# adelacvg/NS2VC

Measured on NVIDIA B200. Metric: denoiser-steps/s, higher is better.
Workload: dtype f32 (3xBF16-split tensor-core contractions, fp32 accumulate)

## Files before the change

### ns2vc_b200/csrc/common.cuh

```cuda
#pragma once
#include <cuda_runtime.h>
#include <cuda_bf16.h>
#include <stdint.h>
#include <stddef.h>

namespace ns2vc {

void set_error(const char* fmt, ...);
const char* get_error();

#define NS_CHECK_CUDA(expr)                                                                    \
  do {                                                                                         \
    cudaError_t _e = (expr);                                                                   \
    if (_e != cudaSuccess) {                                                                   \
      ns2vc::set_error("%s:%d CUDA error %s: %s", __FILE__, __LINE__, cudaGetErrorName(_e),    \
                       cudaGetErrorString(_e));                                                \
      return -2;                                                                               \
    }                                                                                          \
  } while (0)

#define NS_REQUIRE(cond, ...)                                                                  \
  do {                                                                                         \
    if (!(cond)) {                                                                             \
      ns2vc::set_error(__VA_ARGS__);                                                           \
      return -1;                                                                               \
    }                                                                                          \
  } while (0)

struct SplitBuf {
  __nv_bfloat16* hi;
  __nv_bfloat16* lo;
  int T;
  int C;
  int ld;
  long long bpitch;
};

struct alignas(128) TMap { unsigned long long v[16]; };

enum PrepMode : int { PREP_RAW = 0, PREP_AFFINE = 1, PREP_AFFINE_SILU = 2 };
struct GnStats {
  const double* sum1; const double* sq1;
  const double* sum2; const double* sq2;
  const float* gamma; const float* beta;
  const float* film; int film_ld;
  int G; float eps;
  double inv_n;
};
struct alignas(16) PrepOp {
  const float* src1; int ld1; int C1;
  const float* src2; int ld2; int C2;
  int B, T_src, T_dst;
  int row_mul, row_add;
  const int* rowmap;
  int mode;
  const float* scale; const float* shift;
  GnStats gn;
  SplitBuf out;
  SplitBuf raw;
  unsigned long long* span;
};

constexpr int kMaxSrc = 4;
constexpr int kMaxSeg = 8;

struct GSeg {
  int src;
  int c0;
  int nkb;
  int tap;
};

enum EpiFlags : int {
  EPI_BIAS = 1,
  EPI_RESIDUAL = 2,
  EPI_GEGLU = 4,
  EPI_OUT_NCT = 8,
  EPI_ROWBIAS = 16,
  EPI_OUT_F32 = 32,
  EPI_OUT_SPLIT = 64,
  EPI_STATS = 128,
  EPI_LNFOLD = 256,
  EPI_ROWSTATS = 512,
  EPI_RELU = 1024,
  EPI_ROWMASK = 2048,
};

constexpr int kMaxXSeg = 4;
struct XSeg {
  int src;
  int c0;
  int ncb;
  int ntap;
  int kb_tap[3];
  int xf;
  int aff_c0;
};

struct GemmOp {
  SplitBuf src[kMaxSrc];
  int nsrc;
  GSeg seg[kMaxSeg];
  int nseg;
  int nkb_total;
  int B, T_out;
  const __nv_bfloat16* w_hi;
  const __nv_bfloat16* w_lo;
  const float* w_f32;
  int N;
  int flags;
  const float* bias;
  const float* rowbias;
  int rowbias_ld;
  const float* res;
  int res_ld;
  float* out;
  int out_ld;
  __nv_bfloat16* out_hi;
  __nv_bfloat16* out_lo;
  int out_split_ld;
  int n_valid;
  const double* ln_stats;
  const float* ln_g;
  int ln_C; float ln_eps;
  double* row_stats;
  int f16_col0;
  double* stat_sum;
  double* stat_sq;
  unsigned long long* trace;
  unsigned long long* span;
  int tma_out;
  int bn;
  int xmode;
  int ksplit;
  int nxs;
  XSeg xs[kMaxXSeg];
  const PrepOp* pre;
  const float* pre_film;
  const float* rowmask;
  TMap tmap[2 * kMaxSrc];
  TMap tmap_out[3];
};
void plan_gemm(GemmOp& op);
constexpr int kXfMaxC = 1024;
int gemm_sm_count();

int launch_gemm_tc(const GemmOp& op, cudaStream_t st);
int launch_gemm_simt(const GemmOp& op, cudaStream_t st);
int encode_tmaps(GemmOp& op);

struct PackSeg {
  const float* w;
  int n_rows;
  int cin_total;
  int ktaps;
  int tap;
  int cin0, ncin;
  int n_dst0;
  int kb0;
  int nkb;
  int geglu_half;
  const float* cscale;
};
int launch_pack_b(const PackSeg& ps, __nv_bfloat16* w_hi, __nv_bfloat16* w_lo, float* w_f32, int Npad,
                  cudaStream_t st);

int launch_prep_split(const PrepOp& op, cudaStream_t st);

int launch_ln_split(const float* x, int ld, int M, int C, float eps, const float* gamma, const float* beta,
                    SplitBuf out, cudaStream_t st, unsigned long long* span = nullptr);

struct AttnOp {
  const float* q; int q_ld;
  const float* k; int k_ld;
  const float* v; int v_ld;
  const float* bias;
  float* out; int out_ld;
  __nv_bfloat16* out_hi;
  __nv_bfloat16* out_lo;
  int out_split_ld;
  int B, H, Tq, Tk, dh;
  float scale;
  unsigned long long* span;
  unsigned long long* trace;
  SplitBuf qs, ks, vs;
  int q_c0, k_c0, v_c0;
  int v2;
  int pb;
  int p_split;
  TMap tm[6];
};
int launch_attention(const AttnOp& op, cudaStream_t st, bool simt_debug);
int launch_attention_v2(const AttnOp& op, cudaStream_t st);
bool attention_v2_supported(int dh, int Tk, bool biased);
bool attention_v2_p_fp16();
int encode_attn_tmaps(AttnOp& op);
int encode_tmap_rows(TMap* out, const __nv_bfloat16* base, int C, int T, int B, int ld, int box_c, int box_rows, int swizzle_bytes);
int encode_tmap_any(TMap* out, const void* base, int elem_bytes, int C, int T, int B, int ld, int box_c, int box_rows, int swizzle_bytes,
                    long long bpitch = 0);

int launch_ln_stats(const float* x, int ld, int M, int C, float eps, float* stats , cudaStream_t st);
int launch_ln_apply(const float* x, int ld, int M, int C, float eps, const float* gamma, const float* beta,
                    float* y, int y_ld, cudaStream_t st);

int launch_nct_to_tokens(const float* x, long long bstride, int B, int C, int T, float* out, int ldo, int Cpad,
                         cudaStream_t st);
int launch_nct_to_split(const float* x, long long bstride, int B, int C, int T, SplitBuf out, cudaStream_t st, const void* warm = nullptr,
                        long long warm_bytes = 0);
int launch_tokens_to_nct(const float* x, int ld, int B, int C, int T, float* out, cudaStream_t st);

enum LinIn : int { LIN_RAW = 0, LIN_SILU = 1, LIN_SINUSOID = 2 };
struct LinOp {
  const float* x; int x_ld; int M; int K;
  const float* W; const float* bias; int N;
  const float* add; int add_ld;
  int add_rows;
  float* out; int out_ld;
  int in_mode; int flip_sin_to_cos; float freq_shift;
  int out_silu;
};
int launch_small_linear(const LinOp& op, cudaStream_t st);

int launch_pool_class_token(const float* xn , const float* pos , int B, int S, int C,
                            float* tokens , cudaStream_t st);
int launch_pool_attend(const float* q , const float* kv , int B, int S1, int C, int heads,
                       float* out , cudaStream_t st);
int launch_mask_bias(const uint8_t* mask, int n, float* bias, cudaStream_t st);

struct DpmStepCoef {
  float alpha_s, sigma_s;
  float c_x;
  float c_m;
  float c_d;
  float inv_r0;
  int order;
};
int launch_dpm_step(const float* x, const float* unet_out, const float* m_prev, const DpmStepCoef& c,
                    float* m_cur, float* x_next, size_t n, int* nan_flag, cudaStream_t st);

struct UniPcStepCoef {
  float alpha_t, sigma_t;
  float c_x, c_m;
  float ab;
  float rk;
  float rho0, rho1;
  int corr_order;
  float n_c_x, n_c_m, nab, nrk;
  int pred_order;
};
int launch_unipc_step(const float* x_prev, const float* x_eval, const float* unet_out, const float* m0,
                      const float* m1, const UniPcStepCoef& c, float* m_t, float* x_t, float* x_pred, size_t n,
                      int* nan_flag, cudaStream_t st);

int launch_seq_mask(const long long* len, int B, int T, float* keep, float* kbias, cudaStream_t st);
int launch_enc_input(const float* x, long long bstride, const float* rowbias, const float* keep, int B, int C, int T, float* out, int ld,
                     cudaStream_t st);
int launch_ln_mask(const float* x, int ld, int M, int C, float eps, const float* gamma, const float* beta, const float* keep, float* y, int y_ld,
                   cudaStream_t st);
int launch_pool_attend_wide(const float* q, const float* kv, int B, int S1, int C, int heads, float* out, cudaStream_t st);
int launch_tbc_weight(const float* w, int k, int cin, int cout, float* o, cudaStream_t st);
int launch_ffn_taps(const float* const* w, int k, int F, int H, int centre, float scale, float* o, cudaStream_t st);
int launch_scale_vec(const float* a, float s, float* o, int n, cudaStream_t st);
int launch_ln_fold_vec(const float* W, const float* gamma, const float* beta, const float* bias, float* g, float* bf, int N, int C, cudaStream_t st);

inline int ceil_div(int a, int b) { return (a + b - 1) / b; }

}
```

### ns2vc_b200/csrc/engine.cu

```cuda
#include "common.cuh"
#include "../../include/ns2vc_b200.h"

#include <algorithm>
#include <cmath>
#include <cstdio>
#include <cstdlib>
#include <cstring>
#include <map>
#include <string>
#include <unordered_map>
#include <vector>

using namespace ns2vc;

namespace {

struct PlanOp {
  enum Kind { PUSH, POP_CAT, RESNET, XFORMER, DOWN, UP } kind;
  std::string prefix;
  int cin = 0, cout = 0, level = 0;
  int c1 = 0, c2 = 0;
};

struct WSlot {
  std::string name;
  std::vector<int64_t> shape;
  float* d = nullptr;
  bool loaded = false;
  size_t numel() const { size_t n = 1; for (auto s : shape) n *= (size_t)s; return n; }
};

struct PackedB {
  __nv_bfloat16* hi = nullptr;
  __nv_bfloat16* lo = nullptr;
  float* f32 = nullptr;
  int Npad = 0, nkb = 0, n_logical = 0;
};

inline int pad_to(int v, int m) { return (v + m - 1) / m * m; }
inline int nkb_of(int c) { return (c + 63) / 64; }

struct ResnetSite {
  std::string p;
  int c1, c2, cin, cout;
  bool shortcut;
  PackedB conv1, conv2;
  float* bias2 = nullptr;
  int film_off = 0;
};
struct XformerSite {
  std::string p;
  int c;
  PackedB proj_in, qkv, out1, q2, out2, ff1, ff2, proj_out;
  PackedB ff2p; float* bias_ff2p = nullptr;
  int kv_off = 0;
  int v_off = 0;
  float* g_qkv = nullptr; float* bf_qkv = nullptr;
  float* g_q2 = nullptr; float* bf_q2 = nullptr;
  float* g_ff1 = nullptr; float* bf_ff1 = nullptr;
};
struct ConvSite { std::string p; int c; PackedB w; };

struct Launch {
  enum Kind { GEMM, ATTN, LN_SPLIT, LN_APPLY, LINEAR, NCT2SPLIT, POOL_CLS, POOL_ATT, MASKBIAS, PREP, MEMSET, TAP } kind;
  GemmOp gemm;
  AttnOp attn;
  LinOp lin;
  PrepOp prep;
  SplitBuf split;
  const float* a = nullptr; const float* b = nullptr; const float* c = nullptr; float* o = nullptr;
  int i0 = 0, i1 = 0, i2 = 0, i3 = 0; float f0 = 0;
  void* mem = nullptr; size_t mem_bytes = 0;
  int patch = 0;
  int tap_index = -1;
  int reads_film = 0;
  int time_path = 0;
};

struct Arena {
  uint8_t* base = nullptr;
  size_t off = 0;
  template <class T> T* get(size_t n) {
    off = (off + 255) & ~(size_t)255;
    T* p = base ? reinterpret_cast<T*>(base + off) : nullptr;
    off += n * sizeof(T);
    return p;
  }
};

}

struct ns2vc_unet {
  ns2vc_unet_cfg cfg;
  int ted = 0;
  std::vector<PlanOp> plan;
  std::vector<WSlot> weights;
  std::unordered_map<std::string, int> windex;
  bool finalized = false;
  bool simt = false;
  std::string plan_str;

  std::vector<ResnetSite> resnets;
  std::vector<XformerSite> xformers;
  std::vector<ConvSite> resamplers;
  PackedB convin_lat, convin_content, conv_out, kv_all;
  int kv_total = 0, k_total = 0, film_total = 0;
  float* film_W = nullptr; float* film_b = nullptr;
  float* pool_kv_W = nullptr; float* pool_kv_b = nullptr;
  std::vector<void*> owned;

  int pB = 0, pT = 0, pS = 0; void* pws = nullptr; bool has_mask = false; bool cond_ready = false;
  float* aug = nullptr;
  std::vector<void*> static_bufs;
  std::vector<Launch> prog_cond, prog_fwd;
  std::vector<std::string> tap_names; std::vector<int> tap_level, tap_ch;
  std::vector<float*> tap_dst;
  struct Stash {
    int pB, pT, pS; void* pws; bool has_mask, cond_ready;
    std::vector<Launch> prog_cond, prog_fwd; float* film_base; float* aug;
    std::vector<std::string> tap_names; std::vector<int> tap_level, tap_ch; std::vector<float*> tap_dst;
  };
  std::vector<Stash> stash;
  int last_launches = 0;
  bool profiling = false;
  bool ksplit = true;
  bool xf = true;
  bool merge_ff = true;
  float* film_base = nullptr;
  const float* film_ext = nullptr;
  bool lnfold = true;
  unsigned long long* trace = nullptr; int trace_cap = 0;
  unsigned long long* attn_trace = nullptr; int attn_trace_cap = 0;
  unsigned long long* span = nullptr; int span_cap = 0;
  struct ProfRec { int kind; cudaEvent_t a, b; int M, N, K, nseg, ctas; };
  std::vector<ProfRec> prof;

  const float* W(const std::string& n) const {
    auto it = windex.find(n);
    return it == windex.end() ? nullptr : weights[it->second].d;
  }
};

namespace {

int level_len(int T, int level) {
  for (int i = 0; i < level; ++i) T = (T - 1) / 2 + 1;
  return T;
}

void add_w(ns2vc_unet* h, const std::string& n, std::vector<int64_t> shape) {
  h->windex[n] = (int)h->weights.size();
  WSlot s; s.name = n; s.shape = std::move(shape);
  h->weights.push_back(std::move(s));
}
void add_conv(ns2vc_unet* h, const std::string& p, int co, int ci, int k) { add_w(h, p + ".weight", {co, ci, k}); add_w(h, p + ".bias", {co}); }
void add_lin(ns2vc_unet* h, const std::string& p, int co, int ci, bool bias = true) { add_w(h, p + ".weight", {co, ci}); if (bias) add_w(h, p + ".bias", {co}); }
void add_norm(ns2vc_unet* h, const std::string& p, int c) { add_w(h, p + ".weight", {c}); add_w(h, p + ".bias", {c}); }

void build_plan(ns2vc_unet* h) {
  const ns2vc_unet_cfg& c = h->cfg;
  const int n = c.n_levels;
  std::vector<int> skip;
  auto push = [&](int ch, int level) { PlanOp o; o.kind = PlanOp::PUSH; o.cout = ch; o.level = level; h->plan.push_back(o); skip.push_back(ch); };
  int ch = c.block_out_channels[0], level = 0;
  push(ch, 0);
  for (int i = 0; i < n; ++i) {
    const int cout = c.block_out_channels[i];
    for (int j = 0; j < c.layers_per_block[i]; ++j) {
      PlanOp r; r.kind = PlanOp::RESNET; r.prefix = "down_blocks." + std::to_string(i) + ".resnets." + std::to_string(j);
      r.cin = ch; r.cout = cout; r.level = level; r.c1 = ch; r.c2 = 0; h->plan.push_back(r);
      ch = cout;
      if (c.down_has_attn[i]) {
        PlanOp x; x.kind = PlanOp::XFORMER; x.prefix = "down_blocks." + std::to_string(i) + ".attentions." + std::to_string(j);
        x.cin = x.cout = ch; x.level = level; h->plan.push_back(x);
      }
      push(ch, level);
    }
    if (i != n - 1) {
      ++level;
      PlanOp d; d.kind = PlanOp::DOWN; d.prefix = "down_blocks." + std::to_string(i) + ".downsamplers.0"; d.cin = d.cout = ch; d.level = level;
      h->plan.push_back(d);
      push(ch, level);
    }
  }
  auto res = [&](const std::string& p, int c1, int c2, int cout) {
    PlanOp r; r.kind = PlanOp::RESNET; r.prefix = p; r.cin = c1 + c2; r.cout = cout; r.level = level; r.c1 = c1; r.c2 = c2; h->plan.push_back(r);
  };
  auto xf = [&](const std::string& p, int cc) {
    PlanOp x; x.kind = PlanOp::XFORMER; x.prefix = p; x.cin = x.cout = cc; x.level = level; h->plan.push_back(x);
  };
  res("mid_block.resnets.0", ch, 0, ch);
  xf("mid_block.attentions.0", ch);
  res("mid_block.resnets.1", ch, 0, ch);
  for (int i = 0; i < n; ++i) {
    const int cout = c.block_out_channels[n - 1 - i];
    const int layers = c.layers_per_block[n - 1 - i] + 1;
    for (int j = 0; j < layers; ++j) {
      const int sk = skip.back(); skip.pop_back();
      PlanOp pc; pc.kind = PlanOp::POP_CAT; pc.cin = ch; pc.cout = ch + sk; pc.level = level; h->plan.push_back(pc);
      res("up_blocks." + std::to_string(i) + ".resnets." + std::to_string(j), ch, sk, cout);
      ch = cout;
      if (c.up_has_attn[i]) xf("up_blocks." + std::to_string(i) + ".attentions." + std::to_string(j), ch);
    }
    if (i != n - 1) {
      --level;
      PlanOp u; u.kind = PlanOp::UP; u.prefix = "up_blocks." + std::to_string(i) + ".upsamplers.0"; u.cin = u.cout = ch; u.level = level;
      h->plan.push_back(u);
    }
  }
  static const char* kn[] = {"push", "pop_cat", "resnet", "xformer", "down", "up"};
  for (auto& o : h->plan) {
    char buf[256];
    snprintf(buf, sizeof(buf), "%s|%s|%d|%d|%d\n", kn[o.kind], o.prefix.c_str(), o.cin, o.cout, o.level);
    h->plan_str += buf;
  }
}

void register_weights(ns2vc_unet* h) {
  const ns2vc_unet_cfg& c = h->cfg;
  const int c0 = c.block_out_channels[0], ted = h->ted, xd = c.cross_attention_dim;
  add_conv(h, "conv_in", c0, c.in_channels, 3);
  add_lin(h, "time_embedding.linear_1", ted, c0);
  add_lin(h, "time_embedding.linear_2", ted, ted);
  if (c.add_embed_text) {
    add_norm(h, "add_embedding.norm1", xd);
    add_w(h, "add_embedding.pool.positional_embedding", {1, xd});
    add_lin(h, "add_embedding.pool.k_proj", xd, xd);
    add_lin(h, "add_embedding.pool.q_proj", xd, xd);
    add_lin(h, "add_embedding.pool.v_proj", xd, xd);
    add_lin(h, "add_embedding.proj", ted, xd);
    add_norm(h, "add_embedding.norm2", ted);
  }
  for (auto& o : h->plan) {
    if (o.kind == PlanOp::RESNET) {
      const std::string& p = o.prefix;
      add_norm(h, p + ".norm1", o.cin);
      add_conv(h, p + ".conv1", o.cout, o.cin, 3);
      add_lin(h, p + ".time_emb_proj", c.time_scale_shift ? 2 * o.cout : o.cout, ted);
      add_norm(h, p + ".norm2", o.cout);
      add_conv(h, p + ".conv2", o.cout, o.cout, 3);
      if (o.cin != o.cout) add_conv(h, p + ".conv_shortcut", o.cout, o.cin, 1);
    } else if (o.kind == PlanOp::XFORMER) {
      const std::string& p = o.prefix; const int cc = o.cout;
      add_norm(h, p + ".norm", cc);
      add_conv(h, p + ".proj_in", cc, cc, 1);
      const std::string b = p + ".transformer_blocks.0";
      add_norm(h, b + ".norm1", cc);
      add_lin(h, b + ".attn1.to_q", cc, cc, false); add_lin(h, b + ".attn1.to_k", cc, cc, false); add_lin(h, b + ".attn1.to_v", cc, cc, false);
      add_lin(h, b + ".attn1.to_out.0", cc, cc);
      add_norm(h, b + ".norm2", cc);
      add_lin(h, b + ".attn2.to_q", cc, cc, false); add_lin(h, b + ".attn2.to_k", cc, xd, false); add_lin(h, b + ".attn2.to_v", cc, xd, false);
      add_lin(h, b + ".attn2.to_out.0", cc, cc);
      add_norm(h, b + ".norm3", cc);
      add_lin(h, b + ".ff.net.0.proj", 8 * cc, cc);
      add_lin(h, b + ".ff.net.2", cc, 4 * cc);
      add_conv(h, p + ".proj_out", cc, cc, 1);
    } else if (o.kind == PlanOp::DOWN || o.kind == PlanOp::UP) {
      add_conv(h, o.prefix + ".conv", o.cout, o.cin, 3);
    }
  }
  add_norm(h, "conv_norm_out", c0);
  add_conv(h, "conv_out", c.out_channels, c0, 3);
}

template <class T>
int dev_alloc(ns2vc_unet* h, T** p, size_t n, bool zero) {
  void* q = nullptr;
  NS_CHECK_CUDA(cudaMalloc(&q, std::max<size_t>(n, 1) * sizeof(T)));
  if (zero) NS_CHECK_CUDA(cudaMemset(q, 0, std::max<size_t>(n, 1) * sizeof(T)));
  h->owned.push_back(q);
  *p = reinterpret_cast<T*>(q);
  return 0;
}

int alloc_packed(ns2vc_unet* h, PackedB& pb, int n_logical, int n_packed, int nkb) {
  pb.n_logical = n_logical;
  pb.Npad = pad_to(n_packed, 128);
  pb.nkb = nkb;
  const size_t elems = (size_t)nkb * pb.Npad * 64;
  if (dev_alloc(h, &pb.hi, elems, true)) return -2;
  if (dev_alloc(h, &pb.lo, elems, true)) return -2;
  if (h->simt) { if (dev_alloc(h, &pb.f32, elems, true)) return -2; }
  return 0;
}

__global__ void ln_fold_vec_kernel(const float* __restrict__ W, const float* __restrict__ gamma, const float* __restrict__ beta,
                                   const float* __restrict__ bias, float* __restrict__ g, float* __restrict__ bf, int N, int C) {
  const int n = blockIdx.x * (blockDim.x >> 5) + (threadIdx.x >> 5), lane = threadIdx.x & 31;
  if (n >= N) return;
  double sg = 0, sb = 0;
  for (int c = lane; c < C; c += 32) { const double w = W[(long long)n * C + c]; sg += w * gamma[c]; sb += w * beta[c]; }
  for (int o = 16; o > 0; o >>= 1) { sg += __shfl_xor_sync(0xffffffffu, sg, o); sb += __shfl_xor_sync(0xffffffffu, sb, o); }
  if (lane == 0) { g[n] = (float)sg; bf[n] = (float)(sb + (bias ? (double)bias[n] : 0.0)); }
}
int ln_fold_vectors(ns2vc_unet* h, const std::string& wname, const std::string& bname, const std::string& norm, int N, int C,
                    float* g, float* bf, int n_dst0, cudaStream_t st) {
  const float* W = h->W(wname); const float* ga = h->W(norm + ".weight"); const float* be = h->W(norm + ".bias");
  NS_REQUIRE(W && ga && be, "ln fold: %s / %s missing", wname.c_str(), norm.c_str());
  const float* bias = bname.empty() ? nullptr : h->W(bname);
  ln_fold_vec_kernel<<<ceil_div(N, 8), 256, 0, st>>>(W, ga, be, bias, g + n_dst0, bf + n_dst0, N, C);
  NS_CHECK_CUDA(cudaGetLastError());
  return 0;
}

int pack_seg_ptr(ns2vc_unet* h, PackedB& pb, const float* w, int n_rows, int cin_total, int ktaps, int tap, int cin0,
                 int ncin, int n_dst0, int kb0, int geglu_half, cudaStream_t st, const float* cscale = nullptr);
int pack_seg(ns2vc_unet* h, PackedB& pb, const std::string& wname, int n_rows, int cin_total, int ktaps, int tap, int cin0,
             int ncin, int n_dst0, int kb0, int geglu_half, cudaStream_t st, const float* cscale = nullptr) {
  const float* w = h->W(wname);
  NS_REQUIRE(w != nullptr, "pack: weight %s missing", wname.c_str());
  return pack_seg_ptr(h, pb, w, n_rows, cin_total, ktaps, tap, cin0, ncin, n_dst0, kb0, geglu_half, st, cscale);
}
int pack_seg_ptr(ns2vc_unet* h, PackedB& pb, const float* w, int n_rows, int cin_total, int ktaps, int tap, int cin0,
                 int ncin, int n_dst0, int kb0, int geglu_half, cudaStream_t st, const float* cscale) {
  (void)h;
  PackSeg ps;
  ps.cscale = cscale;
  ps.w = w; ps.n_rows = n_rows; ps.cin_total = cin_total; ps.ktaps = ktaps; ps.tap = tap; ps.cin0 = cin0; ps.ncin = ncin;
  ps.n_dst0 = n_dst0; ps.kb0 = kb0; ps.nkb = nkb_of(ncin); ps.geglu_half = geglu_half;
  return launch_pack_b(ps, pb.hi, pb.lo, pb.f32, pb.Npad, st);
}

__global__ void matmul_nn_kernel(const float* __restrict__ Wp, const float* __restrict__ W2, float* __restrict__ Wm, int N, int Cmid, int K) {
  const int k = blockIdx.x * blockDim.x + threadIdx.x, n = blockIdx.y;
  if (k >= K || n >= N) return;
  double acc = 0;
  for (int c = 0; c < Cmid; ++c) acc += (double)Wp[(long long)n * Cmid + c] * (double)W2[(long long)c * K + k];
  Wm[(long long)n * K + k] = (float)acc;
}
__global__ void matvec_bias_kernel(const float* __restrict__ Wp, const float* __restrict__ b2, const float* __restrict__ bp, float* __restrict__ bm, int N, int Cmid) {
  const int n = blockIdx.x * blockDim.x + threadIdx.x;
  if (n >= N) return;
  double acc = bp[n];
  for (int c = 0; c < Cmid; ++c) acc += (double)Wp[(long long)n * Cmid + c] * (double)b2[c];
  bm[n] = (float)acc;
}

__global__ void add_vec_kernel(const float* a, const float* b, float* o, int n) {
  int i = blockIdx.x * blockDim.x + threadIdx.x;
  if (i < n) o[i] = a[i] + (b ? b[i] : 0.f);
}

int pack_all(ns2vc_unet* h, cudaStream_t st) {
  const ns2vc_unet_cfg& c = h->cfg;
  const int c0 = c.block_out_channels[0];
  const int Cl = c.latent_channels, Cc = c.in_channels - c.latent_channels;
  int rc;
  {
    const int nl = nkb_of(Cl);
    if ((rc = alloc_packed(h, h->convin_lat, c0, c0, 3 * nl))) return rc;
    for (int j = 0; j < 3; ++j)
      if ((rc = pack_seg(h, h->convin_lat, "conv_in.weight", c0, c.in_channels, 3, j, 0, Cl, 0, j * nl, 0, st))) return rc;
    if (Cc > 0) {
      const int nc = nkb_of(Cc);
      if ((rc = alloc_packed(h, h->convin_content, c0, c0, 3 * nc))) return rc;
      for (int j = 0; j < 3; ++j)
        if ((rc = pack_seg(h, h->convin_content, "conv_in.weight", c0, c.in_channels, 3, j, Cl, Cc, 0, j * nc, 0, st))) return rc;
    }
  }
  int film_off = 0, kv_off = 0;
  for (auto& o : h->plan) {
    if (o.kind == PlanOp::RESNET) {
      ResnetSite s; s.p = o.prefix; s.c1 = o.c1; s.c2 = o.c2; s.cin = o.cin; s.cout = o.cout; s.shortcut = o.cin != o.cout;
      const int ni = nkb_of(s.cin), no = nkb_of(s.cout);
      if ((rc = alloc_packed(h, s.conv1, s.cout, s.cout, 3 * ni))) return rc;
      for (int j = 0; j < 3; ++j)
        if ((rc = pack_seg(h, s.conv1, s.p + ".conv1.weight", s.cout, s.cin, 3, j, 0, s.cin, 0, j * ni, 0, st))) return rc;
      const int nsc = s.shortcut ? ni : 0;
      if ((rc = alloc_packed(h, s.conv2, s.cout, s.cout, 3 * no + nsc))) return rc;
      for (int j = 0; j < 3; ++j)
        if ((rc = pack_seg(h, s.conv2, s.p + ".conv2.weight", s.cout, s.cout, 3, j, 0, s.cout, 0, j * no, 0, st))) return rc;
      if (s.shortcut)
        if ((rc = pack_seg(h, s.conv2, s.p + ".conv_shortcut.weight", s.cout, s.cin, 1, 0, 0, s.cin, 0, 3 * no, 0, st))) return rc;
      if (dev_alloc(h, &s.bias2, s.cout, false)) return -2;
      add_vec_kernel<<<ceil_div(s.cout, 256), 256, 0, st>>>(h->W(s.p + ".conv2.bias"), s.shortcut ? h->W(s.p + ".conv_shortcut.bias") : nullptr, s.bias2, s.cout);
      s.film_off = film_off;
      film_off += c.time_scale_shift ? 2 * s.cout : s.cout;
      h->resnets.push_back(s);
    } else if (o.kind == PlanOp::XFORMER) {
      XformerSite x; x.p = o.prefix; x.c = o.cout;
      const int C = x.c, nk = nkb_of(C);
      const std::string b = x.p + ".transformer_blocks.0";
      if ((rc = alloc_packed(h, x.proj_in, C, C, nk))) return rc;
      if ((rc = pack_seg(h, x.proj_in, x.p + ".proj_in.weight", C, C, 1, 0, 0, C, 0, 0, 0, st))) return rc;
      if ((rc = alloc_packed(h, x.qkv, 3 * C, 3 * C, nk))) return rc;
      const char* qkvn[3] = {".attn1.to_q.weight", ".attn1.to_k.weight", ".attn1.to_v.weight"};
      const bool fold = h->lnfold;
      for (int i = 0; i < 3; ++i)
        if ((rc = pack_seg(h, x.qkv, b + qkvn[i], C, C, 1, 0, 0, C, i * C, 0, 0, st, fold ? h->W(b + ".norm1.weight") : nullptr))) return rc;
      if (fold) {
        if (dev_alloc(h, &x.g_qkv, (size_t)3 * C, false) || dev_alloc(h, &x.bf_qkv, (size_t)3 * C, false)) return -2;
        if (dev_alloc(h, &x.g_q2, (size_t)C, false) || dev_alloc(h, &x.bf_q2, (size_t)C, false)) return -2;
        if (dev_alloc(h, &x.g_ff1, (size_t)8 * C, false) || dev_alloc(h, &x.bf_ff1, (size_t)8 * C, false)) return -2;
        for (int i = 0; i < 3; ++i)
          if ((rc = ln_fold_vectors(h, b + qkvn[i], "", b + ".norm1", C, C, x.g_qkv, x.bf_qkv, i * C, st))) return rc;
        if ((rc = ln_fold_vectors(h, b + ".attn2.to_q.weight", "", b + ".norm2", C, C, x.g_q2, x.bf_q2, 0, st))) return rc;
        if ((rc = ln_fold_vectors(h, b + ".ff.net.0.proj.weight", b + ".ff.net.0.proj.bias", b + ".norm3", 8 * C, C, x.g_ff1, x.bf_ff1, 0, st))) return rc;
      }
      if ((rc = alloc_packed(h, x.out1, C, C, nk))) return rc;
      if ((rc = pack_seg(h, x.out1, b + ".attn1.to_out.0.weight", C, C, 1, 0, 0, C, 0, 0, 0, st))) return rc;
      if ((rc = alloc_packed(h, x.q2, C, C, nk))) return rc;
      if ((rc = pack_seg(h, x.q2, b + ".attn2.to_q.weight", C, C, 1, 0, 0, C, 0, 0, 0, st, fold ? h->W(b + ".norm2.weight") : nullptr))) return rc;
      if ((rc = alloc_packed(h, x.out2, C, C, nk))) return rc;
      if ((rc = pack_seg(h, x.out2, b + ".attn2.to_out.0.weight", C, C, 1, 0, 0, C, 0, 0, 0, st))) return rc;
      NS_REQUIRE((4 * C) % 64 == 0, "transformer width %d: 4C must be a multiple of 64", C);
      if ((rc = alloc_packed(h, x.ff1, 4 * C, 8 * C, nk))) return rc;
      if ((rc = pack_seg(h, x.ff1, b + ".ff.net.0.proj.weight", 8 * C, C, 1, 0, 0, C, 0, 0, 4 * C, st, fold ? h->W(b + ".norm3.weight") : nullptr))) return rc;
      if ((rc = alloc_packed(h, x.ff2, C, C, nkb_of(4 * C)))) return rc;
      if ((rc = pack_seg(h, x.ff2, b + ".ff.net.2.weight", C, 4 * C, 1, 0, 0, 4 * C, 0, 0, 0, st))) return rc;
      if ((rc = alloc_packed(h, x.proj_out, C, C, nk))) return rc;
      if ((rc = pack_seg(h, x.proj_out, x.p + ".proj_out.weight", C, C, 1, 0, 0, C, 0, 0, 0, st))) return rc;
      if (h->merge_ff && fold) {
        const float* Wp = h->W(x.p + ".proj_out.weight"); const float* W2 = h->W(b + ".ff.net.2.weight");
        NS_REQUIRE(Wp && W2, "pack: %s feed-forward / proj_out weights missing", x.p.c_str());
        float* Wm = nullptr;
        if (dev_alloc(h, &Wm, (size_t)C * 4 * C, false) || dev_alloc(h, &x.bias_ff2p, (size_t)C, false)) return -2;
        matmul_nn_kernel<<<dim3(ceil_div(4 * C, 128), C), 128, 0, st>>>(Wp, W2, Wm, C, C, 4 * C);
        matvec_bias_kernel<<<ceil_div(C, 128), 128, 0, st>>>(Wp, h->W(b + ".ff.net.2.bias"), h->W(x.p + ".proj_out.bias"), x.bias_ff2p, C, C);
        if ((rc = alloc_packed(h, x.ff2p, C, C, nkb_of(4 * C) + nk))) return rc;
        if ((rc = pack_seg_ptr(h, x.ff2p, Wm, C, 4 * C, 1, 0, 0, 4 * C, 0, 0, 0, st))) return rc;
        if ((rc = pack_seg(h, x.ff2p, x.p + ".proj_out.weight", C, C, 1, 0, 0, C, 0, nkb_of(4 * C), 0, st))) return rc;
      }
      x.kv_off = kv_off;
      kv_off += C;
      h->xformers.push_back(x);
    } else if (o.kind == PlanOp::DOWN || o.kind == PlanOp::UP) {
      ConvSite s; s.p = o.prefix; s.c = o.cout;
      const int nk = nkb_of(s.c);
      if ((rc = alloc_packed(h, s.w, s.c, s.c, 3 * nk))) return rc;
      for (int j = 0; j < 3; ++j)
        if ((rc = pack_seg(h, s.w, s.p + ".conv.weight", s.c, s.c, 3, j, 0, s.c, 0, j * nk, 0, st))) return rc;
      h->resamplers.push_back(s);
    }
  }
  h->film_total = film_off;
  h->k_total = kv_off;
  for (auto& x : h->xformers) x.v_off = h->k_total + x.kv_off;
  h->kv_total = 2 * kv_off;
  {
    const int nk = nkb_of(c0);
    if ((rc = alloc_packed(h, h->conv_out, c.out_channels, c.out_channels, 3 * nk))) return rc;
    for (int j = 0; j < 3; ++j)
      if ((rc = pack_seg(h, h->conv_out, "conv_out.weight", c.out_channels, c0, 3, j, 0, c0, 0, j * nk, 0, st))) return rc;
  }
  if (h->kv_total > 0) {
    const int xd = c.cross_attention_dim;
    if ((rc = alloc_packed(h, h->kv_all, h->kv_total, h->kv_total, nkb_of(xd)))) return rc;
    for (auto& x : h->xformers) {
      const std::string b = x.p + ".transformer_blocks.0";
      if ((rc = pack_seg(h, h->kv_all, b + ".attn2.to_k.weight", x.c, xd, 1, 0, 0, xd, x.kv_off, 0, 0, st))) return rc;
      if ((rc = pack_seg(h, h->kv_all, b + ".attn2.to_v.weight", x.c, xd, 1, 0, 0, xd, x.v_off, 0, 0, st))) return rc;
    }
  }
  if (dev_alloc(h, &h->film_W, (size_t)h->film_total * h->ted, false)) return -2;
  if (dev_alloc(h, &h->film_b, (size_t)h->film_total, false)) return -2;
  for (auto& s : h->resnets) {
    const int rows = c.time_scale_shift ? 2 * s.cout : s.cout;
    NS_CHECK_CUDA(cudaMemcpyAsync(h->film_W + (size_t)s.film_off * h->ted, h->W(s.p + ".time_emb_proj.weight"), (size_t)rows * h->ted * 4, cudaMemcpyDeviceToDevice, st));
    NS_CHECK_CUDA(cudaMemcpyAsync(h->film_b + s.film_off, h->W(s.p + ".time_emb_proj.bias"), (size_t)rows * 4, cudaMemcpyDeviceToDevice, st));
  }
  if (c.add_embed_text) {
    const int xd = c.cross_attention_dim;
    if (dev_alloc(h, &h->pool_kv_W, (size_t)2 * xd * xd, false)) return -2;
    if (dev_alloc(h, &h->pool_kv_b, (size_t)2 * xd, false)) return -2;
    NS_CHECK_CUDA(cudaMemcpyAsync(h->pool_kv_W, h->W("add_embedding.pool.k_proj.weight"), (size_t)xd * xd * 4, cudaMemcpyDeviceToDevice, st));
    NS_CHECK_CUDA(cudaMemcpyAsync(h->pool_kv_W + (size_t)xd * xd, h->W("add_embedding.pool.v_proj.weight"), (size_t)xd * xd * 4, cudaMemcpyDeviceToDevice, st));
    NS_CHECK_CUDA(cudaMemcpyAsync(h->pool_kv_b, h->W("add_embedding.pool.k_proj.bias"), (size_t)xd * 4, cudaMemcpyDeviceToDevice, st));
    NS_CHECK_CUDA(cudaMemcpyAsync(h->pool_kv_b + xd, h->W("add_embedding.pool.v_proj.bias"), (size_t)xd * 4, cudaMemcpyDeviceToDevice, st));
  }
  NS_CHECK_CUDA(cudaGetLastError());
  return 0;
}

__global__ void nearest_index_kernel(int t_in, int t_out, int* idx) {
  const int i = blockIdx.x * blockDim.x + threadIdx.x;
  if (i >= t_out) return;
  int s;
  if (t_out == t_in) s = i;
  else if (t_out == 2 * t_in) s = i >> 1;
  else { const float scale = __fdiv_rn((float)t_in, (float)t_out); s = min((int)floorf(__fmul_rn((float)i, scale)), t_in - 1); }
  idx[i] = s;
}

struct Builder {
  ns2vc_unet* h;
  Arena ar;
  int B, T, S;
  std::vector<Launch>* out;
  bool dry;
  bool taps = false;
  int err = 0;

  SplitBuf split(int Tn, int C) {
    SplitBuf s{}; s.T = Tn; s.C = C; s.ld = pad_to(C, 8);
    s.hi = ar.get<__nv_bfloat16>((size_t)B * Tn * s.ld);
    s.lo = ar.get<__nv_bfloat16>((size_t)B * Tn * s.ld);
    return s;
  }
  static SplitBuf view(const SplitBuf& base, int Tn, int C) {
    SplitBuf s = base; s.T = Tn; s.C = C; s.ld = pad_to(C, 8); return s;
  }
  GemmOp gemm_base(const PackedB& w, int T_out) {
    GemmOp g; memset(&g, 0, sizeof(g));
    g.B = B; g.T_out = T_out;
    g.w_hi = w.hi; g.w_lo = w.lo; g.w_f32 = w.f32; g.N = w.Npad; g.n_valid = w.n_logical;
    g.f16_col0 = 0x7fffffff;
    g.ksplit = 1;
    return g;
  }
  int add_src(GemmOp& g, const SplitBuf& s) { g.src[g.nsrc] = s; return g.nsrc++; }
  void seg(GemmOp& g, int src, int c0, int nch, int tap) {
    GSeg& s = g.seg[g.nseg++];
    s.src = src; s.c0 = c0; s.nkb = nkb_of(nch); s.tap = tap;
    g.nkb_total += s.nkb;
  }
  void conv3(GemmOp& g, const SplitBuf& s) {
    const int i = add_src(g, s);
    for (int j = 0; j < 3; ++j) seg(g, i, 0, s.C, j - 1);
  }
  void emit_gemm(GemmOp& g, const PackedB& w, int patch = 0) {
    Launch l; l.kind = Launch::GEMM; l.patch = patch;
    if (g.xmode && h->ksplit) {
      const int tiles = B * ceil_div(g.T_out, 128) * (w.Npad / 64);
      int panels = 0;
      for (int i = 0; i < g.nxs; ++i) panels += g.xs[i].ncb;
      if (2 * tiles <= gemm_sm_count() && panels >= 8) g.ksplit = 2;
    }
    if (!dry) {
      if (g.nkb_total != w.nkb) { fprintf(stderr, "ns2vc: internal K mismatch %d vs %d\n", g.nkb_total, w.nkb); abort(); }
      plan_gemm(g);
      if (!h->simt) { int rc = encode_tmaps(g); if (rc) err = rc; }
    }
    l.gemm = g;
    if (g.pre_film || (g.flags & EPI_ROWBIAS)) l.reads_film = 1;
    out->push_back(l);
  }
  void xseg(GemmOp& g, int src, int c0, int nch, int ntap, int kb0, int kb_stride, int xf, int aff_c0) {
    XSeg& x = g.xs[g.nxs++];
    x.src = src; x.c0 = c0; x.ncb = nkb_of(nch); x.ntap = ntap; x.xf = xf; x.aff_c0 = aff_c0;
    for (int j = 0; j < 3; ++j) x.kb_tap[j] = kb0 + j * kb_stride;
    g.nkb_total += x.ncb * ntap;
    g.xmode = 1;
  }
  const PrepOp* affine_desc(const double* st1, int C1, const double* st2, int C2, int Tn, int mode, float eps, const float* gamma,
                            const float* beta, int film_ld) {
    PrepOp p; memset(&p, 0, sizeof(p));
    p.C1 = C1; p.C2 = C2; p.B = B; p.T_src = Tn; p.T_dst = Tn; p.mode = mode;
    p.gn.sum1 = st1; p.gn.sq1 = st1 ? st1 + (size_t)B * C1 : nullptr;
    p.gn.sum2 = st2; p.gn.sq2 = st2 ? st2 + (size_t)B * C2 : nullptr;
    p.gn.gamma = gamma; p.gn.beta = beta; p.gn.film_ld = film_ld; p.gn.G = h->cfg.norm_num_groups; p.gn.eps = eps;
    p.gn.inv_n = 1.0 / ((double)Tn * ((C1 + C2) / p.gn.G));
    if ((int)aff_host.size() >= aff_cap) { err = -1; set_error("internal: affine descriptor table full"); return nullptr; }
    aff_host.push_back(p);
    return aff_dev ? aff_dev + (aff_host.size() - 1) : reinterpret_cast<const PrepOp*>(uintptr_t(16));
  }
  std::vector<PrepOp> aff_host; PrepOp* aff_dev = nullptr; int aff_cap = 0;
  Arena sar;
  void reserve_affine(int n) { aff_cap = n; aff_dev = sar.get<PrepOp>((size_t)n); aff_host.reserve(n); }
  int upload_affine(cudaStream_t st) {
    if (dry || aff_host.empty()) return 0;
    return cudaMemcpyAsync(aff_dev, aff_host.data(), aff_host.size() * sizeof(PrepOp), cudaMemcpyHostToDevice, st) == cudaSuccess ? 0 : -2;
  }
  void push(const Launch& l) { out->push_back(l); }
  void emit_prep(const float* s1, int C1, const float* s2, int C2, int T_src, int T_dst, int mode, const float* scale,
                 const float* shift, const SplitBuf& o, const SplitBuf* raw = nullptr, int row_mul = 1, int row_add = 0,
                 const int* rowmap = nullptr, int patch = 0) {
    Launch l; l.kind = Launch::PREP; l.patch = patch;
    PrepOp& p = l.prep; memset(&p, 0, sizeof(p));
    p.src1 = s1; p.ld1 = C1; p.C1 = C1; p.src2 = s2; p.ld2 = C2; p.C2 = C2; p.B = B; p.T_src = T_src; p.T_dst = T_dst;
    p.row_mul = row_mul; p.row_add = row_add; p.rowmap = rowmap; p.mode = mode; p.scale = scale; p.shift = shift; p.out = o;
    if (raw) p.raw = *raw;
    out->push_back(l);
  }
  void emit_prep_gn(const float* s1, int C1, const double* st1, const float* s2, int C2, const double* st2, int Tn, int mode,
                    float eps, const float* gamma, const float* beta, const float* film, int film_ld, const SplitBuf& o,
                    const SplitBuf* raw = nullptr) {
    emit_prep(s1, C1, s2, C2, Tn, Tn, mode, nullptr, nullptr, o, raw);
    PrepOp& p = out->back().prep;
    if (film) out->back().reads_film = 1;
    p.gn.sum1 = st1; p.gn.sq1 = st1 ? st1 + (size_t)B * C1 : nullptr;
    p.gn.sum2 = st2; p.gn.sq2 = st2 ? st2 + (size_t)B * C2 : nullptr;
    p.gn.gamma = gamma; p.gn.beta = beta; p.gn.film = film; p.gn.film_ld = film_ld; p.gn.G = h->cfg.norm_num_groups; p.gn.eps = eps;
    p.gn.inv_n = 1.0 / ((double)Tn * ((C1 + C2) / p.gn.G));
  }
  void emit_ln_split(const float* x, int ld, int M, int C, const float* gamma, const float* beta, const SplitBuf& o) {
    Launch l; l.kind = Launch::LN_SPLIT; l.a = x; l.i0 = ld; l.i1 = M; l.i2 = C; l.f0 = 1e-5f; l.b = gamma; l.c = beta; l.split = o;
    push(l);
  }
  void emit_tap(const std::string& name, const float* src, int level, int C, int Tl) {
    if (!dry && taps) {
      Launch l; l.kind = Launch::TAP; l.a = src; l.i0 = B * Tl * C; l.tap_index = (int)h->tap_names.size(); push(l);
      h->tap_names.push_back(name); h->tap_level.push_back(level); h->tap_ch.push_back(C);
    }
  }
};

int build_programs(ns2vc_unet* h, int B, int T, int S, void* ws, size_t* bytes_out, cudaStream_t st = nullptr) {
  const ns2vc_unet_cfg& c = h->cfg;
  const bool dry = (ws == nullptr);
  const int nlev = c.n_levels;
  const int c0 = c.block_out_channels[0];
  const int Cl = c.latent_channels, Cc = c.in_channels - Cl;
  const int xd = c.cross_attention_dim, ted = h->ted;
  std::vector<int> Tl(nlev);
  for (int l = 0; l < nlev; ++l) Tl[l] = level_len(T, l);
  NS_REQUIRE(Tl[nlev - 1] >= 1 && T >= 1 && B >= 1 && S >= 1, "bad shape B=%d T=%d S=%d", B, T, S);

  std::vector<Launch> cond, fwd;
  if (!dry) {
    cudaStreamCaptureStatus cs = cudaStreamCaptureStatusNone;
    if (cudaStreamIsCapturing(st, &cs) == cudaSuccess && cs != cudaStreamCaptureStatusNone) {
      set_error("the first call for a new (B=%d, T=%d, S=%d, workspace) builds its launch program and must not run under stream capture", B, T, S);
      return -1;
    }
    h->tap_names.clear(); h->tap_level.clear(); h->tap_ch.clear();
  }
  Builder bld{h, Arena{(uint8_t*)ws, 0}, B, T, S, &cond, dry};
  Arena& ar = bld.ar;
  {
    const int n_aff = 2 * (int)h->resnets.size() + (int)h->xformers.size() + 2;
    size_t sbytes = 1024 + (size_t)n_aff * sizeof(PrepOp);
    for (auto& o : h->plan) if (o.kind == PlanOp::UP) sbytes += 256 + (size_t)Tl[o.level] * sizeof(int);
    if (!dry) {
      void* sb = nullptr;
      NS_CHECK_CUDA(cudaMalloc(&sb, sbytes));
      h->static_bufs.push_back(sb);
      bld.sar = Arena{(uint8_t*)sb, 0};
    }
    bld.reserve_affine(n_aff);
  }

  float* P = (Cc > 0) ? ar.get<float>((size_t)B * T * c0) : nullptr;
  float* kvc = ar.get<float>((size_t)B * S * std::max(h->kv_total, 1));
  SplitBuf kvs{};
  kvs.T = S; kvs.C = std::max(h->kv_total, 8); kvs.ld = pad_to(kvs.C, 8);
  kvs.hi = ar.get<__nv_bfloat16>((size_t)B * S * kvs.ld);
  kvs.lo = ar.get<__nv_bfloat16>((size_t)B * S * kvs.ld);
  float* maskbias = ar.get<float>((size_t)B * S);
  float* aug = ar.get<float>((size_t)B * ted);
  SplitBuf s_content = (Cc > 0) ? bld.split(T, Cc) : SplitBuf{};
  SplitBuf s_prompt = bld.split(S, xd);
  float* pn = ar.get<float>((size_t)B * S * xd);
  float* ptok = ar.get<float>((size_t)B * (S + 1) * xd);
  float* pq = ar.get<float>((size_t)B * xd);
  float* pkv = ar.get<float>((size_t)B * (S + 1) * 2 * xd);
  float* ppool = ar.get<float>((size_t)B * xd);
  float* pproj = ar.get<float>((size_t)B * ted);

  constexpr int kFp16MinKeys = 256;
  auto p16 = [&](int keys) { return attention_v2_p_fp16() && keys >= kFp16MinKeys; };

  if (Cc > 0) {
    { Launch l; l.kind = Launch::NCT2SPLIT; l.patch = 4; l.i0 = Cc; l.i1 = T; l.split = s_content; cond.push_back(l); }
    GemmOp g = bld.gemm_base(h->convin_content, T);
    bld.conv3(g, s_content);
    g.flags = EPI_BIAS | EPI_OUT_F32; g.bias = h->W("conv_in.bias"); g.out = P; g.out_ld = c0;
    bld.emit_gemm(g, h->convin_content);
  }
  { Launch l; l.kind = Launch::MASKBIAS; l.patch = 6; l.i0 = B * S; l.o = maskbias; cond.push_back(l); }
  if (h->kv_total > 0) {
    bld.emit_prep(nullptr, xd, nullptr, 0, S, S, PREP_RAW, nullptr, nullptr, s_prompt, nullptr, 1, 0, nullptr, 5);
    GemmOp g = bld.gemm_base(h->kv_all, S);
    const int i = bld.add_src(g, s_prompt);
    bld.seg(g, i, 0, xd, 0);
    g.flags = EPI_OUT_F32 | EPI_OUT_SPLIT; g.out = kvc; g.out_ld = h->kv_total;
    g.out_hi = kvs.hi; g.out_lo = kvs.lo; g.out_split_ld = kvs.ld;
    if (p16(S)) g.f16_col0 = h->k_total;
    bld.emit_gemm(g, h->kv_all);
  }
  if (c.add_embed_text) {
    { Launch l; l.kind = Launch::LN_APPLY; l.patch = 5; l.i0 = xd; l.i1 = B * S; l.i2 = xd; l.f0 = 1e-5f;
      l.b = h->W("add_embedding.norm1.weight"); l.c = h->W("add_embedding.norm1.bias"); l.o = pn; l.i3 = xd; cond.push_back(l); }
    { Launch l; l.kind = Launch::POOL_CLS; l.a = pn; l.b = h->W("add_embedding.pool.positional_embedding"); l.i0 = S; l.i1 = xd; l.o = ptok; cond.push_back(l); }
    { Launch l; l.kind = Launch::LINEAR; LinOp& o = l.lin; memset(&o, 0, sizeof(o));
      o.x = ptok; o.x_ld = (S + 1) * xd; o.M = B; o.K = xd; o.W = h->W("add_embedding.pool.q_proj.weight"); o.bias = h->W("add_embedding.pool.q_proj.bias");
      o.N = xd; o.out = pq; o.out_ld = xd; cond.push_back(l); }
    { Launch l; l.kind = Launch::LINEAR; LinOp& o = l.lin; memset(&o, 0, sizeof(o));
      o.x = ptok; o.x_ld = xd; o.M = B * (S + 1); o.K = xd; o.W = h->pool_kv_W; o.bias = h->pool_kv_b; o.N = 2 * xd; o.out = pkv; o.out_ld = 2 * xd; cond.push_back(l); }
    { Launch l; l.kind = Launch::POOL_ATT; l.a = pq; l.b = pkv; l.i0 = S + 1; l.i1 = xd; l.i2 = c.add_embed_heads; l.o = ppool; cond.push_back(l); }
    { Launch l; l.kind = Launch::LINEAR; LinOp& o = l.lin; memset(&o, 0, sizeof(o));
      o.x = ppool; o.x_ld = xd; o.M = B; o.K = xd; o.W = h->W("add_embedding.proj.weight"); o.bias = h->W("add_embedding.proj.bias"); o.N = ted; o.out = pproj; o.out_ld = ted; cond.push_back(l); }
    { Launch l; l.kind = Launch::LN_APPLY; l.a = pproj; l.i0 = ted; l.i1 = B; l.i2 = ted; l.f0 = 1e-5f;
      l.b = h->W("add_embedding.norm2.weight"); l.c = h->W("add_embedding.norm2.bias"); l.o = aug; l.i3 = ted; cond.push_back(l); }
  }

  bld.out = &fwd;
  bld.taps = true;
  SplitBuf s_xin = bld.split(T, Cl);
  float* temb1 = ar.get<float>((size_t)B * ted);
  float* emb = ar.get<float>((size_t)B * ted);
  float* film = ar.get<float>((size_t)B * std::max(h->film_total, 1));
  size_t stat_doubles = (size_t)2 * B * c0;
  for (auto& o : h->plan) {
    if (o.kind == PlanOp::RESNET) stat_doubles += (size_t)4 * B * o.cout;
    else if (o.kind == PlanOp::XFORMER || o.kind == PlanOp::DOWN || o.kind == PlanOp::UP) stat_doubles += (size_t)2 * B * o.cout;
    if (o.kind == PlanOp::XFORMER && h->lnfold) stat_doubles += (size_t)3 * 2 * B * Tl[o.level];
  }
  double* stat_arena = ar.get<double>(stat_doubles);
  size_t stat_used = 0;
  auto new_stats = [&](int C) { double* p = stat_arena ? stat_arena + stat_used : nullptr; stat_used += (size_t)2 * B * C; return p; };
  auto new_rowstats = [&](size_t nrows) { double* p = stat_arena ? stat_arena + stat_used : nullptr; stat_used += 2 * nrows; return p; };
  auto with_stats = [&](GemmOp& g, double* st_, int C) { g.flags |= EPI_STATS; g.stat_sum = st_; g.stat_sq = st_ ? st_ + (size_t)B * C : nullptr; };
  { Launch l; l.kind = Launch::MEMSET; l.mem = stat_arena; l.mem_bytes = stat_doubles * sizeof(double); fwd.push_back(l); }
  size_t max_act = (size_t)B * T * c0, max_cat = 0, max_ff = 1, max_qkv = 1;
  for (auto& o : h->plan) {
    const size_t rows = (size_t)B * Tl[o.level];
    if (o.kind == PlanOp::RESNET) { max_act = std::max(max_act, rows * o.cout); max_cat = std::max(max_cat, rows * o.cin); }
    if (o.kind == PlanOp::DOWN || o.kind == PlanOp::UP) { max_act = std::max(max_act, rows * o.cout); max_cat = std::max(max_cat, rows * o.cout); }
    if (o.kind == PlanOp::XFORMER) { max_act = std::max(max_act, rows * o.cout); max_ff = std::max(max_ff, rows * 4 * o.cout); max_qkv = std::max(max_qkv, rows * 3 * o.cout); }
  }
  max_cat = std::max(max_cat, max_act);
  float* rot[3]; for (int i = 0; i < 3; ++i) rot[i] = ar.get<float>(max_act);
  float* H1 = ar.get<float>(max_act);
  float* T0 = ar.get<float>(max_act);
  float* T1 = ar.get<float>(max_act);
  float* QKV = ar.get<float>(max_qkv);
  auto scratch_split = [&](size_t elems) { SplitBuf s{}; s.hi = ar.get<__nv_bfloat16>(elems); s.lo = ar.get<__nv_bfloat16>(elems); return s; };
  const SplitBuf SP_A = scratch_split(max_cat);
  const SplitBuf SP_R = scratch_split(max_cat);
  const SplitBuf SP_H = scratch_split(max_act);
  const SplitBuf SP_X = scratch_split(max_act);
  const SplitBuf SP_ATT = scratch_split(max_act);
  const SplitBuf SP_FF = scratch_split(max_ff);
  const SplitBuf SP_QKV = scratch_split(max_qkv);
  const SplitBuf SP_LN = scratch_split(max_act);

  { Launch l; l.kind = Launch::NCT2SPLIT; l.patch = 1; l.i0 = Cl; l.i1 = T; l.split = s_xin; fwd.push_back(l); }
  { Launch l; l.kind = Launch::LINEAR; l.patch = 2; LinOp& o = l.lin; memset(&o, 0, sizeof(o));
    o.x = nullptr; o.x_ld = 1; o.M = B; o.K = c0; o.W = h->W("time_embedding.linear_1.weight"); o.bias = h->W("time_embedding.linear_1.bias");
    o.N = ted; o.out = temb1; o.out_ld = ted; o.in_mode = LIN_SINUSOID; o.flip_sin_to_cos = c.flip_sin_to_cos; o.freq_shift = c.freq_shift; o.out_silu = 1; l.time_path = 1; fwd.push_back(l); }
  { Launch l; l.kind = Launch::LINEAR; LinOp& o = l.lin; memset(&o, 0, sizeof(o));
    o.x = temb1; o.x_ld = ted; o.M = B; o.K = ted; o.W = h->W("time_embedding.linear_2.weight"); o.bias = h->W("time_embedding.linear_2.bias");
    o.N = ted; o.out = emb; o.out_ld = ted; if (c.add_embed_text) { o.add = aug; o.add_ld = ted; } l.time_path = 1; fwd.push_back(l); }
  if (h->film_total > 0) {
    Launch l; l.kind = Launch::LINEAR; LinOp& o = l.lin; memset(&o, 0, sizeof(o));
    o.x = emb; o.x_ld = ted; o.M = B; o.K = ted; o.W = h->film_W; o.bias = h->film_b; o.N = h->film_total; o.out = film; o.out_ld = h->film_total; o.in_mode = LIN_SILU; l.time_path = 1; fwd.push_back(l);
  }

  struct Act { float* p = nullptr; SplitBuf sp{}; int c = 0; double* st = nullptr; };
  const bool xf_on = h->xf && !h->simt;
  SplitBuf rot_sp[3];
  for (int i = 0; i < 3; ++i) rot_sp[i] = xf_on ? scratch_split(max_act) : SplitBuf{};
  std::vector<Act> skips;
  int rot_i = 0;
  auto next_out = [&](bool is_skip, int TLn, int C) -> Act {
    Act a; a.c = C;
    const size_t elems = (size_t)B * TLn * C;
    if (is_skip) { a.p = ar.get<float>(elems); if (xf_on) a.sp = Builder::view(scratch_split((size_t)B * TLn * pad_to(C, 8)), TLn, C); }
    else { a.p = rot[rot_i]; if (xf_on) a.sp = Builder::view(rot_sp[rot_i], TLn, C); rot_i = (rot_i + 1) % 3; }
    return a;
  };
  auto emits_block_out = [&](GemmOp& g, const Act& a) {
    g.flags |= EPI_OUT_F32; g.out = a.p; g.out_ld = a.c;
    if (xf_on) { g.flags |= EPI_OUT_SPLIT; g.out_hi = a.sp.hi; g.out_lo = a.sp.lo; g.out_split_ld = a.sp.ld; }
  };
  auto xf_ok = [&](int c1, int c2) { return xf_on && (c2 == 0 || c1 % 64 == 0) && c1 + c2 <= kXfMaxC && c.norm_num_groups <= 64; };
  auto followed_by_push = [&](size_t i) { return i + 1 < h->plan.size() && h->plan[i + 1].kind == PlanOp::PUSH; };

  Act cur;
  {
    Act o = next_out(true, T, c0);
    GemmOp g = bld.gemm_base(h->convin_lat, T);
    bld.conv3(g, s_xin);
    if (Cc > 0) { g.flags |= EPI_RESIDUAL; g.res = P; g.res_ld = c0; }
    else { g.flags |= EPI_BIAS; g.bias = h->W("conv_in.bias"); }
    emits_block_out(g, o);
    o.st = new_stats(c0);
    with_stats(g, o.st, c0);
    bld.emit_gemm(g, h->convin_lat);
    cur = o;
    bld.emit_tap("conv_in", cur.p, 0, c0, T);
  }
  Act cat2;
  size_t ri = 0, xi = 0, si = 0;
  for (size_t pi = 0; pi < h->plan.size(); ++pi) {
    const PlanOp& o = h->plan[pi];
    const int TL = Tl[o.level];
    const size_t rows = (size_t)B * TL;
    switch (o.kind) {
      case PlanOp::PUSH: skips.push_back(cur); break;
      case PlanOp::POP_CAT: cat2 = skips.back(); skips.pop_back(); break;
      case PlanOp::RESNET: {
        const ResnetSite& s = h->resnets[ri++];
        const float* s1 = cur.p; const float* s2 = s.c2 ? cat2.p : nullptr;
        const SplitBuf a_h = Builder::view(SP_H, TL, s.cout);
        double* h1_st = new_stats(s.cout);
        Act outp = next_out(followed_by_push(pi), TL, s.cout);
        outp.st = new_stats(s.cout);
        if (xf_ok(s.c1, s.c2) && s.cout <= kXfMaxC) {
          const int ni = nkb_of(s.cin), n1 = nkb_of(s.c1), no = nkb_of(s.cout);
          {
            GemmOp g = bld.gemm_base(s.conv1, TL);
            const int i0 = bld.add_src(g, cur.sp);
            bld.xseg(g, i0, 0, s.c1, 3, 0, ni, 1, 0);
            if (s.c2) { const int i1 = bld.add_src(g, cat2.sp); bld.xseg(g, i1, 0, s.c2, 3, n1, ni, 1, s.c1); }
            g.pre = bld.affine_desc(cur.st, s.c1, s.c2 ? cat2.st : nullptr, s.c2, TL, PREP_AFFINE_SILU, c.norm_eps,
                                    h->W(s.p + ".norm1.weight"), h->W(s.p + ".norm1.bias"), 0);
            g.flags = EPI_BIAS | EPI_OUT_SPLIT; g.bias = h->W(s.p + ".conv1.bias");
            if (!c.time_scale_shift) { g.flags |= EPI_ROWBIAS; g.rowbias = film + s.film_off; g.rowbias_ld = h->film_total; }
            g.out_hi = a_h.hi; g.out_lo = a_h.lo; g.out_split_ld = a_h.ld;
            with_stats(g, h1_st, s.cout);
            bld.emit_gemm(g, s.conv1);
          }
          {
            GemmOp g = bld.gemm_base(s.conv2, TL);
            g.flags = EPI_BIAS; g.bias = s.bias2;
            if (s.shortcut) {
              const int a0 = bld.add_src(g, cur.sp);
              bld.xseg(g, a0, 0, s.c1, 1, 3 * no, 0, 0, 0);
              if (s.c2) { const int a1 = bld.add_src(g, cat2.sp); bld.xseg(g, a1, 0, s.c2, 1, 3 * no + n1, 0, 0, 0); }
            } else { g.flags |= EPI_RESIDUAL; g.res = s1; g.res_ld = s.c1; }
            const int j0 = bld.add_src(g, a_h);
            bld.xseg(g, j0, 0, s.cout, 3, 0, no, 1, 0);
            g.pre = bld.affine_desc(h1_st, s.cout, nullptr, 0, TL, PREP_AFFINE_SILU, c.norm_eps, h->W(s.p + ".norm2.weight"),
                                    h->W(s.p + ".norm2.bias"), h->film_total);
            g.pre_film = c.time_scale_shift ? film + s.film_off : nullptr;
            emits_block_out(g, outp);
            with_stats(g, outp.st, s.cout);
            bld.emit_gemm(g, s.conv2);
          }
        } else {
          const SplitBuf a_in = Builder::view(SP_A, TL, s.cin), a_raw = Builder::view(SP_R, TL, s.cin);
          bld.emit_prep_gn(s1, s.c1, cur.st, s2, s.c2, s.c2 ? cat2.st : nullptr, TL, PREP_AFFINE_SILU, c.norm_eps,
                           h->W(s.p + ".norm1.weight"), h->W(s.p + ".norm1.bias"), nullptr, 0, a_in, s.shortcut ? &a_raw : nullptr);
          {
            GemmOp g = bld.gemm_base(s.conv1, TL);
            bld.conv3(g, a_in);
            g.flags = EPI_BIAS | EPI_OUT_F32; g.bias = h->W(s.p + ".conv1.bias");
            if (!c.time_scale_shift) { g.flags |= EPI_ROWBIAS; g.rowbias = film + s.film_off; g.rowbias_ld = h->film_total; }
            g.out = H1; g.out_ld = s.cout;
            with_stats(g, h1_st, s.cout);
            bld.emit_gemm(g, s.conv1);
          }
          bld.emit_prep_gn(H1, s.cout, h1_st, nullptr, 0, nullptr, TL, PREP_AFFINE_SILU, c.norm_eps, h->W(s.p + ".norm2.weight"),
                           h->W(s.p + ".norm2.bias"), c.time_scale_shift ? film + s.film_off : nullptr, h->film_total, a_h);
          {
            GemmOp g = bld.gemm_base(s.conv2, TL);
            bld.conv3(g, a_h);
            g.flags = EPI_BIAS; g.bias = s.bias2;
            if (s.shortcut) { const int i = bld.add_src(g, a_raw); bld.seg(g, i, 0, s.cin, 0); }
            else { g.flags |= EPI_RESIDUAL; g.res = s1; g.res_ld = s.c1; }
            emits_block_out(g, outp);
            with_stats(g, outp.st, s.cout);
            bld.emit_gemm(g, s.conv2);
          }
        }
        cur = outp; cat2 = Act{};
        bld.emit_tap(s.p, cur.p, o.level, cur.c, TL);
        break;
      }
      case PlanOp::XFORMER: {
        const XformerSite& x = h->xformers[xi++];
        const int C = x.c, H = c.num_heads, dh = C / H;
        const std::string b = x.p + ".transformer_blocks.0";
        const SplitBuf sx = Builder::view(SP_X, TL, C), satt = Builder::view(SP_ATT, TL, C), sff = Builder::view(SP_FF, TL, 4 * C),
                       sh2 = Builder::view(SP_H, TL, C);
        auto lin = [&](const PackedB& w, const SplitBuf& in, int nch) { GemmOp g = bld.gemm_base(w, TL); const int i = bld.add_src(g, in); bld.seg(g, i, 0, nch, 0); return g; };
        const bool xin = xf_ok(C, 0);
        if (!xin) bld.emit_prep_gn(cur.p, C, cur.st, nullptr, 0, nullptr, TL, PREP_AFFINE, 1e-6f, h->W(x.p + ".norm.weight"), h->W(x.p + ".norm.bias"), nullptr, 0, sx);
        const bool fold = h->lnfold;
        const SplitBuf sln = Builder::view(SP_LN, TL, C);
        double* rs1 = fold ? new_rowstats(rows) : nullptr; double* rs2 = fold ? new_rowstats(rows) : nullptr; double* rs3 = fold ? new_rowstats(rows) : nullptr;
        auto emits_ln_input = [&](GemmOp& g, double* rs) { g.flags |= EPI_OUT_SPLIT | EPI_ROWSTATS; g.out_hi = sln.hi; g.out_lo = sln.lo; g.out_split_ld = sln.ld; g.row_stats = rs; };
        auto consumes_ln = [&](GemmOp& g, const double* rs, const float* gv, const float* bf) {
          g.flags |= EPI_LNFOLD | EPI_BIAS; g.ln_stats = rs; g.ln_g = gv; g.bias = bf; g.ln_C = C; g.ln_eps = 1e-5f; };
        { GemmOp g = xin ? bld.gemm_base(x.proj_in, TL) : lin(x.proj_in, sx, C);
          if (xin) {
            const int i0 = bld.add_src(g, cur.sp);
            bld.xseg(g, i0, 0, C, 1, 0, 0, 1, 0);
            g.pre = bld.affine_desc(cur.st, C, nullptr, 0, TL, PREP_AFFINE, 1e-6f, h->W(x.p + ".norm.weight"), h->W(x.p + ".norm.bias"), 0);
          }
          g.flags = EPI_BIAS | EPI_OUT_F32; g.bias = h->W(x.p + ".proj_in.bias"); g.out = T0; g.out_ld = C;
          if (fold) emits_ln_input(g, rs1);
          bld.emit_gemm(g, x.proj_in); }
        if (!fold) bld.emit_ln_split(T0, C, (int)rows, C, h->W(b + ".norm1.weight"), h->W(b + ".norm1.bias"), sx);
        const SplitBuf& sn = fold ? sln : sx;
        const bool av2 = !h->simt && attention_v2_supported(dh, TL, false) && attention_v2_supported(dh, S, true);
        const SplitBuf sqkv = Builder::view(SP_QKV, TL, 3 * C), sq2 = Builder::view(SP_QKV, TL, C);
        { GemmOp g = lin(x.qkv, sn, C);
          if (av2) { g.flags = EPI_OUT_SPLIT; g.out_hi = sqkv.hi; g.out_lo = sqkv.lo; g.out_split_ld = sqkv.ld;
                     if (p16(TL)) g.f16_col0 = 2 * C; }
          else { g.flags = EPI_OUT_F32; g.out = QKV; g.out_ld = 3 * C; }
          if (fold) consumes_ln(g, rs1, x.g_qkv, x.bf_qkv);
          bld.emit_gemm(g, x.qkv); }
        { Launch l; l.kind = Launch::ATTN; AttnOp& a = l.attn; memset(&a, 0, sizeof(a));
          a.q = QKV; a.q_ld = 3 * C; a.k = QKV + C; a.k_ld = 3 * C; a.v = QKV + 2 * C; a.v_ld = 3 * C;
          a.out_hi = satt.hi; a.out_lo = satt.lo; a.out_split_ld = satt.ld;
          a.B = B; a.H = H; a.Tq = TL; a.Tk = TL; a.dh = dh; a.scale = 1.0f / sqrtf((float)dh);
          if (av2) { a.v2 = 1; a.p_split = p16(TL) ? 0 : 1; a.qs = sqkv; a.ks = sqkv; a.vs = sqkv; a.q_c0 = 0; a.k_c0 = C; a.v_c0 = 2 * C;
                     if (!dry) { int rc = encode_attn_tmaps(a); if (rc) bld.err = rc; } }
          bld.push(l); }
        { GemmOp g = lin(x.out1, satt, C); g.flags = EPI_BIAS | EPI_RESIDUAL | EPI_OUT_F32; g.bias = h->W(b + ".attn1.to_out.0.bias"); g.res = T0; g.res_ld = C; g.out = T1; g.out_ld = C;
          if (fold) emits_ln_input(g, rs2);
          bld.emit_gemm(g, x.out1); }
        if (!fold) bld.emit_ln_split(T1, C, (int)rows, C, h->W(b + ".norm2.weight"), h->W(b + ".norm2.bias"), sx);
        { GemmOp g = lin(x.q2, sn, C);
          if (av2) { g.flags = EPI_OUT_SPLIT; g.out_hi = sq2.hi; g.out_lo = sq2.lo; g.out_split_ld = sq2.ld; }
          else { g.flags = EPI_OUT_F32; g.out = QKV; g.out_ld = C; }
          if (fold) consumes_ln(g, rs2, x.g_q2, x.bf_q2);
          bld.emit_gemm(g, x.q2); }
        { Launch l; l.kind = Launch::ATTN; AttnOp& a = l.attn; memset(&a, 0, sizeof(a));
          a.q = QKV; a.q_ld = C; a.k = kvc + x.kv_off; a.k_ld = h->kv_total; a.v = kvc + x.v_off; a.v_ld = h->kv_total; a.bias = maskbias;
          a.out_hi = satt.hi; a.out_lo = satt.lo; a.out_split_ld = satt.ld;
          a.B = B; a.H = H; a.Tq = TL; a.Tk = S; a.dh = dh; a.scale = 1.0f / sqrtf((float)dh); l.i0 = 1 ;
          if (av2) { a.v2 = 1; a.p_split = p16(S) ? 0 : 1; a.qs = sq2; a.ks = kvs; a.vs = kvs; a.q_c0 = 0; a.k_c0 = x.kv_off; a.v_c0 = x.v_off;
                     if (!dry) { int rc = encode_attn_tmaps(a); if (rc) bld.err = rc; } }
          bld.push(l); }
        { GemmOp g = lin(x.out2, satt, C); g.flags = EPI_BIAS | EPI_RESIDUAL | EPI_OUT_F32; g.bias = h->W(b + ".attn2.to_out.0.bias"); g.res = T1; g.res_ld = C; g.out = T0; g.out_ld = C;
          if (fold) emits_ln_input(g, rs3);
          bld.emit_gemm(g, x.out2); }
        if (!fold) bld.emit_ln_split(T0, C, (int)rows, C, h->W(b + ".norm3.weight"), h->W(b + ".norm3.bias"), sx);
        { GemmOp g = lin(x.ff1, sn, C); g.flags = EPI_GEGLU | EPI_OUT_SPLIT; g.bias = h->W(b + ".ff.net.0.proj.bias");
          g.out_hi = sff.hi; g.out_lo = sff.lo; g.out_split_ld = sff.ld;
          if (fold) { consumes_ln(g, rs3, x.g_ff1, x.bf_ff1); g.flags &= ~EPI_BIAS; }
          bld.emit_gemm(g, x.ff1); }
        Act outp = next_out(followed_by_push(pi), TL, C);
        outp.st = new_stats(C);
        if (h->merge_ff && fold) {
          GemmOp g = bld.gemm_base(x.ff2p, TL);
          const int i0 = bld.add_src(g, sff); bld.seg(g, i0, 0, 4 * C, 0);
          const int i1 = bld.add_src(g, sln); bld.seg(g, i1, 0, C, 0);
          g.flags = EPI_BIAS | EPI_RESIDUAL; g.bias = x.bias_ff2p; g.res = cur.p; g.res_ld = C;
          emits_block_out(g, outp); with_stats(g, outp.st, C); bld.emit_gemm(g, x.ff2p);
        } else {
          { GemmOp g = lin(x.ff2, sff, 4 * C); g.flags = EPI_BIAS | EPI_RESIDUAL | EPI_OUT_SPLIT; g.bias = h->W(b + ".ff.net.2.bias"); g.res = T0; g.res_ld = C;
            g.out_hi = sh2.hi; g.out_lo = sh2.lo; g.out_split_ld = sh2.ld; bld.emit_gemm(g, x.ff2); }
          { GemmOp g = lin(x.proj_out, sh2, C); g.flags = EPI_BIAS | EPI_RESIDUAL; g.bias = h->W(x.p + ".proj_out.bias"); g.res = cur.p; g.res_ld = C;
            emits_block_out(g, outp); with_stats(g, outp.st, C); bld.emit_gemm(g, x.proj_out); }
        }
        cur = outp;
        bld.emit_tap(x.p, cur.p, o.level, C, TL);
        break;
      }
      case PlanOp::DOWN: {
        const ConvSite& s = h->resamplers[si++];
        const int Tin = Tl[o.level - 1];
        const int To = Tin / 2;
        SplitBuf ev = Builder::view(SP_A, TL, s.c), od = Builder::view(SP_R, std::max(To, 1), s.c);
        if (xf_on && To >= 1) {
          ev = cur.sp; ev.T = TL; ev.ld = 2 * cur.sp.ld; ev.bpitch = (long long)Tin * cur.sp.ld;
          od = ev; od.hi += cur.sp.ld; od.lo += cur.sp.ld; od.T = To;
        } else {
          bld.emit_prep(cur.p, s.c, nullptr, 0, Tin, TL, PREP_RAW, nullptr, nullptr, ev, nullptr, 2, 0);
          bld.emit_prep(cur.p, s.c, nullptr, 0, Tin, std::max(To, 1), PREP_RAW, nullptr, nullptr, od, nullptr, 2, 1);
        }
        Act outp = next_out(followed_by_push(pi), TL, s.c);
        outp.st = new_stats(s.c);
        GemmOp g = bld.gemm_base(s.w, TL);
        const int ie = bld.add_src(g, ev), io = bld.add_src(g, od);
        bld.seg(g, io, 0, s.c, -1); bld.seg(g, ie, 0, s.c, 0); bld.seg(g, io, 0, s.c, 0);
        g.flags = EPI_BIAS; g.bias = h->W(s.p + ".conv.bias");
        emits_block_out(g, outp); with_stats(g, outp.st, s.c);
        bld.emit_gemm(g, s.w);
        cur = outp;
        bld.emit_tap(s.p, cur.p, o.level, s.c, TL);
        break;
      }
      case PlanOp::UP: {
        const ConvSite& s = h->resamplers[si++];
        const int Tin = Tl[o.level + 1];
        int* map_d = bld.sar.get<int>((size_t)TL);
        if (!dry) {
          nearest_index_kernel<<<ceil_div(TL, 256), 256, 0, st>>>(Tin, TL, map_d);
          NS_CHECK_CUDA(cudaGetLastError());
        }
        const SplitBuf up = Builder::view(SP_A, TL, s.c);
        bld.emit_prep(cur.p, s.c, nullptr, 0, Tin, TL, PREP_RAW, nullptr, nullptr, up, nullptr, 1, 0, map_d);
        Act outp = next_out(followed_by_push(pi), TL, s.c);
        outp.st = new_stats(s.c);
        GemmOp g = bld.gemm_base(s.w, TL);
        bld.conv3(g, up);
        g.flags = EPI_BIAS; g.bias = h->W(s.p + ".conv.bias");
        emits_block_out(g, outp); with_stats(g, outp.st, s.c);
        bld.emit_gemm(g, s.w);
        cur = outp;
        bld.emit_tap(s.p, cur.p, o.level, s.c, TL);
        break;
      }
    }
  }
  {
    const SplitBuf a_h = Builder::view(SP_H, T, c0);
    GemmOp g = bld.gemm_base(h->conv_out, T);
    if (xf_ok(c0, 0)) {
      const int i0 = bld.add_src(g, cur.sp);
      bld.xseg(g, i0, 0, c0, 3, 0, nkb_of(c0), 1, 0);
      g.pre = bld.affine_desc(cur.st, c0, nullptr, 0, T, PREP_AFFINE_SILU, c.norm_eps, h->W("conv_norm_out.weight"), h->W("conv_norm_out.bias"), 0);
    } else {
      bld.emit_prep_gn(cur.p, c0, cur.st, nullptr, 0, nullptr, T, PREP_AFFINE_SILU, c.norm_eps, h->W("conv_norm_out.weight"), h->W("conv_norm_out.bias"), nullptr, 0, a_h);
      bld.conv3(g, a_h);
    }
    g.flags = EPI_BIAS | EPI_OUT_NCT; g.bias = h->W("conv_out.bias"); g.out = nullptr;
    bld.emit_gemm(g, h->conv_out, 3);
  }
  if (!bld.err && bld.upload_affine(st)) { set_error("affine descriptor upload failed"); return -2; }
  if (bld.err) return bld.err;
  if (bytes_out) *bytes_out = ar.off + 256;
  if (!dry) {
    h->prog_cond = std::move(cond);
    h->prog_fwd = std::move(fwd);
    h->tap_dst.assign(h->tap_names.size(), nullptr);
    h->pB = B; h->pT = T; h->pS = S; h->pws = ws; h->cond_ready = false;
    h->film_base = film; h->aug = aug;
  }
  return 0;
}

int run_program(ns2vc_unet* h, std::vector<Launch>& prog, const float* x, long long x_bstride, const float* t, float* out,
                const float* content, long long content_bstride, const float* prompt, const uint8_t* mask, cudaStream_t st) {
  int rc = 0, count = 0, gemm_idx = 0, attn_idx = 0;
  const float* film_ext = h->film_ext;
  auto rebase = [&](const float* p) { return (film_ext && p) ? film_ext + (p - h->film_base) : p; };
  for (size_t li = 0; li < prog.size(); ++li) {
    Launch& l = prog[li];
    if (film_ext && l.time_path) continue;
    cudaEvent_t ev_a = nullptr, ev_b = nullptr;
    const bool prof = h->profiling && l.kind != Launch::TAP;
    if (prof) {
      cudaEventCreate(&ev_a); cudaEventCreate(&ev_b);
      cudaEventRecord(ev_a, st);
    }
    switch (l.kind) {
      case Launch::GEMM: {
        if (l.patch == 3 || h->trace || h->span || (film_ext && l.reads_film)) {
          GemmOp g = l.gemm;
          if (l.patch == 3) g.out = out;
          if (film_ext && l.reads_film) {
            g.rowbias = rebase(g.rowbias);
            g.pre_film = rebase(g.pre_film);
          }
          if (h->span && count < h->span_cap) g.span = h->span + 2 * count;
          if (h->trace && gemm_idx < h->trace_cap) g.trace = h->trace + 32 * gemm_idx;
          ++gemm_idx;
          rc = h->simt ? launch_gemm_simt(g, st) : launch_gemm_tc(g, st);
        } else {
          rc = h->simt ? launch_gemm_simt(l.gemm, st) : launch_gemm_tc(l.gemm, st);
        }
        break;
      }
      case Launch::ATTN: {
        AttnOp a = l.attn;
        if (l.i0 == 1 && !h->has_mask) a.bias = nullptr;
        if (h->span && count < h->span_cap) a.span = h->span + 2 * count;
        if (h->attn_trace && attn_idx < h->attn_trace_cap) a.trace = h->attn_trace + 2048 * attn_idx;
        ++attn_idx;
        rc = (a.v2 && !h->simt) ? launch_attention_v2(a, st) : launch_attention(a, st, h->simt);
        break;
      }
      case Launch::LN_SPLIT: rc = launch_ln_split(l.a, l.i0, l.i1, l.i2, l.f0, l.b, l.c, l.split, st, (h->span && count < h->span_cap) ? h->span + 2 * count : nullptr); break;
      case Launch::LN_APPLY: {
        const float* src = (l.patch == 5) ? prompt : l.a;
        rc = launch_ln_apply(src, l.i0, l.i1, l.i2, l.f0, l.b, l.c, l.o, l.i3, st);
        break;
      }
      case Launch::LINEAR: {
        LinOp o = l.lin;
        if (l.patch == 2) o.x = t;
        rc = launch_small_linear(o, st);
        break;
      }
      case Launch::NCT2SPLIT: {
        const float* src = (l.patch == 1) ? x : content;
        const long long bs = (l.patch == 1) ? x_bstride : content_bstride;
        const bool warm = l.patch == 1 && film_ext != nullptr;
        rc = launch_nct_to_split(src, bs, h->pB, l.i0, l.i1, l.split, st, warm ? film_ext : nullptr, warm ? (long long)h->pB * h->film_total * 4 : 0);
        break;
      }
      case Launch::PREP: {
        PrepOp p = l.prep;
        if (l.patch == 5) p.src1 = prompt;
        if (film_ext && l.reads_film) p.gn.film = rebase(p.gn.film);
        if (h->span && count < h->span_cap) p.span = h->span + 2 * count;
        rc = launch_prep_split(p, st);
        break;
      }
      case Launch::MEMSET: {
        cudaError_t e = cudaMemsetAsync(l.mem, 0, l.mem_bytes, st);
        if (e != cudaSuccess) { set_error("memset failed: %s", cudaGetErrorString(e)); rc = -2; }
        break;
      }
      case Launch::POOL_CLS: rc = launch_pool_class_token(l.a, l.b, h->pB, l.i0, l.i1, l.o, st); break;
      case Launch::POOL_ATT: rc = launch_pool_attend(l.a, l.b, h->pB, l.i0, l.i1, l.i2, l.o, st); break;
      case Launch::MASKBIAS:
        if (mask) rc = launch_mask_bias(mask, l.i0, l.o, st); else --count;
        break;
      case Launch::TAP:
        --count;
        if (l.tap_index >= 0 && l.tap_index < (int)h->tap_dst.size() && h->tap_dst[l.tap_index]) {
          cudaError_t e = cudaMemcpyAsync(h->tap_dst[l.tap_index], l.a, (size_t)l.i0 * sizeof(float), cudaMemcpyDeviceToDevice, st);
          if (e != cudaSuccess) { set_error("tap copy failed: %s", cudaGetErrorString(e)); rc = -2; }
        }
        break;
    }
    if (prof) {
      cudaEventRecord(ev_b, st);
      ns2vc_unet::ProfRec pr{(int)l.kind, ev_a, ev_b, 0, 0, 0, 0, 0};
      if (l.kind == Launch::GEMM) { pr.M = l.gemm.B * l.gemm.T_out; pr.N = l.gemm.n_valid; pr.K = l.gemm.nkb_total * 64; pr.nseg = l.gemm.nseg; }
      if (l.kind == Launch::PREP) { pr.M = l.prep.B * l.prep.T_dst; pr.N = l.prep.C1 + l.prep.C2; }
      if (l.kind == Launch::ATTN) { pr.M = l.attn.Tq; pr.N = l.attn.Tk; pr.K = l.attn.dh; }
      h->prof.push_back(pr);
    }
    if (rc) return rc;
    ++count;
  }
  h->last_launches = count;
  return 0;
}

void stash_active(ns2vc_unet* h) {
  if (!h->pws) return;
  ns2vc_unet::Stash s;
  s.pB = h->pB; s.pT = h->pT; s.pS = h->pS; s.pws = h->pws; s.has_mask = h->has_mask; s.cond_ready = false;
  s.prog_cond = std::move(h->prog_cond); s.prog_fwd = std::move(h->prog_fwd); s.film_base = h->film_base; s.aug = h->aug;
  s.tap_names = std::move(h->tap_names); s.tap_level = std::move(h->tap_level); s.tap_ch = std::move(h->tap_ch); s.tap_dst = std::move(h->tap_dst);
  h->prog_cond.clear(); h->prog_fwd.clear(); h->tap_names.clear(); h->tap_level.clear(); h->tap_ch.clear(); h->tap_dst.clear();
  h->pB = h->pT = h->pS = 0; h->pws = nullptr; h->cond_ready = false;
  if (h->stash.size() >= 16) h->stash.erase(h->stash.begin());
  h->stash.push_back(std::move(s));
}

void drop_all_programs(ns2vc_unet* h) {
  h->stash.clear();
  for (void* p : h->static_bufs) cudaFree(p);
  h->static_bufs.clear();
  h->prog_cond.clear(); h->prog_fwd.clear();
  h->pB = h->pT = h->pS = 0; h->pws = nullptr; h->cond_ready = false;
}

int ensure_program(ns2vc_unet* h, int B, int T, int S, void* ws, cudaStream_t st) {
  NS_REQUIRE(h->finalized, "ns2vc_unet_finalize() has not been called");
  NS_REQUIRE(ws != nullptr, "workspace is NULL");
  if (h->pB == B && h->pT == T && h->pS == S && h->pws == ws) return 0;
  stash_active(h);
  for (size_t i = 0; i < h->stash.size(); ++i) {
    ns2vc_unet::Stash& s = h->stash[i];
    if (s.pB == B && s.pT == T && s.pS == S && s.pws == ws) {
      h->pB = s.pB; h->pT = s.pT; h->pS = s.pS; h->pws = s.pws; h->has_mask = s.has_mask; h->cond_ready = s.cond_ready;
      h->prog_cond = std::move(s.prog_cond); h->prog_fwd = std::move(s.prog_fwd); h->film_base = s.film_base; h->aug = s.aug;
      h->tap_names = std::move(s.tap_names); h->tap_level = std::move(s.tap_level); h->tap_ch = std::move(s.tap_ch); h->tap_dst = std::move(s.tap_dst);
      h->stash.erase(h->stash.begin() + i);
      return 0;
    }
  }
  return build_programs(h, B, T, S, ws, nullptr, st);
}

}

extern "C" {

const char* ns2vc_last_error(void) { return ns2vc::get_error(); }

const char* ns2vc_build_info(void) { return "ns2vc_b200 sm_100a tcgen05/3xBF16 engine, built " __DATE__ " " __TIME__; }

int ns2vc_down_length(int t) { return (t - 1) / 2 + 1; }

int ns2vc_nearest_index(int t_in, int t_out, int* idx) {
  if (t_in <= 0 || t_out <= 0 || !idx) { ns2vc::set_error("nearest_index: bad sizes %d -> %d", t_in, t_out); return -1; }
  const float scale = (float)t_in / (float)t_out;
  for (int i = 0; i < t_out; ++i) {
    int s;
    if (t_out == t_in) s = i;
    else if (t_out == 2 * t_in) s = i >> 1;
    else s = std::min((int)floorf((float)i * scale), t_in - 1);
    idx[i] = s;
  }
  return 0;
}

int ns2vc_unet_create(const ns2vc_unet_cfg* cfg, ns2vc_unet** out) {
  NS_REQUIRE(cfg && out, "null argument");
  NS_REQUIRE(cfg->n_levels >= 1 && cfg->n_levels <= NS2VC_MAX_LEVELS, "n_levels %d out of range", cfg->n_levels);
  NS_REQUIRE(cfg->latent_channels >= 1 && cfg->latent_channels <= cfg->in_channels, "latent_channels %d invalid", cfg->latent_channels);
  for (int i = 0; i < cfg->n_levels; ++i) {
    const int c = cfg->block_out_channels[i];
    NS_REQUIRE(c % cfg->norm_num_groups == 0 && c % cfg->num_heads == 0 && c % 16 == 0,
               "block width %d must be divisible by groups %d, heads %d and 16", c, cfg->norm_num_groups, cfg->num_heads);
    NS_REQUIRE(cfg->layers_per_block[i] >= 1, "layers_per_block must be >= 1");
  }
  NS_REQUIRE(cfg->cross_attention_dim % 8 == 0, "cross_attention_dim must be a multiple of 8");
  if (cfg->add_embed_text)
    NS_REQUIRE(cfg->cross_attention_dim % cfg->add_embed_heads == 0 && cfg->cross_attention_dim / cfg->add_embed_heads <= 16,
               "addition_embed heads %d unsupported for dim %d", cfg->add_embed_heads, cfg->cross_attention_dim);
  ns2vc_unet* h = new ns2vc_unet();
  h->cfg = *cfg;
  h->ted = 4 * cfg->block_out_channels[0];
  const char* be = getenv("NS2VC_GEMM_BACKEND");
  h->simt = be && strcmp(be, "simt") == 0;
  { const char* e = getenv("NS2VC_LNFOLD"); h->lnfold = !(e && e[0] == '0'); }
  { const char* e = getenv("NS2VC_XF"); h->xf = !(e && e[0] == '0'); }
  { const char* e = getenv("NS2VC_KSPLIT"); h->ksplit = !(e && e[0] == '0'); }
  { const char* e = getenv("NS2VC_MERGE_FF"); h->merge_ff = !(e && e[0] == '0'); }
  build_plan(h);
  register_weights(h);
  *out = h;
  return 0;
}

void ns2vc_unet_destroy(ns2vc_unet* h) {
  if (!h) return;
  for (auto& w : h->weights) if (w.d) cudaFree(w.d);
  for (void* p : h->owned) cudaFree(p);
  drop_all_programs(h);
  delete h;
}

int ns2vc_unet_num_weights(const ns2vc_unet* h) { return h ? (int)h->weights.size() : -1; }

int ns2vc_unet_weight_info(const ns2vc_unet* h, int i, const char** name, int64_t shape[4], int* ndim) {
  NS_REQUIRE(h && i >= 0 && i < (int)h->weights.size(), "weight index %d out of range", i);
  const WSlot& w = h->weights[i];
  if (name) *name = w.name.c_str();
  if (ndim) *ndim = (int)w.shape.size();
  if (shape) for (size_t k = 0; k < w.shape.size() && k < 4; ++k) shape[k] = w.shape[k];
  return 0;
}

int ns2vc_unet_load_weight(ns2vc_unet* h, const char* key, const float* dptr, const int64_t* shape, int ndim, ns2vc_stream stream) {
  NS_REQUIRE(h && key && dptr, "null argument");
  auto it = h->windex.find(key);
  NS_REQUIRE(it != h->windex.end(), "Unexpected key in state_dict: %s", key);
  WSlot& w = h->weights[it->second];
  NS_REQUIRE(ndim == (int)w.shape.size(), "size mismatch for %s: expected %d dims, got %d", key, (int)w.shape.size(), ndim);
  for (int k = 0; k < ndim; ++k) NS_REQUIRE(shape[k] == w.shape[k], "size mismatch for %s at dim %d: expected %lld, got %lld", key, k, (long long)w.shape[k], (long long)shape[k]);
  if (!w.d) NS_CHECK_CUDA(cudaMalloc(&w.d, w.numel() * sizeof(float)));
  NS_CHECK_CUDA(cudaMemcpyAsync(w.d, dptr, w.numel() * sizeof(float), cudaMemcpyDeviceToDevice, (cudaStream_t)stream));
  w.loaded = true;
  h->finalized = false;
  return 0;
}

int ns2vc_unet_finalize(ns2vc_unet* h, ns2vc_stream stream) {
  NS_REQUIRE(h, "null handle");
  for (auto& w : h->weights) NS_REQUIRE(w.loaded, "Missing key in state_dict: %s", w.name.c_str());
  for (void* p : h->owned) cudaFree(p);
  h->owned.clear(); h->resnets.clear(); h->xformers.clear(); h->resamplers.clear();
  drop_all_programs(h);
  int rc = pack_all(h, (cudaStream_t)stream);
  if (rc) return rc;
  h->finalized = true;
  return 0;
}

int ns2vc_unet_workspace_bytes(const ns2vc_unet* h, int B, int T, int S, size_t* bytes) {
  NS_REQUIRE(h && bytes, "null argument");
  NS_REQUIRE(h->finalized, "ns2vc_unet_finalize() has not been called");
  return build_programs(const_cast<ns2vc_unet*>(h), B, T, S, nullptr, bytes);
}

int ns2vc_unet_prepare_cond(ns2vc_unet* h, const float* content, long long content_bstride, const float* prompt, const uint8_t* mask,
                            int B, int T, int S, void* ws, ns2vc_stream stream) {
  NS_REQUIRE(h && prompt, "null argument");
  int rc = ensure_program(h, B, T, S, ws, (cudaStream_t)stream);
  if (rc) return rc;
  const int Cc = h->cfg.in_channels - h->cfg.latent_channels;
  NS_REQUIRE(Cc == 0 || content != nullptr, "content is NULL but the model has %d content channels", Cc);
  h->has_mask = mask != nullptr;
  rc = run_program(h, h->prog_cond, nullptr, 0, nullptr, nullptr, content, content_bstride, prompt, mask, (cudaStream_t)stream);
  if (rc) return rc;
  h->cond_ready = true;
  return 0;
}

int ns2vc_unet_forward(ns2vc_unet* h, const float* x, long long x_bstride, const float* t, float* out, int B, int T, int S, void* ws,
                       ns2vc_stream stream) {
  NS_REQUIRE(h && x && t && out, "null argument");
  int rc0 = ensure_program(h, B, T, S, ws, (cudaStream_t)stream);
  if (rc0) return rc0;
  NS_REQUIRE(h->cond_ready, "ns2vc_unet_prepare_cond() must be called with the same (B,T,S,workspace) before forward");
  return run_program(h, h->prog_fwd, x, x_bstride, t, out, nullptr, 0, nullptr, nullptr, (cudaStream_t)stream);
}

int ns2vc_unet_film_width(const ns2vc_unet* h) { return h ? h->film_total : -1; }

size_t ns2vc_unet_time_table_floats(const ns2vc_unet* h, int n_rows) {
  if (!h || n_rows <= 0) return 0;
  return (size_t)n_rows * ((size_t)std::max(h->film_total, 1) + 2 * (size_t)h->ted);
}

int ns2vc_unet_time_table(ns2vc_unet* h, const float* t_rows, int n_rows, float* table, int B, int T, int S, void* ws, ns2vc_stream stream) {
  NS_REQUIRE(h && t_rows && table, "null argument");
  NS_REQUIRE(n_rows > 0 && n_rows % B == 0, "time table: %d rows is not a multiple of the batch %d", n_rows, B);
  int rc = ensure_program(h, B, T, S, ws, (cudaStream_t)stream);
  if (rc) return rc;
  NS_REQUIRE(h->cond_ready || !h->cfg.add_embed_text, "ns2vc_unet_prepare_cond() must precede ns2vc_unet_time_table() (the pooled prompt embedding is added to every row)");
  const ns2vc_unet_cfg& c = h->cfg;
  const int ted = h->ted, c0 = c.block_out_channels[0];
  float* film = table;
  float* temb1 = table + (size_t)n_rows * std::max(h->film_total, 1);
  float* emb = temb1 + (size_t)n_rows * ted;
  cudaStream_t st = (cudaStream_t)stream;
  { LinOp o; memset(&o, 0, sizeof(o));
    o.x = t_rows; o.x_ld = 1; o.M = n_rows; o.K = c0; o.W = h->W("time_embedding.linear_1.weight"); o.bias = h->W("time_embedding.linear_1.bias");
    o.N = ted; o.out = temb1; o.out_ld = ted; o.in_mode = LIN_SINUSOID; o.flip_sin_to_cos = c.flip_sin_to_cos; o.freq_shift = c.freq_shift; o.out_silu = 1;
    if ((rc = launch_small_linear(o, st))) return rc; }
  { LinOp o; memset(&o, 0, sizeof(o));
    o.x = temb1; o.x_ld = ted; o.M = n_rows; o.K = ted; o.W = h->W("time_embedding.linear_2.weight"); o.bias = h->W("time_embedding.linear_2.bias");
    o.N = ted; o.out = emb; o.out_ld = ted; if (c.add_embed_text) { o.add = h->aug; o.add_ld = ted; o.add_rows = B; }
    if ((rc = launch_small_linear(o, st))) return rc; }
  if (h->film_total > 0) {
    LinOp o; memset(&o, 0, sizeof(o));
    o.x = emb; o.x_ld = ted; o.M = n_rows; o.K = ted; o.W = h->film_W; o.bias = h->film_b; o.N = h->film_total; o.out = film; o.out_ld = h->film_total; o.in_mode = LIN_SILU;
    if ((rc = launch_small_linear(o, st))) return rc;
  }
  return 0;
}

int ns2vc_unet_forward_film(ns2vc_unet* h, const float* x, long long x_bstride, const float* film_rows, float* out, int B, int T, int S,
                            void* ws, ns2vc_stream stream) {
  NS_REQUIRE(h && x && film_rows && out, "null argument");
  int rc0 = ensure_program(h, B, T, S, ws, (cudaStream_t)stream);
  if (rc0) return rc0;
  NS_REQUIRE(h->cond_ready, "ns2vc_unet_prepare_cond() must be called with the same (B,T,S,workspace) before forward");
  NS_REQUIRE(h->film_total > 0, "the model has no FiLM rows");
  h->film_ext = film_rows;
  const int rc = run_program(h, h->prog_fwd, x, x_bstride, nullptr, out, nullptr, 0, nullptr, nullptr, (cudaStream_t)stream);
  h->film_ext = nullptr;
  return rc;
}

int ns2vc_dpm_step(const float* x, const float* unet_out, const float* m_prev, const ns2vc_dpm_coef* c, float* m_cur, float* x_next,
                   size_t n, int* nan_flag, ns2vc_stream stream) {
  NS_REQUIRE(x && unet_out && c && m_cur, "null argument");
  NS_REQUIRE(c->order == 0 || x_next, "x_next is NULL");
  NS_REQUIRE(c->order < 2 || m_prev, "m_prev is NULL for a second-order step");
  DpmStepCoef k; k.alpha_s = c->alpha_s; k.sigma_s = c->sigma_s; k.c_x = c->c_x; k.c_m = c->c_m; k.c_d = c->c_d; k.inv_r0 = c->inv_r0; k.order = c->order;
  return launch_dpm_step(x, unet_out, m_prev, k, m_cur, x_next, n, nan_flag, (cudaStream_t)stream);
}

int ns2vc_unipc_step(const float* x_prev, const float* x_eval, const float* unet_out, const float* m0, const float* m1,
                     const ns2vc_unipc_coef* c, float* m_t, float* x_t, float* x_pred, size_t n, int* nan_flag, ns2vc_stream stream) {
  NS_REQUIRE(x_eval && unet_out && c && m_t, "null argument");
  NS_REQUIRE(c->corr_order == 0 || (x_prev && m0 && x_t), "corrector inputs missing");
  NS_REQUIRE(c->corr_order < 2 || m1, "m1 is NULL for an order-2 corrector");
  NS_REQUIRE(c->pred_order == 0 || x_pred, "x_pred is NULL");
  NS_REQUIRE(c->pred_order < 2 || c->corr_order > 0, "order-2 predictor needs the previous model output");
  UniPcStepCoef k;
  k.alpha_t = c->alpha_t; k.sigma_t = c->sigma_t; k.c_x = c->c_x; k.c_m = c->c_m; k.ab = c->ab; k.rk = c->rk; k.rho0 = c->rho0; k.rho1 = c->rho1;
  k.corr_order = c->corr_order; k.n_c_x = c->n_c_x; k.n_c_m = c->n_c_m; k.nab = c->nab; k.nrk = c->nrk; k.pred_order = c->pred_order;
  return launch_unipc_step(x_prev, x_eval, unet_out, m0, m1, k, m_t, x_t, x_pred, n, nan_flag, (cudaStream_t)stream);
}

int ns2vc_mask_bias(const uint8_t* mask, int n, float* bias, ns2vc_stream stream) {
  NS_REQUIRE(mask && bias && n >= 0, "bad argument");
  return launch_mask_bias(mask, n, bias, (cudaStream_t)stream);
}

int ns2vc_unet_num_taps(const ns2vc_unet* h) { return h ? (int)h->tap_names.size() : -1; }
int ns2vc_unet_tap_info(const ns2vc_unet* h, int i, const char** name, int* level, int* channels) {
  NS_REQUIRE(h && i >= 0 && i < (int)h->tap_names.size(), "tap index %d out of range", i);
  if (name) *name = h->tap_names[i].c_str();
  if (level) *level = h->tap_level[i];
  if (channels) *channels = h->tap_ch[i];
  return 0;
}
int ns2vc_unet_set_tap(ns2vc_unet* h, int i, float* dst) {
  NS_REQUIRE(h && i >= 0 && i < (int)h->tap_dst.size(), "tap index %d out of range", i);
  h->tap_dst[i] = dst;
  return 0;
}
int ns2vc_unet_set_attn_trace(ns2vc_unet* h, unsigned long long* dbuf, int n_launches) {
  if (!h) return -1;
  h->attn_trace = dbuf; h->attn_trace_cap = n_launches;
  return 0;
}
int ns2vc_unet_set_trace(ns2vc_unet* h, unsigned long long* dbuf, int n_gemms) {
  NS_REQUIRE(h, "null handle");
  h->trace = dbuf; h->trace_cap = n_gemms;
  return 0;
}
int ns2vc_unet_set_span_trace(ns2vc_unet* h, unsigned long long* dbuf, int n_launches) {
  NS_REQUIRE(h, "null handle");
  h->span = dbuf; h->span_cap = n_launches;
  return 0;
}
int ns2vc_unet_launch_kind(const ns2vc_unet* h, int i) {
  if (!h || i < 0) return -1;
  int c = 0;
  for (auto& l : h->prog_fwd) {
    if (l.kind == Launch::TAP) continue;
    if (c == i) return (int)l.kind;
    ++c;
  }
  return -1;
}
int ns2vc_unet_set_profiling(ns2vc_unet* h, int on) {
  NS_REQUIRE(h, "null handle");
  h->profiling = on != 0;
  return 0;
}
int ns2vc_profile_num_kinds(void) { return 11; }
const char* ns2vc_profile_kind_name(int k) {
  static const char* names[] = {"gemm_tc", "attention", "ln_split", "ln_apply", "small_linear", "nct_to_split",
                               "pool_class_token", "pool_attend", "mask_bias", "prep_split", "memset"};
  return (k >= 0 && k < 11) ? names[k] : "";
}
int ns2vc_unet_profile_read(ns2vc_unet* h, int kind, double* ms_total, long long* launches) {
  NS_REQUIRE(h && ms_total && launches, "null argument");
  double ms = 0; long long n = 0;
  for (auto& r : h->prof) {
    if (r.kind != kind) continue;
    NS_CHECK_CUDA(cudaEventSynchronize(r.b));
    float e = 0;
    NS_CHECK_CUDA(cudaEventElapsedTime(&e, r.a, r.b));
    ms += e; ++n;
  }
  *ms_total = ms; *launches = n;
  return 0;
}
int ns2vc_unet_profile_dump(ns2vc_unet* h, const char* path) {
  NS_REQUIRE(h && path, "null argument");
  FILE* f = fopen(path, "w");
  NS_REQUIRE(f, "cannot open %s", path);
  fprintf(f, "idx,kind,us,M,N,K,nseg\n");
  int i = 0;
  for (auto& r : h->prof) {
    cudaEventSynchronize(r.b);
    float e = 0; cudaEventElapsedTime(&e, r.a, r.b);
    fprintf(f, "%d,%s,%.2f,%d,%d,%d,%d\n", i++, ns2vc_profile_kind_name(r.kind), e * 1e3f, r.M, r.N, r.K, r.nseg);
  }
  fclose(f);
  return 0;
}
int ns2vc_unet_profile_reset(ns2vc_unet* h) {
  NS_REQUIRE(h, "null handle");
  for (auto& r : h->prof) { cudaEventDestroy(r.a); cudaEventDestroy(r.b); }
  h->prof.clear();
  return 0;
}
const char* ns2vc_unet_plan_string(const ns2vc_unet* h) { return h ? h->plan_str.c_str() : ""; }
int ns2vc_unet_launch_count(const ns2vc_unet* h) { return h ? h->last_launches : -1; }

}
```

### ns2vc_b200/csrc/gemm_common.cuh

```cuda
#pragma once
#include "common.cuh"

namespace ns2vc {

__device__ __forceinline__ float silu_f(float v) {
  float e, r;
  asm("ex2.approx.ftz.f32 %0, %1;" : "=f"(e) : "f"(v * -1.4426950408889634f));
  asm("rcp.approx.ftz.f32 %0, %1;" : "=f"(r) : "f"(1.0f + e));
  return v * r;
}

__device__ __forceinline__ float gelu_erf_f(float v) {
  const float x = fabsf(v) * 0.70710678118654752440f;
  const float t = __fdividef(1.0f, fmaf(0.3275911f, x, 1.0f));
  float p = fmaf(t, 1.061405429f, -1.453152027f);
  p = fmaf(t, p, 1.421413741f);
  p = fmaf(t, p, -0.284496736f);
  p = fmaf(t, p, 0.254829592f);
  const float erf_abs = 1.0f - p * t * __expf(-x * x);
  return 0.5f * v * (1.0f + copysignf(erf_abs, v));
}

__device__ __forceinline__ uint32_t pack_bf16x2(float a, float b) {
  __nv_bfloat162 t = __floats2bfloat162_rn(a, b);
  return *reinterpret_cast<uint32_t*>(&t);
}

__device__ __forceinline__ unsigned long long pk2(float a, float b) { unsigned long long r; asm("mov.b64 %0, {%1, %2};" : "=l"(r) : "f"(a), "f"(b)); return r; }
__device__ __forceinline__ void upk2(unsigned long long v, float& a, float& b) { asm("mov.b64 {%0, %1}, %2;" : "=f"(a), "=f"(b) : "l"(v)); }
__device__ __forceinline__ unsigned long long ffma2(unsigned long long a, unsigned long long b, unsigned long long c) {
  unsigned long long d; asm("fma.rn.f32x2 %0, %1, %2, %3;" : "=l"(d) : "l"(a), "l"(b), "l"(c)); return d; }
__device__ __forceinline__ unsigned long long fadd2(unsigned long long a, unsigned long long b) {
  unsigned long long d; asm("add.rn.f32x2 %0, %1, %2;" : "=l"(d) : "l"(a), "l"(b)); return d; }
__device__ __forceinline__ unsigned long long fsub2(unsigned long long a, unsigned long long b) {
  unsigned long long d; asm("sub.rn.f32x2 %0, %1, %2;" : "=l"(d) : "l"(a), "l"(b)); return d; }
__device__ __forceinline__ unsigned long long fmul2(unsigned long long a, unsigned long long b) {
  unsigned long long d; asm("mul.rn.f32x2 %0, %1, %2;" : "=l"(d) : "l"(a), "l"(b)); return d; }

__device__ __forceinline__ void split2(float a, float b, uint32_t& hi, uint32_t& lo) {
  hi = pack_bf16x2(a, b);
  const float ha = __uint_as_float(hi << 16), hb = __uint_as_float(hi & 0xffff0000u);
  float la, lb;
  upk2(fsub2(pk2(a, b), pk2(ha, hb)), la, lb);
  lo = pack_bf16x2(la, lb);
}

__device__ __forceinline__ unsigned long long gelu_erf2(unsigned long long v2) {
  float a, b;
  upk2(v2, a, b);
  const unsigned long long x2 = pk2(fabsf(a) * 0.70710678118654752440f, fabsf(b) * 0.70710678118654752440f);
  float da, db;
  upk2(ffma2(pk2(0.3275911f, 0.3275911f), x2, pk2(1.0f, 1.0f)), da, db);
  float ta, tb;
  asm("rcp.approx.ftz.f32 %0, %1;" : "=f"(ta) : "f"(da));
  asm("rcp.approx.ftz.f32 %0, %1;" : "=f"(tb) : "f"(db));
  const unsigned long long t2 = pk2(ta, tb);
  unsigned long long p2 = ffma2(t2, pk2(1.061405429f, 1.061405429f), pk2(-1.453152027f, -1.453152027f));
  p2 = ffma2(t2, p2, pk2(1.421413741f, 1.421413741f));
  p2 = ffma2(t2, p2, pk2(-0.284496736f, -0.284496736f));
  p2 = ffma2(t2, p2, pk2(0.254829592f, 0.254829592f));
  float ea, eb;
  upk2(fmul2(fmul2(x2, x2), pk2(-1.4426950408889634f, -1.4426950408889634f)), ea, eb);
  asm("ex2.approx.ftz.f32 %0, %1;" : "=f"(ea) : "f"(ea));
  asm("ex2.approx.ftz.f32 %0, %1;" : "=f"(eb) : "f"(eb));
  float ra, rb;
  upk2(fsub2(pk2(1.0f, 1.0f), fmul2(fmul2(p2, t2), pk2(ea, eb))), ra, rb);
  const unsigned long long one_plus = fadd2(pk2(1.0f, 1.0f), pk2(copysignf(ra, a), copysignf(rb, b)));
  return fmul2(fmul2(v2, pk2(0.5f, 0.5f)), one_plus);
}

__device__ __forceinline__ unsigned long long silu2(unsigned long long y2) {
  float z0, z1, e0, e1, r0, r1, d0, d1;
  upk2(fmul2(y2, pk2(-1.4426950408889634f, -1.4426950408889634f)), z0, z1);
  asm("ex2.approx.ftz.f32 %0, %1;" : "=f"(e0) : "f"(z0));
  asm("ex2.approx.ftz.f32 %0, %1;" : "=f"(e1) : "f"(z1));
  upk2(fadd2(pk2(e0, e1), pk2(1.0f, 1.0f)), d0, d1);
  asm("rcp.approx.ftz.f32 %0, %1;" : "=f"(r0) : "f"(d0));
  asm("rcp.approx.ftz.f32 %0, %1;" : "=f"(r1) : "f"(d1));
  return fmul2(y2, pk2(r0, r1));
}

__device__ __forceinline__ uint32_t pack_f16x2(float lo, float hi) { uint32_t r; asm("cvt.rn.f16x2.f32 %0, %1, %2;" : "=r"(r) : "f"(hi), "f"(lo)); return r; }
__device__ __forceinline__ float f16lo_to_f32(uint32_t h2) { float f; asm("{.reg .f16 l, h; mov.b32 {l, h}, %1; cvt.f32.f16 %0, l;}" : "=f"(f) : "r"(h2)); return f; }
__device__ __forceinline__ float f16hi_to_f32(uint32_t h2) { float f; asm("{.reg .f16 l, h; mov.b32 {l, h}, %1; cvt.f32.f16 %0, h;}" : "=f"(f) : "r"(h2)); return f; }
__device__ __forceinline__ void split2_f16(float a, float b, uint32_t& hi, uint32_t& lo) {
  hi = pack_f16x2(a, b);
  float la, lb;
  upk2(fsub2(pk2(a, b), pk2(f16lo_to_f32(hi), f16hi_to_f32(hi))), la, lb);
  lo = pack_f16x2(la, lb);
}
__device__ __forceinline__ void split8_f16(const float* v, uint4& hi, uint4& lo) {
  split2_f16(v[0], v[1], hi.x, lo.x); split2_f16(v[2], v[3], hi.y, lo.y);
  split2_f16(v[4], v[5], hi.z, lo.z); split2_f16(v[6], v[7], hi.w, lo.w);
}

__device__ __forceinline__ void split8(const float* v, uint4& hi, uint4& lo) {
  split2(v[0], v[1], hi.x, lo.x); split2(v[2], v[3], hi.y, lo.y);
  split2(v[4], v[5], hi.z, lo.z); split2(v[6], v[7], hi.w, lo.w);
}

__device__ __forceinline__ float a_fetch_split(const GemmOp& op, const GSeg& s, int b, int t, int c) {
  const SplitBuf& src = op.src[s.src];
  const int r = t + s.tap, ch = s.c0 + c;
  if (r < 0 || r >= src.T || ch >= src.C) return 0.f;
  const long long off = (src.bpitch ? (long long)b * src.bpitch + (long long)r * src.ld : ((long long)b * src.T + r) * src.ld) + ch;
  return __bfloat162float(src.hi[off]) + __bfloat162float(src.lo[off]);
}

__device__ __forceinline__ void ln_row_stats(const GemmOp& op, long long m, float& mu, float& rstd) {
  const double s = op.ln_stats[m * 2], q = op.ln_stats[m * 2 + 1];
  const double mean = s / (double)op.ln_C;
  double var = q / (double)op.ln_C - mean * mean;
  if (var < 0) var = 0;
  mu = (float)mean;
  rstd = rsqrtf((float)var + op.ln_eps);
}

template <bool LNF = true>
__device__ __forceinline__ float epi_value(const GemmOp& op, int b, long long m, int n, float acc, float acc_gate) {
  if (LNF && (op.flags & EPI_LNFOLD)) {
    float mu, rstd;
    ln_row_stats(op, m, mu, rstd);
    acc = rstd * (acc - mu * __ldg(op.ln_g + n));
    if (op.flags & EPI_GEGLU) acc_gate = rstd * (acc_gate - mu * __ldg(op.ln_g + op.n_valid + n));
  }
  float v = acc;
  if (op.flags & EPI_GEGLU) {
    const int half = op.n_valid;
    v = (acc + __ldg(op.bias + n)) * gelu_erf_f(acc_gate + __ldg(op.bias + half + n));
  } else if (op.flags & EPI_BIAS) {
    v += __ldg(op.bias + n);
  }
  if (op.flags & EPI_ROWBIAS) v += __ldg(op.rowbias + (long long)b * op.rowbias_ld + n);
  if (op.flags & EPI_RESIDUAL) v += __ldg(op.res + m * op.res_ld + n);
  if (op.flags & EPI_RELU) v = fmaxf(v, 0.f);
  if (op.flags & EPI_ROWMASK) v *= __ldg(op.rowmask + m);
  return v;
}

}
```

### ns2vc_b200/csrc/gemm_tc.cu

```cuda
#include "gemm_common.cuh"
#include "prep_common.cuh"
#include "tc_common.cuh"
#include "launch.cuh"
#include <cuda.h>
#include <cuda_fp16.h>
#include <cstdlib>

namespace ns2vc {

constexpr int BM = 128;
constexpr int BK = 64;
constexpr int kEpiWarps = 8;
constexpr int kThreads = (2 + kEpiWarps) * 32;
constexpr int kATileBytes = BM * BK * 2;

constexpr int kMaxStages = 4;
constexpr int kStagePerWarp = 8192;
constexpr int kStageOff = 8192;
constexpr int kStagingBytes = kStageOff + kEpiWarps * kStagePerWarp;

constexpr int kPanelRows = BM + 2;
constexpr int kPanelBytes = 136 * 128;
constexpr int kXAStageBytes = 2 * kPanelBytes;
constexpr int kXBStageBytes = 3 * 2 * (64 * BK * 2);
constexpr int kXAStages = 3;
constexpr int kXBStages = 2;
constexpr int kXOffB = kXAStages * kXAStageBytes;
constexpr int kXOffAff = kXOffB + kXBStages * kXBStageBytes;
constexpr int kXAffBytes = (2 * kXfMaxC + 2 * 64) * 4;

template <int BN_> struct TileCfg {
  static constexpr int BN = BN_;
  static constexpr int kBTileBytes = BN_ * BK * 2;
  static constexpr int kStageBytes = 2 * kATileBytes + 2 * kBTileBytes;
  static constexpr int kStagesSingle = (BN_ == 128) ? 3 : 4;
  static constexpr int kStagesMulti = (BN_ == 128) ? 2 : 3;
  static constexpr int kOffStagingMulti = kStagesMulti * kStageBytes;
  static constexpr int kPipeBytes = (kStagesSingle * kStageBytes > kOffStagingMulti + kStagingBytes) ? kStagesSingle * kStageBytes : kOffStagingMulti + kStagingBytes;
  static constexpr int kOffBar = kPipeBytes;
  static constexpr int kOffDesc = kOffBar + 1024;
  static constexpr int kOffLnG = kOffDesc + 3072;
  static constexpr int kSmemBytes = kOffLnG + 4096 + 1024 ;
  static constexpr uint32_t kIdesc = umma_idesc_bf16(BM, BN_);
  static constexpr uint32_t kIdesc2 = umma_idesc_bf16(BM, 2 * BN_);
};
static_assert(TileCfg<64>::kSmemBytes <= 227 * 1024 && TileCfg<128>::kSmemBytes <= 227 * 1024, "shared memory budget");
static_assert(kXOffAff + kXAffBytes <= TileCfg<64>::kPipeBytes && kPrepSlots * kEpiWarps * 32 >= kXfMaxC, "panel mode: stages + affine table inside the pipeline area");


__device__ __forceinline__ float* stage_f32_ptr(uint8_t* st, int row, int c4) {
  return reinterpret_cast<float*>(st + row * 128 + ((c4 ^ (row & 7)) << 4));
}


template <bool LNF>
__device__ __noinline__ void epi_cold(const GemmOp& op, int b, long long m, int nbase, uint8_t* st, int lane, bool with_gate) {
#pragma unroll 1
  for (int j = 0; j < 32; ++j) {
    float* pv = stage_f32_ptr(st, lane, j >> 2) + (j & 3);
    const float g = with_gate ? reinterpret_cast<const float*>(st + 4096)[lane * 32 + j] : 0.f;
    *pv = (nbase + j < op.n_valid) ? epi_value<LNF>(op, b, m, nbase + j, *pv, g) : 0.f;
  }
}
__device__ __noinline__ void store_cold(const GemmOp& op, int flags, int b, int t, long long m, int nbase, uint8_t* st, int lane) {
  const bool f16 = nbase >= op.f16_col0;
#pragma unroll 1
  for (int j = 0; j < 32; ++j) {
    const int n = nbase + j;
    if (n >= op.n_valid) break;
    const float v = stage_f32_ptr(st, lane, j >> 2)[j & 3];
    if (flags & EPI_OUT_NCT) { op.out[((long long)b * op.n_valid + n) * op.T_out + t] = v; continue; }
    if (flags & EPI_OUT_F32) op.out[m * op.out_ld + n] = v;
    if (flags & EPI_OUT_SPLIT) {
      const long long o = m * op.out_split_ld + n;
      if (f16) {
        const __half h = __float2half_rn(v);
        reinterpret_cast<__half*>(op.out_hi)[o] = h;
        reinterpret_cast<__half*>(op.out_lo)[o] = __float2half_rn(v - __half2float(h));
      } else {
        const __nv_bfloat16 h = __float2bfloat16_rn(v);
        op.out_hi[o] = h;
        op.out_lo[o] = __float2bfloat16_rn(v - __bfloat162float(h));
      }
    }
  }
}
__device__ __forceinline__ void park_row(uint8_t* st, int lane, const float* val) {
#pragma unroll
  for (int j = 0; j < 8; ++j) *reinterpret_cast<float4*>(stage_f32_ptr(st, lane, j)) = make_float4(val[4 * j], val[4 * j + 1], val[4 * j + 2], val[4 * j + 3]);
}
__device__ __forceinline__ void fetch_row(uint8_t* st, int lane, float* val) {
#pragma unroll
  for (int j = 0; j < 8; ++j) { const float4 v = *reinterpret_cast<const float4*>(stage_f32_ptr(st, lane, j)); val[4 * j] = v.x; val[4 * j + 1] = v.y; val[4 * j + 2] = v.z; val[4 * j + 3] = v.w; }
}

__device__ __forceinline__ void emit_chunk(const GemmOp& op, const TMap* tmo, uint8_t* st, int lane, bool leader, bool stage_f32, int b, int t,
                                           int t_warp0, long long m, bool mv, int nbase, const float* val, bool with_split = true,
                                           unsigned long long* stamp = nullptr) {
  if (stage_f32) {
#pragma unroll
    for (int j = 0; j < 8; ++j) *reinterpret_cast<float4*>(stage_f32_ptr(st, lane, j)) = make_float4(val[4 * j], val[4 * j + 1], val[4 * j + 2], val[4 * j + 3]);
  }
  const int tma = with_split ? op.tma_out : (op.tma_out & ~2);
  if (tma & 2) {
    const bool f16 = nbase >= op.f16_col0;
#pragma unroll
    for (int j = 0; j < 4; ++j) {
      uint4 hi, lo;
      if (f16) split8_f16(val + 8 * j, hi, lo); else split8(val + 8 * j, hi, lo);
      const int off = lane * 64 + ((j ^ ((lane >> 1) & 3)) << 4);
      *reinterpret_cast<uint4*>(st + 4096 + off) = hi;
      *reinterpret_cast<uint4*>(st + 6144 + off) = lo;
    }
  }
  if (stamp) { long long t; asm volatile("mov.u64 %0, %%clock64;" : "=l"(t)); stamp[12] = t; }
  if (tma & 3) {
    fence_proxy_async();
    __syncwarp();
    if (stamp) { long long t; asm volatile("mov.u64 %0, %%clock64;" : "=l"(t)); stamp[13] = t; }
    if (leader) {
      const uint32_t sa = smem_u32(st);
      if (tma & 1) tma_store_3d(&tmo[0], sa, nbase, t_warp0, b);
      if (tma & 2) { tma_store_3d(&tmo[1], sa + 4096u, nbase, t_warp0, b); tma_store_3d(&tmo[2], sa + 6144u, nbase, t_warp0, b); }
      bulk_commit();
    }
  }
  const int direct = ((op.flags & EPI_OUT_NCT) ? EPI_OUT_NCT : 0) | (((op.flags & EPI_OUT_F32) && !(op.tma_out & 1)) ? EPI_OUT_F32 : 0) |
                     (((op.flags & EPI_OUT_SPLIT) && with_split && !(op.tma_out & 2)) ? EPI_OUT_SPLIT : 0);
  if (direct) {
    if (!stage_f32) park_row(st, lane, val);
    if (mv) store_cold(op, direct, b, t, m, nbase, st, lane);
  }
}

__device__ __forceinline__ unsigned long long gtime() { unsigned long long t; asm volatile("mov.u64 %0, %%globaltimer;" : "=l"(t)); return t; }
#define XTRACE(i) do { if (op_param.trace && blockIdx.x == 0 && tid == 64) op_param.trace[16 + (i)] = gtime(); } while (0)
#define TRACE(i) do { if (op.trace && blockIdx.x == 0 && blockIdx.y == 0) op.trace[i] = gtime(); } while (0)
__device__ __forceinline__ long long gclk() { long long t; asm volatile("mov.u64 %0, %%clock64;" : "=l"(t)); return t; }
#define ETRACE(i) do { if (op.trace && blockIdx.x == 0 && blockIdx.y == 0 && warp == 2 && lane == 0) op.trace[8 + (i)] = gclk(); } while (0)

constexpr int kGemmOpHotBytes = (int)offsetof(GemmOp, tmap);
static_assert(kGemmOpHotBytes % 16 == 0 && kGemmOpHotBytes <= 2688 && sizeof(PrepOp) <= 320, "GemmOp's hot part must fit the shared-memory descriptor copy");

template <int BN_, bool LNF, bool XF, bool ENC = false>
__global__ void __launch_bounds__(kThreads, 1) gemm_tc_kernel(const __grid_constant__ GemmOp op_param) {
  using Cfg = TileCfg<BN_>;
  constexpr int BN = Cfg::BN;
  constexpr int kStageBytes = Cfg::kStageBytes;
  constexpr int kAccCols = 2 * BN;
  extern __shared__ uint8_t smem_raw[];
  const uint32_t raw = smem_u32(smem_raw);
  const uint32_t base = (raw + 1023u) & ~1023u;
  uint8_t* smem = smem_raw + (base - raw);
  const uint32_t bar_base = base + Cfg::kOffBar;
  auto full_bar = [&](int s) { return bar_base + 8u * s; };
  auto empty_bar = [&](int s) { return bar_base + 8u * (kMaxStages + s); };
  auto acc_full = [&](int a) { return bar_base + 8u * (2 * kMaxStages + a); };
  auto acc_empty = [&](int a) { return bar_base + 8u * (2 * kMaxStages + 2 + a); };
  volatile uint32_t* tmem_slot = reinterpret_cast<volatile uint32_t*>(smem + Cfg::kOffBar + 8 * (2 * kMaxStages + 4));
  auto a_ready = [&](int s) { return bar_base + 8u * (16 + s); };
  auto b_full = [&](int s) { return bar_base + 8u * (19 + s); };
  auto b_empty = [&](int s) { return bar_base + 8u * (21 + s); };

  const int tid = threadIdx.x, warp = tid >> 5, lane = tid & 31;
  {
    const uint4* src = reinterpret_cast<const uint4*>(&op_param);
    uint4* dst = reinterpret_cast<uint4*>(smem + Cfg::kOffDesc);
    for (int i = tid; i < kGemmOpHotBytes / 16; i += kThreads) dst[i] = src[i];
    if (XF && op_param.xmode && op_param.pre) {
      const uint4* ps = reinterpret_cast<const uint4*>(op_param.pre);
      uint4* pd = reinterpret_cast<uint4*>(smem + Cfg::kOffDesc + 2688);
      for (int i = tid; i < (int)(sizeof(PrepOp) / 16); i += kThreads) pd[i] = __ldg(ps + i);
    }
  }
  const GemmOp& op = *reinterpret_cast<const GemmOp*>(smem + Cfg::kOffDesc);
  const TMap* tmaps = op_param.tmap;
  const int tiles_per_batch = (op_param.T_out + BM - 1) / BM;
  const int n_tiles = op_param.N / BN;
  const int total_tiles = op_param.B * tiles_per_batch * n_tiles;
  const int ks = (XF && op_param.xmode && op_param.ksplit > 1) ? op_param.ksplit : 1;
  const int kr = (int)blockIdx.x % ks, bid = (int)blockIdx.x / ks, nblk = (int)gridDim.x / ks;
  const int my_tiles = (total_tiles - bid + nblk - 1) / nblk;
  const bool multi = my_tiles > 1;
  const int nst = multi ? Cfg::kStagesMulti : Cfg::kStagesSingle;
  uint8_t* stage_area = smem + (multi ? Cfg::kOffStagingMulti : 0);
  const int nkb = op_param.nkb_total;
  const bool tr0 = blockIdx.x == 0;
  auto xr_ready = [&]() { return bar_base + 8u * 23; };
  auto xr_full = [&]() { return bar_base + 8u * 24; };
  if (tid == 0 && op_param.trace && tr0) op_param.trace[0] = gtime();
  span_begin(op_param.span);

  if (warp == 1 && lane == 0) {
    for (int s = 0; s < kMaxStages; ++s) { mbar_init(full_bar(s), 1); mbar_init(empty_bar(s), 1); }
    for (int a = 0; a < 2; ++a) { mbar_init(acc_full(a), 1); mbar_init(acc_empty(a), kEpiWarps); }
    if (XF) { mbar_init(xr_ready(), 1); mbar_init(xr_full(), kEpiWarps); for (int a = 0; a < kXAStages; ++a) mbar_init(a_ready(a), kEpiWarps); for (int a = 0; a < kXBStages; ++a) { mbar_init(b_full(a), 1); mbar_init(b_empty(a), 1); } }
    mbar_fence_init();
  }
  if (warp == 0 && lane == 0) {
    for (int i = 0; i < 2 * op_param.nsrc; ++i) prefetch_tmap(&tmaps[i]);
    const TMap* pm = op_param.tmap_out;
    if (op_param.tma_out & 1) prefetch_tmap(&pm[0]);
    if (op_param.tma_out & 2) { prefetch_tmap(&pm[1]); prefetch_tmap(&pm[2]); }
  }
  pdl_trigger();
#ifdef NS2VC_TMEM_LATE
  __syncthreads();
  uint32_t tmem_base = 0;
  if (warp >= 1) {
    if (warp == 2) tmem_alloc(smem_u32((const void*)tmem_slot), 2 * kAccCols);
    tc_fence_before();
    asm volatile("bar.sync 2, 288;" ::: "memory");
    tc_fence_after();
    tmem_base = *tmem_slot;
  }
#else
  if (warp == 2) tmem_alloc(smem_u32((const void*)tmem_slot), 2 * kAccCols);
  tc_fence_before();
  __syncthreads();
  tc_fence_after();
  const uint32_t tmem_base = *tmem_slot;
#endif
  if (tid == 0 && tr0) TRACE(1);
  if constexpr (XF) if (ks > 1) cluster_sync_all();

  constexpr bool xpanel = XF;
  if constexpr (XF) {
    const int tile = bid, mtile = tile / n_tiles;
    const int xb = mtile / tiles_per_batch, xt0 = (mtile % tiles_per_batch) * BM, xn0 = (tile % n_tiles) * BN;
    int ncblk = 0;
    for (int si = 0; si < op.nxs; ++si) ncblk += op.xs[si].ncb;
    const int p_lo = ncblk * kr / ks, p_hi = ncblk * (kr + 1) / ks;
    if (warp == 0) {
      if (elect_one()) {
        auto issue_w = [&](const XSeg& xs, int cb, int sb) {
          const uint32_t b0 = base + kXOffB + sb * kXBStageBytes;
          mbar_arrive_expect_tx(b_full(sb), (uint32_t)xs.ntap * 2u * Cfg::kBTileBytes);
          for (int j = 0; j < xs.ntap; ++j) {
            const size_t eoff = ((size_t)(xs.kb_tap[j] + cb) * op.N + xn0) * 64;
            bulk_g2s(b0 + j * 2 * Cfg::kBTileBytes, op.w_hi + eoff, Cfg::kBTileBytes, b_full(sb));
            bulk_g2s(b0 + j * 2 * Cfg::kBTileBytes + Cfg::kBTileBytes, op.w_lo + eoff, Cfg::kBTileBytes, b_full(sb));
          }
        };
        { int it = 0, gp = 0;
          for (int si = 0; si < op.nxs && it < kXBStages; ++si)
            for (int cb = 0; cb < op.xs[si].ncb && it < kXBStages; ++cb, ++gp) {
              if (gp < p_lo || gp >= p_hi) continue;
              issue_w(op.xs[si], cb, it); ++it;
            } }
        pdl_wait();
        if (tr0) TRACE(2);
        int it = 0, gp = 0;
        for (int si = 0; si < op.nxs; ++si) {
          const XSeg& xs = op.xs[si];
          for (int cb = 0; cb < xs.ncb; ++cb, ++gp) {
            if (gp < p_lo || gp >= p_hi) continue;
            const int sa = it % kXAStages, sb = it % kXBStages;
            if (it >= kXAStages) mbar_wait(empty_bar(sa), (uint32_t)(((it / kXAStages) & 1) ^ 1));
            const uint32_t a_hi = base + sa * kXAStageBytes;
            const uint32_t rows = xs.ntap == 3 ? (uint32_t)kPanelRows : (uint32_t)BM;
            const int c = xs.c0 + cb * 64, trow = xt0 + (xs.ntap == 3 ? -1 : 0);
            mbar_arrive_expect_tx(full_bar(sa), 2u * rows * 128u);
            tma_load_3d(a_hi, &tmaps[2 * xs.src], c, trow, xb, full_bar(sa));
            tma_load_3d(a_hi + kPanelBytes, &tmaps[2 * xs.src + 1], c, trow, xb, full_bar(sa));
            if (it >= kXBStages) { mbar_wait(b_empty(sb), (uint32_t)(((it / kXBStages) & 1) ^ 1)); issue_w(xs, cb, sb); }
            ++it;
          }
        }
      }
    } else if (warp == 1) {
      if (elect_one()) {
        int it = 0, gp = 0;
        for (int si = 0; si < op.nxs; ++si) {
          const XSeg& xs = op.xs[si];
          for (int cb = 0; cb < xs.ncb; ++cb, ++gp) {
            if (gp < p_lo || gp >= p_hi) continue;
            const int sa = it % kXAStages, sb = it % kXBStages;
            mbar_wait(b_full(sb), (uint32_t)((it / kXBStages) & 1));
            mbar_wait(a_ready(sa), (uint32_t)((it / kXAStages) & 1));
            if (it == 0 && tr0) TRACE(3);
            tc_fence_after();
            const uint32_t a_hi = base + sa * kXAStageBytes, a_lo = a_hi + kPanelBytes, b0 = base + kXOffB + sb * kXBStageBytes;
            for (int j = 0; j < xs.ntap; ++j) {
#pragma unroll
              for (int k = 0; k < BK / 16; ++k) {
                const uint64_t dah = umma_desc(a_hi + j * 128 + k * 32), dal = umma_desc(a_lo + j * 128 + k * 32);
                const uint64_t dbh = umma_desc(b0 + j * 2 * Cfg::kBTileBytes + k * 32);
                umma_bf16(tmem_base, dah, dbh, Cfg::kIdesc2, (it | j | k) != 0 ? 1u : 0u);
                umma_bf16(tmem_base, dal, dbh, Cfg::kIdesc, 1u);
              }
            }
            umma_commit(empty_bar(sa));
            umma_commit(b_empty(sb));
            ++it;
          }
        }
        umma_commit(acc_full(0));
        if (tr0) TRACE(4);
      }
    } else {
      const int xt = tid - 64;
      float* aff = reinterpret_cast<float*>(smem + kXOffAff);
      const PrepOp& pr = *reinterpret_cast<const PrepOp*>(smem + Cfg::kOffDesc + 2688);
      const bool have_aff = op.pre != nullptr;
      const int C = have_aff ? pr.C1 + pr.C2 : 0;
      auto sync256 = [] { asm volatile("bar.sync 1, 256;" ::: "memory"); };
      float pg[kPrepSlots], pbv[kPrepSlots], fs[kPrepSlots], fbv[kPrepSlots];
      if (have_aff) prep_fetch_norm_weights(pr, C, pg, pbv, xt, 256);
      pdl_wait();
      XTRACE(0);
      if (have_aff) prep_fetch_film(pr, op.pre_film, xb, C, fs, fbv, xt, 256);
      bool aff_done = !have_aff;
      const bool silu = have_aff && pr.mode == PREP_AFFINE_SILU;
      int it = 0, gp = 0;
      for (int si = 0; si < op.nxs; ++si) {
        const XSeg& xs = op.xs[si];
        const int rows = xs.ntap == 3 ? kPanelRows : BM, tfirst = xt0 + (xs.ntap == 3 ? -1 : 0);
        const int Tsrc = op.src[xs.src].T;
        if (xs.xf && !aff_done && gp < p_hi && gp + xs.ncb > p_lo) {
          for (int c = C + xt; c < ((C + 63) & ~63); c += 256) { aff[c] = 0.f; aff[kXfMaxC + c] = 0.f; }
          prep_affine(pr, xb, C, kXfMaxC, aff, pg, pbv, fs, fbv, xt, 256, sync256);
          aff_done = true;
          XTRACE(1);
        }
        for (int cb = 0; cb < xs.ncb; ++cb, ++gp) {
          if (gp < p_lo || gp >= p_hi) continue;
          const int sa = it % kXAStages;
          const int q = xt & 7;
          float scv[8], shv[8];
          if (xs.xf) {
            const float* sc = aff + xs.aff_c0 + cb * 64 + q * 8;
            const float4 s0 = *reinterpret_cast<const float4*>(sc), s1 = *reinterpret_cast<const float4*>(sc + 4);
            const float4 b0 = *reinterpret_cast<const float4*>(sc + kXfMaxC), b1 = *reinterpret_cast<const float4*>(sc + kXfMaxC + 4);
            scv[0] = s0.x; scv[1] = s0.y; scv[2] = s0.z; scv[3] = s0.w; scv[4] = s1.x; scv[5] = s1.y; scv[6] = s1.z; scv[7] = s1.w;
            shv[0] = b0.x; shv[1] = b0.y; shv[2] = b0.z; shv[3] = b0.w; shv[4] = b1.x; shv[5] = b1.y; shv[6] = b1.z; shv[7] = b1.w;
          }
          mbar_wait(full_bar(sa), (uint32_t)((it / kXAStages) & 1));
          if (it == 0) XTRACE(2);
          if (xs.xf) {
            uint8_t* p_hi = smem + sa * kXAStageBytes;
            uint8_t* p_lo = p_hi + kPanelBytes;
            auto xform = [&](int r, uint4& h4, uint4& l4) {
              const int t = tfirst + r;
              const float keep = (t >= 0 && t < Tsrc) ? 1.f : 0.f;
              const uint32_t hw[4] = {h4.x, h4.y, h4.z, h4.w}, lw[4] = {l4.x, l4.y, l4.z, l4.w};
              float v[8];
#pragma unroll
              for (int j = 0; j < 4; ++j) {
                float x0, x1;
                upk2(fadd2(pk2(__uint_as_float(hw[j] << 16), __uint_as_float(hw[j] & 0xffff0000u)),
                           pk2(__uint_as_float(lw[j] << 16), __uint_as_float(lw[j] & 0xffff0000u))), x0, x1);
                unsigned long long y2 = ffma2(pk2(x0, x1), pk2(scv[2 * j], scv[2 * j + 1]), pk2(shv[2 * j], shv[2 * j + 1]));
                if (silu) y2 = silu2(y2);
                upk2(fmul2(y2, pk2(keep, keep)), v[2 * j], v[2 * j + 1]);
              }
              split8(v, h4, l4);
            };
            const int rb = xt >> 3;
            uint4 h4[4], l4[4];
            int off[4];
#pragma unroll
            for (int u = 0; u < 4; ++u) {
              const int r = rb + 32 * u;
              off[u] = r * 128 + ((q ^ (r & 7)) << 4);
              h4[u] = *reinterpret_cast<const uint4*>(p_hi + off[u]);
              l4[u] = *reinterpret_cast<const uint4*>(p_lo + off[u]);
            }
#pragma unroll
            for (int u = 0; u < 4; ++u) xform(rb + 32 * u, h4[u], l4[u]);
#pragma unroll
            for (int u = 0; u < 4; ++u) {
              *reinterpret_cast<uint4*>(p_hi + off[u]) = h4[u];
              *reinterpret_cast<uint4*>(p_lo + off[u]) = l4[u];
            }
            if (rb + 128 < rows) {
              const int r = rb + 128, o = r * 128 + ((q ^ (r & 7)) << 4);
              uint4 hh = *reinterpret_cast<const uint4*>(p_hi + o), ll = *reinterpret_cast<const uint4*>(p_lo + o);
              xform(r, hh, ll);
              *reinterpret_cast<uint4*>(p_hi + o) = hh; *reinterpret_cast<uint4*>(p_lo + o) = ll;
            }
            fence_proxy_async();
          }
          __syncwarp();
          if (lane == 0) mbar_arrive(a_ready(sa));
          if (it == 0) XTRACE(3);
          ++it;
        }
      }
      XTRACE(4);
    }
  }

  const int npf = nkb < nst ? nkb : nst;
  if constexpr (!xpanel) if (warp == 0 && elect_one()) {
    const int n0 = (bid % n_tiles) * BN;
    for (int kb = 0; kb < npf; ++kb) {
      const uint32_t b_hi = base + kb * kStageBytes + 2 * kATileBytes;
      mbar_arrive_expect_tx(full_bar(kb), 2u * kATileBytes + 2u * Cfg::kBTileBytes);
      const size_t eoff = ((size_t)kb * op.N + n0) * 64;
      bulk_g2s(b_hi, op.w_hi + eoff, Cfg::kBTileBytes, full_bar(kb));
      bulk_g2s(b_hi + Cfg::kBTileBytes, op.w_lo + eoff, Cfg::kBTileBytes, full_bar(kb));
    }
  }
  __syncwarp();

  if (warp == 0) {
    if constexpr (!xpanel) if (elect_one()) {
      const int npre = npf;
      pdl_wait();
      if (tr0) TRACE(2);
      int g = 0;
      for (int it = 0; it < my_tiles; ++it) {
        const int tile = bid + it * nblk;
        const int mt = tile / n_tiles, n0 = (tile % n_tiles) * BN;
        const int b = mt / tiles_per_batch, t0 = (mt % tiles_per_batch) * BM;
        int si = 0, kbl = 0;
        for (int kb = 0; kb < nkb; ++kb, ++g) {
          const int stage = g % nst;
          const GSeg& s = op.seg[si];
          const uint32_t a_hi = base + stage * kStageBytes;
          const uint32_t a_lo = a_hi + kATileBytes;
          const uint32_t b_hi = a_lo + kATileBytes;
          if (g >= npre) {
            if (g >= nst) mbar_wait(empty_bar(stage), (uint32_t)(((g / nst) & 1) ^ 1));
            mbar_arrive_expect_tx(full_bar(stage), 2u * kATileBytes + 2u * Cfg::kBTileBytes);
            const size_t eoff = ((size_t)kb * op.N + n0) * 64;
            bulk_g2s(b_hi, op.w_hi + eoff, Cfg::kBTileBytes, full_bar(stage));
            bulk_g2s(b_hi + Cfg::kBTileBytes, op.w_lo + eoff, Cfg::kBTileBytes, full_bar(stage));
          }
          const int c = s.c0 + kbl * 64;
          tma_load_3d(a_hi, &tmaps[2 * s.src], c, t0 + s.tap, b, full_bar(stage));
          tma_load_3d(a_lo, &tmaps[2 * s.src + 1], c, t0 + s.tap, b, full_bar(stage));
          if (++kbl == s.nkb) { kbl = 0; ++si; }
        }
      }
    }
  } else if (warp == 1) {
    if constexpr (!xpanel) if (elect_one()) {
      int g = 0;
      for (int it = 0; it < my_tiles; ++it) {
        const uint32_t acc = tmem_base + (uint32_t)((it & 1) * kAccCols);
        if (it >= 2) { mbar_wait(acc_empty(it & 1), (uint32_t)(((it >> 1) & 1) ^ 1)); tc_fence_after(); }
        for (int kb = 0; kb < nkb; ++kb, ++g) {
          const int stage = g % nst;
          mbar_wait(full_bar(stage), (uint32_t)((g / nst) & 1));
          if (g == 0 && tr0) TRACE(3);
          tc_fence_after();
          const uint32_t a_hi = base + stage * kStageBytes;
          const uint32_t a_lo = a_hi + kATileBytes;
          const uint32_t b_hi = a_lo + kATileBytes;
#pragma unroll
          for (int k = 0; k < BK / 16; ++k) {
            const uint64_t dah = umma_desc(a_hi + k * 32), dal = umma_desc(a_lo + k * 32);
            const uint64_t dbh = umma_desc(b_hi + k * 32);
            umma_bf16(acc, dah, dbh, Cfg::kIdesc2, (kb | k) != 0 ? 1u : 0u);
            umma_bf16(acc, dal, dbh, Cfg::kIdesc, 1u);
          }
          umma_commit(empty_bar(stage));
        }
        umma_commit(acc_full(it & 1));
        if (it == 0 && tr0) TRACE(4);
      }
    }
  } else {
    pdl_wait();
    __syncwarp();
    const bool leader = elect_one();
    const int q = warp & 3;
    const int r = q * 32 + lane;
    const int cc0 = (warp - 2) >> 2;
    uint8_t* st = stage_area + kStageOff + (warp - 2) * kStagePerWarp;
    const TMap* tmo = op_param.tmap_out;
    bool staged_once = false;
    for (int it = 0; it < my_tiles; ++it) {
      const int tile = bid + it * nblk;
      const int mt = tile / n_tiles, nt = tile % n_tiles, n0 = nt * BN;
      const int b = mt / tiles_per_batch, t0 = (mt % tiles_per_batch) * BM;
      const int t = t0 + r;
      const bool mv = t < op.T_out;
      const long long m = (long long)b * op.T_out + t;
      const uint32_t trow = tmem_base + (uint32_t)((it & 1) * kAccCols) + ((uint32_t)(q * 32) << 16);
      const int t_warp0 = t0 + q * 32;
      float pre[32];
      float preg[32];
      bool pre_ok = false;
      float ln_mu = 0.f, ln_rstd = 1.f;
      float* sg = reinterpret_cast<float*>(smem + Cfg::kOffLnG) + (warp - 2) * 128;
      if constexpr (LNF) {
        if (mv) ln_row_stats(op, m, ln_mu, ln_rstd);
        __syncwarp();
        if constexpr (BN == 128) {
          const int nb = nt * 64 + cc0 * 32 + lane;
          const bool ok = nb < op.n_valid;
          sg[lane] = ok ? __ldg(op.ln_g + nb) : 0.f;
          sg[32 + lane] = ok ? __ldg(op.ln_g + op.n_valid + nb) : 0.f;
          sg[64 + lane] = ok ? __ldg(op.bias + nb) : 0.f;
          sg[96 + lane] = ok ? __ldg(op.bias + op.n_valid + nb) : 0.f;
          pre_ok = BN == 128 && nt * 64 + cc0 * 32 + 32 <= op.n_valid;
        } else {
          const int nb = n0 + cc0 * 32 + lane;
          const bool ok = nb < op.n_valid;
          sg[lane] = ok ? __ldg(op.ln_g + nb) : 0.f;
          sg[64 + lane] = (ok && (op.flags & EPI_BIAS)) ? __ldg(op.bias + nb) : 0.f;
          pre_ok = mv && n0 + cc0 * 32 + 32 <= op.n_valid && !(op.flags & (EPI_ROWBIAS | EPI_RESIDUAL));
        }
        __syncwarp();
      }
      if constexpr (!LNF) {
      if constexpr (BN == 128) {
        const int nb = nt * 64 + cc0 * 32;
        if (BN == 128 && nb + 32 <= op.n_valid) {
          pre_ok = true;
          const float4* bv = reinterpret_cast<const float4*>(op.bias + nb);
          const float4* bg = reinterpret_cast<const float4*>(op.bias + op.n_valid + nb);
#pragma unroll
          for (int j = 0; j < 8; ++j) {
            const float4 x = __ldg(bv + j), y = __ldg(bg + j);
            pre[4 * j] = x.x; pre[4 * j + 1] = x.y; pre[4 * j + 2] = x.z; pre[4 * j + 3] = x.w;
            preg[4 * j] = y.x; preg[4 * j + 1] = y.y; preg[4 * j + 2] = y.z; preg[4 * j + 3] = y.w;
          }
        }
      } else {
        const int nb = n0 + cc0 * 32;
        if (mv && nb + 32 <= op.n_valid && !(op.flags & EPI_ROWBIAS) && (!(op.flags & EPI_RESIDUAL) || (op.res_ld & 3) == 0)) {
          pre_ok = true;
#pragma unroll
          for (int j = 0; j < 32; ++j) pre[j] = 0.f;
          if (op.flags & EPI_BIAS) {
            const float4* pb = reinterpret_cast<const float4*>(op.bias + nb);
#pragma unroll
            for (int j = 0; j < 8; ++j) { const float4 v = __ldg(pb + j); pre[4 * j] = v.x; pre[4 * j + 1] = v.y; pre[4 * j + 2] = v.z; pre[4 * j + 3] = v.w; }
          }
          if (op.flags & EPI_RESIDUAL) {
            const float4* pr = reinterpret_cast<const float4*>(op.res + m * op.res_ld + nb);
#pragma unroll
            for (int j = 0; j < 8; ++j) { const float4 v = __ldg(pr + j); pre[4 * j] += v.x; pre[4 * j + 1] += v.y; pre[4 * j + 2] += v.z; pre[4 * j + 3] += v.w; }
          }
        }
      }
      }
      float enc_keep = 1.f;
      if constexpr (ENC) if ((op.flags & EPI_ROWMASK) && mv) enc_keep = __ldg(op.rowmask + m);
      mbar_wait(acc_full(it & 1), (uint32_t)((it >> 1) & 1));
      if (it == 0 && tr0 && warp == 2 && lane == 0) TRACE(5);
      if (it == 0 && tr0) ETRACE(0);
      tc_fence_after();
      auto release_acc = [&]() {
        tc_fence_before();
        __syncwarp();
        if (lane == 0) mbar_arrive(acc_empty(it & 1));
      };
      auto wait_staging = [&]() {
        if (staged_once && op.tma_out) {
          if (leader) asm volatile("cp.async.bulk.wait_group.read 0;" ::: "memory");
          __syncwarp();
        }
      };
      if constexpr (BN == 128) {
        {
          const int hh = cc0;
          float val[32], gate[32];
          tmem_ld32_sum(trow + (uint32_t)(hh * 32), trow + (uint32_t)(BN + hh * 32), val);
          tmem_ld32_sum(trow + (uint32_t)(64 + hh * 32), trow + (uint32_t)(BN + 64 + hh * 32), gate);
          release_acc();
          const int nbase = nt * 64 + hh * 32;
          if (nbase < op.n_valid) {
            if (!mv) {
#pragma unroll
              for (int j = 0; j < 32; ++j) val[j] = 0.f;
            } else if (pre_ok) {
              if constexpr (LNF) {
#pragma unroll
                for (int j = 0; j < 32; j += 2) {
                  const float v0 = fmaf(ln_rstd, val[j] - ln_mu * sg[j], sg[64 + j]), v1 = fmaf(ln_rstd, val[j + 1] - ln_mu * sg[j + 1], sg[65 + j]);
                  const float g0 = fmaf(ln_rstd, gate[j] - ln_mu * sg[32 + j], sg[96 + j]), g1 = fmaf(ln_rstd, gate[j + 1] - ln_mu * sg[33 + j], sg[97 + j]);
                  upk2(fmul2(pk2(v0, v1), gelu_erf2(pk2(g0, g1))), val[j], val[j + 1]);
                }
              } else {
#pragma unroll
                for (int j = 0; j < 32; j += 2)
                  upk2(fmul2(fadd2(pk2(val[j], val[j + 1]), pk2(pre[j], pre[j + 1])), gelu_erf2(fadd2(pk2(gate[j], gate[j + 1]), pk2(preg[j], preg[j + 1])))),
                       val[j], val[j + 1]);
              }
            } else {
              wait_staging();
              park_row(st, lane, val);
#pragma unroll
              for (int j = 0; j < 8; ++j) reinterpret_cast<float4*>(st + 4096)[lane * 8 + j] = make_float4(gate[4 * j], gate[4 * j + 1], gate[4 * j + 2], gate[4 * j + 3]);
              epi_cold<LNF>(op, b, m, nbase, st, lane, true);
              fetch_row(st, lane, val);
            }
            wait_staging();
            emit_chunk(op, tmo, st, lane, leader, false, b, t, t_warp0, m, mv, nbase, val);
            staged_once = true;
          }
        }
      } else {
        float* sm_part = reinterpret_cast<float*>(stage_area) + (it & 1) * (4 * BN * 2);
        const bool stage_f32 = (op.tma_out & 1) || (op.flags & EPI_STATS);
#pragma unroll 1
        for (int cc = cc0; cc < BN / 32; cc += 2) {
          float acc[32];
          tmem_ld32_sum(trow + (uint32_t)(cc * 32), trow + (uint32_t)(BN + cc * 32), acc);
          if (cc + 2 >= BN / 32) release_acc();
          if (it == 0 && tr0) ETRACE(1);
          if constexpr (XF) if (ks > 1) {
            const int te = tid - 64;
            if (kr != 0) {
              mbar_wait_cluster(xr_ready(), 0);
              const uint32_t rbase = mapa_u32(base + kXOffB, 0);
#pragma unroll
              for (int j = 0; j < 8; ++j) st_remote_f32x4(rbase + (uint32_t)((j * 256 + te) * 16), acc[4 * j], acc[4 * j + 1], acc[4 * j + 2], acc[4 * j + 3]);
              asm volatile("fence.acq_rel.cluster;" ::: "memory");
              __syncwarp();
              if (lane == 0) mbar_arrive_remote(mapa_u32(xr_full(), 0));
              continue;
            }
            if (warp == 2 && lane == 0) mbar_arrive_remote(mapa_u32(xr_ready(), 1));
            mbar_wait_cluster(xr_full(), 0);
            const float4* xr = reinterpret_cast<const float4*>(smem + kXOffB);
#pragma unroll
            for (int j = 0; j < 8; ++j) {
              const float4 v = xr[j * 256 + te];
              acc[4 * j] += v.x; acc[4 * j + 1] += v.y; acc[4 * j + 2] += v.z; acc[4 * j + 3] += v.w;
            }
          }
          const int nbase = n0 + cc * 32;
          const bool cvalid = nbase < op.n_valid;
          if (cvalid) {
            const bool fullc = nbase + 32 <= op.n_valid;
            bool enc_hot = ENC && mv;
            if (!mv) {
#pragma unroll
              for (int j = 0; j < 32; ++j) acc[j] = 0.f;
            } else if (cc == cc0 && pre_ok) {
              if constexpr (LNF) {
#pragma unroll
                for (int j = 0; j < 32; ++j) acc[j] = fmaf(ln_rstd, acc[j] - ln_mu * sg[j], sg[64 + j]);
              } else {
#pragma unroll
                for (int j = 0; j < 32; ++j) acc[j] += pre[j];
              }
            } else if (!LNF && fullc && !(op.flags & EPI_ROWBIAS) && (!(op.flags & EPI_RESIDUAL) || (op.res_ld & 3) == 0)) {
              if (op.flags & EPI_BIAS) {
                const float4* pb = reinterpret_cast<const float4*>(op.bias + nbase);
#pragma unroll
                for (int j = 0; j < 8; ++j) { const float4 v = __ldg(pb + j); acc[4 * j] += v.x; acc[4 * j + 1] += v.y; acc[4 * j + 2] += v.z; acc[4 * j + 3] += v.w; }
              }
              if (op.flags & EPI_RESIDUAL) {
                const float4* pr = reinterpret_cast<const float4*>(op.res + m * op.res_ld + nbase);
#pragma unroll
                for (int j = 0; j < 8; ++j) { const float4 v = __ldg(pr + j); acc[4 * j] += v.x; acc[4 * j + 1] += v.y; acc[4 * j + 2] += v.z; acc[4 * j + 3] += v.w; }
              }
            } else {
              wait_staging();
              park_row(st, lane, acc);
              epi_cold<LNF>(op, b, m, nbase, st, lane, false);
              fetch_row(st, lane, acc);
              enc_hot = false;
            }
            if constexpr (ENC) if (enc_hot) {
              if (op.flags & EPI_RELU) {
#pragma unroll
                for (int j = 0; j < 32; ++j) acc[j] = fmaxf(acc[j], 0.f);
              }
              if (op.flags & EPI_ROWMASK) {
#pragma unroll
                for (int j = 0; j < 32; ++j) acc[j] *= enc_keep;
              }
            }
            if (it == 0 && tr0) ETRACE(2);
            if ((op.flags & EPI_ROWSTATS) && mv) {
              float rs = 0.f, rq = 0.f;
#pragma unroll
              for (int j = 0; j < 32; ++j) { rs += acc[j]; rq = fmaf(acc[j], acc[j], rq); }
              atomicAdd(op.row_stats + m * 2, (double)rs);
              atomicAdd(op.row_stats + m * 2 + 1, (double)rq);
            }
            wait_staging();
            emit_chunk(op, tmo, st, lane, leader, stage_f32, b, t, t_warp0, m, mv, nbase, acc, true,
                       (it == 0 && tr0 && warp == 2 && lane == 0) ? op.trace : nullptr);
            staged_once = true;
            if (it == 0 && tr0) ETRACE(3);
            if (op.flags & EPI_STATS) {
              __syncwarp();
              float cs = 0.f, cq = 0.f;
#pragma unroll
              for (int rr = 0; rr < 32; ++rr) { const float v = stage_f32_ptr(st, rr, lane >> 2)[lane & 3]; cs += v; cq += v * v; }
              sm_part[(q * BN + cc * 32 + lane) * 2] = cs;
              sm_part[(q * BN + cc * 32 + lane) * 2 + 1] = cq;
              if (it == 0 && tr0) ETRACE(4);
            }
          } else if (op.flags & EPI_STATS) {
            sm_part[(q * BN + cc * 32 + lane) * 2] = 0.f;
            sm_part[(q * BN + cc * 32 + lane) * 2 + 1] = 0.f;
          }
        }
        if ((op.flags & EPI_STATS) && kr == 0) {
          asm volatile("bar.sync 1, 256;" ::: "memory");
          if (it == 0 && tr0) ETRACE(5);
          const int col = tid - 64;
          if (col < BN && n0 + col < op.n_valid) {
            double cs = 0, cq = 0;
#pragma unroll
            for (int w = 0; w < 4; ++w) { cs += (double)sm_part[(w * BN + col) * 2]; cq += (double)sm_part[(w * BN + col) * 2 + 1]; }
            atomicAdd(op.stat_sum + (long long)b * op.n_valid + n0 + col, cs);
            atomicAdd(op.stat_sq + (long long)b * op.n_valid + n0 + col, cq);
          }
        }
      }
    }
    if (op.tma_out && leader) asm volatile("cp.async.bulk.wait_group.read 0;" ::: "memory");
  }

  if (warp == 2 && lane == 0 && tr0) TRACE(6);
  if (tr0) ETRACE(6);
  tc_fence_before();
  __syncthreads();
  if (tr0) ETRACE(7);
  if (tid == 0 && tr0) TRACE(7);
  span_end(op.span);
  if (warp == 2) tmem_dealloc(tmem_base, 2 * kAccCols);
}

typedef CUresult (*EncodeTiledFn)(CUtensorMap*, CUtensorMapDataType, cuuint32_t, void*, const cuuint64_t*, const cuuint64_t*,
                                  const cuuint32_t*, const cuuint32_t*, CUtensorMapInterleave, CUtensorMapSwizzle,
                                  CUtensorMapL2promotion, CUtensorMapFloatOOBfill);
static EncodeTiledFn get_encode_fn() {
  static EncodeTiledFn fn = nullptr;
  if (!fn) {
    void* p = nullptr;
    cudaDriverEntryPointQueryResult q;
    if (cudaGetDriverEntryPoint("cuTensorMapEncodeTiled", &p, cudaEnableDefault, &q) == cudaSuccess && q == cudaDriverEntryPointSuccess)
      fn = reinterpret_cast<EncodeTiledFn>(p);
  }
  return fn;
}

int encode_tmap_any(TMap* out, const void* base, int elem_bytes, int C, int T, int B, int ld, int box_c, int box_rows, int swizzle_bytes,
                    long long bpitch) {
  static_assert(sizeof(CUtensorMap) == sizeof(TMap), "CUtensorMap size");
  EncodeTiledFn fn = get_encode_fn();
  if (!fn) { set_error("cuTensorMapEncodeTiled entry point not available"); return -2; }
  if (((long long)ld * elem_bytes) % 16 || (reinterpret_cast<uintptr_t>(base) & 15)) { set_error("buffer not TMA-aligned (ld=%d)", ld); return -1; }
  const CUtensorMapSwizzle sw = swizzle_bytes == 128 ? CU_TENSOR_MAP_SWIZZLE_128B : swizzle_bytes == 64 ? CU_TENSOR_MAP_SWIZZLE_64B
                               : swizzle_bytes == 32 ? CU_TENSOR_MAP_SWIZZLE_32B : CU_TENSOR_MAP_SWIZZLE_NONE;
  const cuuint64_t gdim[3] = {(cuuint64_t)C, (cuuint64_t)T, (cuuint64_t)B};
  const cuuint64_t gstr[2] = {(cuuint64_t)ld * elem_bytes, (cuuint64_t)(bpitch ? bpitch : (long long)T * ld) * elem_bytes};
  const cuuint32_t box[3] = {(cuuint32_t)box_c, (cuuint32_t)box_rows, 1};
  const cuuint32_t estr[3] = {1, 1, 1};
  CUresult r = fn(reinterpret_cast<CUtensorMap*>(out), elem_bytes == 4 ? CU_TENSOR_MAP_DATA_TYPE_FLOAT32 : CU_TENSOR_MAP_DATA_TYPE_BFLOAT16, 3,
                  const_cast<void*>(base), gdim, gstr, box, estr, CU_TENSOR_MAP_INTERLEAVE_NONE, sw, CU_TENSOR_MAP_L2_PROMOTION_L2_256B,
                  CU_TENSOR_MAP_FLOAT_OOB_FILL_NONE);
  if (r != CUDA_SUCCESS) { set_error("cuTensorMapEncodeTiled failed (%d) C=%d T=%d B=%d ld=%d box=%dx%d sw=%d", (int)r, C, T, B, ld, box_c, box_rows, swizzle_bytes); return -2; }
  return 0;
}
int encode_tmap_rows(TMap* out, const __nv_bfloat16* base, int C, int T, int B, int ld, int box_c, int box_rows, int swizzle_bytes) {
  return encode_tmap_any(out, base, 2, C, T, B, ld, box_c, box_rows, swizzle_bytes);
}

static int encode_one(TMap* out, const __nv_bfloat16* base, const SplitBuf& s, int B, int box_rows) {
  return encode_tmap_any(out, base, 2, s.C, s.T, B, s.ld, 64, box_rows, 128, s.bpitch);
}

int encode_tmaps(GemmOp& op) {
  op.tma_out = 0;
  if (!(op.flags & EPI_OUT_NCT)) {
    if ((op.flags & EPI_OUT_F32) && op.out && (op.out_ld & 3) == 0 && (reinterpret_cast<uintptr_t>(op.out) & 15) == 0) {
      int rc = encode_tmap_any(&op.tmap_out[0], op.out, 4, op.n_valid, op.T_out, op.B, op.out_ld, 32, 32, 128);
      if (rc) return rc;
      op.tma_out |= 1;
    }
    if ((op.flags & EPI_OUT_SPLIT) && (op.out_split_ld & 7) == 0 && (reinterpret_cast<uintptr_t>(op.out_hi) & 15) == 0 &&
        (reinterpret_cast<uintptr_t>(op.out_lo) & 15) == 0) {
      int rc = encode_tmap_any(&op.tmap_out[1], op.out_hi, 2, op.n_valid, op.T_out, op.B, op.out_split_ld, 32, 32, 64);
      if (rc) return rc;
      rc = encode_tmap_any(&op.tmap_out[2], op.out_lo, 2, op.n_valid, op.T_out, op.B, op.out_split_ld, 32, 32, 64);
      if (rc) return rc;
      op.tma_out |= 2;
    }
  }
  for (int i = 0; i < op.nsrc; ++i) {
    int box_rows = BM;
    if (op.xmode)
      for (int k = 0; k < op.nxs; ++k) if (op.xs[k].src == i && op.xs[k].ntap == 3) box_rows = kPanelRows;
    int rc = encode_one(&op.tmap[2 * i], op.src[i].hi, op.src[i], op.B, box_rows);
    if (rc) return rc;
    rc = encode_one(&op.tmap[2 * i + 1], op.src[i].lo, op.src[i], op.B, box_rows);
    if (rc) return rc;
  }
  return 0;
}

static int sm_count() {
  static int n = 0;
  if (!n) {
    int dev = 0;
    cudaGetDevice(&dev);
    if (cudaDeviceGetAttribute(&n, cudaDevAttrMultiProcessorCount, dev) != cudaSuccess || n <= 0) n = 148;
  }
  return n;
}

template <int BN_, bool LNF, bool XF, bool ENC = false>
static int launch_bn(const GemmOp& op, cudaStream_t st) {
  using Cfg = TileCfg<BN_>;
  static bool attr_set = false;
  if (!attr_set) {
    cudaError_t e = cudaFuncSetAttribute(gemm_tc_kernel<BN_, LNF, XF, ENC>, cudaFuncAttributeMaxDynamicSharedMemorySize, Cfg::kSmemBytes);
    if (e != cudaSuccess) { set_error("gemm_tc: cannot set %d B dynamic smem: %s", Cfg::kSmemBytes, cudaGetErrorString(e)); return -2; }
    attr_set = true;
  }
  const int tiles = op.B * ceil_div(op.T_out, BM) * (op.N / BN_);
  int grid = (XF && op.xmode) ? tiles : (tiles < sm_count() ? tiles : sm_count());
  dim3 cluster(1, 1, 1);
  if (XF && op.xmode && op.ksplit > 1) { grid = tiles * op.ksplit; cluster.x = (unsigned)op.ksplit; }
  cudaError_t e = launch_kc(gemm_tc_kernel<BN_, LNF, XF, ENC>, dim3(grid), dim3(kThreads), (size_t)Cfg::kSmemBytes, st, cluster, op);
  if (e != cudaSuccess) { set_error("gemm_tc launch failed: %s", cudaGetErrorString(e)); return -2; }
  return 0;
}

int gemm_sm_count() { return sm_count(); }

void plan_gemm(GemmOp& op) {
  op.bn = (op.flags & EPI_GEGLU) ? 128 : 64;
}

int launch_gemm_tc(const GemmOp& op, cudaStream_t st) {
  if (op.N % 128) { set_error("gemm_tc: packed N=%d is not a multiple of 128", op.N); return -1; }
  const bool lnf = (op.flags & EPI_LNFOLD) != 0;
  if (op.flags & (EPI_RELU | EPI_ROWMASK)) {
    if (lnf || op.xmode || op.bn != 64 || (op.flags & EPI_GEGLU)) { set_error("gemm_tc: ReLU / row-mask epilogues need a plain 64-wide tile"); return -1; }
    if ((op.flags & EPI_ROWMASK) && !op.rowmask) { set_error("gemm_tc: EPI_ROWMASK without a mask"); return -1; }
    if (op.nkb_total <= 0) { set_error("gemm_tc: empty K"); return -1; }
    return launch_bn<64, false, false, true>(op, st);
  }
  if (op.xmode) {
    if (lnf || op.bn != 64 || op.nxs < 1 || op.nxs > kMaxXSeg) { set_error("gemm_tc: panel mode needs a plain 64-wide tile and 1..%d segments", kMaxXSeg); return -1; }
    if (op.pre == nullptr) { set_error("gemm_tc: panel mode without GroupNorm parameters"); return -1; }
    if (op.ksplit != 1 && op.ksplit != 2) { set_error("gemm_tc: ksplit must be 1 or 2"); return -1; }
    return launch_bn<64, false, true>(op, st);
  }
  if (op.nkb_total <= 0) { set_error("gemm_tc: empty K"); return -1; }
  if ((op.bn == 128) != ((op.flags & EPI_GEGLU) != 0)) { set_error("gemm_tc: the 128-wide tile is the GEGLU instantiation (plan_gemm)"); return -1; }
  if (op.bn == 128) return lnf ? launch_bn<128, true, false>(op, st) : launch_bn<128, false, false>(op, st);
  if (op.bn != 64) { set_error("gemm_tc: plan_gemm() was not called"); return -1; }
  return lnf ? launch_bn<64, true, false>(op, st) : launch_bn<64, false, false>(op, st);
}

}
```

Baseline: 2941.

## Fuse transformer feed-forward FF1+GEGLU+FF2 into a single tensor-core kernel

Adds a dedicated fused FFN kernel that computes the LN-folded FF1 projection, applies GEGLU in the epilogue into a shared-memory G tile, and immediately feeds it into FF2 accumulation in TMEM, with split-K partials exchanged across a cluster. This removes the round trip of the 4C-wide intermediate activation through global memory and one kernel launch per transformer block, and drops the large ff scratch buffer when the fused path applies. In exchange it adds a complex warp-specialized pipeline with cluster-level reduction and a tight shared-memory/TMEM budget, which risks lower occupancy or serialization for small C.

```diff
diff --git a/ns2vc_b200/csrc/common.cuh b/ns2vc_b200/csrc/common.cuh
--- a/ns2vc_b200/csrc/common.cuh
+++ b/ns2vc_b200/csrc/common.cuh
@@ -148,6 +148,36 @@
 int launch_gemm_tc(const GemmOp& op, cudaStream_t st);
 int launch_gemm_simt(const GemmOp& op, cudaStream_t st);
 int encode_tmaps(GemmOp& op);
+int encode_store_tmaps(TMap* maps, int& tma_out, int flags, const float* out, int out_ld, const __nv_bfloat16* out_hi,
+                       const __nv_bfloat16* out_lo, int out_split_ld, int n_valid, int T_out, int B);
+
+struct FfnOp {
+  int B, T, C;
+  SplitBuf a;
+  const __nv_bfloat16* w1_hi;
+  const __nv_bfloat16* w1_lo;
+  const __nv_bfloat16* w2_hi;
+  const __nv_bfloat16* w2_lo;
+  const double* ln_stats;
+  const float* ln_g;
+  const float* ln_bf;
+  int ln_C; float ln_eps;
+  const float* bias;
+  const float* res;
+  int flags;
+  int tma_out, f16_col0, n_valid, T_out, out_ld, out_split_ld;
+  float* out;
+  __nv_bfloat16* out_hi;
+  __nv_bfloat16* out_lo;
+  double* stat_sum;
+  double* stat_sq;
+  unsigned long long* span;
+  TMap tmap_a[2];
+  TMap tmap_out[3];
+};
+bool ffn_tc_supported(int C);
+int encode_ffn_tmaps(FfnOp& op);
+int launch_ffn_tc(const FfnOp& op, cudaStream_t st);
 
 struct PackSeg {
   const float* w;
diff --git a/ns2vc_b200/csrc/engine.cu b/ns2vc_b200/csrc/engine.cu
--- a/ns2vc_b200/csrc/engine.cu
+++ b/ns2vc_b200/csrc/engine.cu
@@ -62,8 +62,9 @@
 struct ConvSite { std::string p; int c; PackedB w; };
 
 struct Launch {
-  enum Kind { GEMM, ATTN, LN_SPLIT, LN_APPLY, LINEAR, NCT2SPLIT, POOL_CLS, POOL_ATT, MASKBIAS, PREP, MEMSET, TAP } kind;
+  enum Kind { GEMM, ATTN, LN_SPLIT, LN_APPLY, LINEAR, NCT2SPLIT, POOL_CLS, POOL_ATT, MASKBIAS, PREP, MEMSET, FFN, TAP } kind;
   GemmOp gemm;
+  FfnOp ffn;
   AttnOp attn;
   LinOp lin;
   PrepOp prep;
@@ -562,6 +563,12 @@
     return cudaMemcpyAsync(aff_dev, aff_host.data(), aff_host.size() * sizeof(PrepOp), cudaMemcpyHostToDevice, st) == cudaSuccess ? 0 : -2;
   }
   void push(const Launch& l) { out->push_back(l); }
+  void emit_ffn(FfnOp& f) {
+    Launch l; l.kind = Launch::FFN;
+    if (!dry) { int rc = encode_ffn_tmaps(f); if (rc) err = rc; }
+    l.ffn = f;
+    out->push_back(l);
+  }
   void emit_prep(const float* s1, int C1, const float* s2, int C2, int T_src, int T_dst, int mode, const float* scale,
                  const float* shift, const SplitBuf& o, const SplitBuf* raw = nullptr, int row_mul = 1, int row_add = 0,
                  const int* rowmap = nullptr, int patch = 0) {
@@ -700,14 +707,18 @@
   size_t stat_used = 0;
   auto new_stats = [&](int C) { double* p = stat_arena ? stat_arena + stat_used : nullptr; stat_used += (size_t)2 * B * C; return p; };
   auto new_rowstats = [&](size_t nrows) { double* p = stat_arena ? stat_arena + stat_used : nullptr; stat_used += 2 * nrows; return p; };
-  auto with_stats = [&](GemmOp& g, double* st_, int C) { g.flags |= EPI_STATS; g.stat_sum = st_; g.stat_sq = st_ ? st_ + (size_t)B * C : nullptr; };
+  auto with_stats = [&](auto& g, double* st_, int C) { g.flags |= EPI_STATS; g.stat_sum = st_; g.stat_sq = st_ ? st_ + (size_t)B * C : nullptr; };
   { Launch l; l.kind = Launch::MEMSET; l.mem = stat_arena; l.mem_bytes = stat_doubles * sizeof(double); fwd.push_back(l); }
   size_t max_act = (size_t)B * T * c0, max_cat = 0, max_ff = 1, max_qkv = 1;
+  auto fused_ff = [&](int C) { return h->merge_ff && h->lnfold && !h->simt && ffn_tc_supported(C); };
   for (auto& o : h->plan) {
     const size_t rows = (size_t)B * Tl[o.level];
     if (o.kind == PlanOp::RESNET) { max_act = std::max(max_act, rows * o.cout); max_cat = std::max(max_cat, rows * o.cin); }
     if (o.kind == PlanOp::DOWN || o.kind == PlanOp::UP) { max_act = std::max(max_act, rows * o.cout); max_cat = std::max(max_cat, rows * o.cout); }
-    if (o.kind == PlanOp::XFORMER) { max_act = std::max(max_act, rows * o.cout); max_ff = std::max(max_ff, rows * 4 * o.cout); max_qkv = std::max(max_qkv, rows * 3 * o.cout); }
+    if (o.kind == PlanOp::XFORMER) {
+      max_act = std::max(max_act, rows * o.cout); max_qkv = std::max(max_qkv, rows * 3 * o.cout);
+      if (!fused_ff(o.cout)) max_ff = std::max(max_ff, rows * 4 * o.cout);
+    }
   }
   max_cat = std::max(max_cat, max_act);
   float* rot[3]; for (int i = 0; i < 3; ++i) rot[i] = ar.get<float>(max_act);
@@ -750,7 +761,7 @@
     else { a.p = rot[rot_i]; if (xf_on) a.sp = Builder::view(rot_sp[rot_i], TLn, C); rot_i = (rot_i + 1) % 3; }
     return a;
   };
-  auto emits_block_out = [&](GemmOp& g, const Act& a) {
+  auto emits_block_out = [&](auto& g, const Act& a) {
     g.flags |= EPI_OUT_F32; g.out = a.p; g.out_ld = a.c;
     if (xf_on) { g.flags |= EPI_OUT_SPLIT; g.out_hi = a.sp.hi; g.out_lo = a.sp.lo; g.out_split_ld = a.sp.ld; }
   };
@@ -910,12 +921,24 @@
           if (fold) emits_ln_input(g, rs3);
           bld.emit_gemm(g, x.out2); }
         if (!fold) bld.emit_ln_split(T0, C, (int)rows, C, h->W(b + ".norm3.weight"), h->W(b + ".norm3.bias"), sx);
+        Act outp = next_out(followed_by_push(pi), TL, C);
+        outp.st = new_stats(C);
+        if (fused_ff(C)) {
+          FfnOp f; memset(&f, 0, sizeof(f));
+          f.B = B; f.T = TL; f.C = C; f.a = sln;
+          f.w1_hi = x.ff1.hi; f.w1_lo = x.ff1.lo; f.w2_hi = x.ff2p.hi; f.w2_lo = x.ff2p.lo;
+          f.ln_stats = rs3; f.ln_g = x.g_ff1; f.ln_bf = x.bf_ff1; f.ln_C = C; f.ln_eps = 1e-5f;
+          f.bias = x.bias_ff2p; f.res = cur.p;
+          f.n_valid = C; f.T_out = TL; f.f16_col0 = 0x7fffffff;
+          emits_block_out(f, outp); with_stats(f, outp.st, C); bld.emit_ffn(f);
+          cur = outp;
+          bld.emit_tap(x.p, cur.p, o.level, C, TL);
+          break;
+        }
         { GemmOp g = lin(x.ff1, sn, C); g.flags = EPI_GEGLU | EPI_OUT_SPLIT; g.bias = h->W(b + ".ff.net.0.proj.bias");
           g.out_hi = sff.hi; g.out_lo = sff.lo; g.out_split_ld = sff.ld;
           if (fold) { consumes_ln(g, rs3, x.g_ff1, x.bf_ff1); g.flags &= ~EPI_BIAS; }
           bld.emit_gemm(g, x.ff1); }
-        Act outp = next_out(followed_by_push(pi), TL, C);
-        outp.st = new_stats(C);
         if (h->merge_ff && fold) {
           GemmOp g = bld.gemm_base(x.ff2p, TL);
           const int i0 = bld.add_src(g, sff); bld.seg(g, i0, 0, 4 * C, 0);
@@ -1074,6 +1097,12 @@
         rc = launch_prep_split(p, st);
         break;
       }
+      case Launch::FFN: {
+        FfnOp f = l.ffn;
+        if (h->span && count < h->span_cap) f.span = h->span + 2 * count;
+        rc = launch_ffn_tc(f, st);
+        break;
+      }
       case Launch::MEMSET: {
         cudaError_t e = cudaMemsetAsync(l.mem, 0, l.mem_bytes, st);
         if (e != cudaSuccess) { set_error("memset failed: %s", cudaGetErrorString(e)); rc = -2; }
@@ -1098,6 +1127,7 @@
       if (l.kind == Launch::GEMM) { pr.M = l.gemm.B * l.gemm.T_out; pr.N = l.gemm.n_valid; pr.K = l.gemm.nkb_total * 64; pr.nseg = l.gemm.nseg; }
       if (l.kind == Launch::PREP) { pr.M = l.prep.B * l.prep.T_dst; pr.N = l.prep.C1 + l.prep.C2; }
       if (l.kind == Launch::ATTN) { pr.M = l.attn.Tq; pr.N = l.attn.Tk; pr.K = l.attn.dh; }
+      if (l.kind == Launch::FFN) { pr.M = l.ffn.B * l.ffn.T; pr.N = l.ffn.C; pr.K = l.ffn.C; }
       h->prof.push_back(pr);
     }
     if (rc) return rc;
@@ -1389,11 +1419,11 @@
   h->profiling = on != 0;
   return 0;
 }
-int ns2vc_profile_num_kinds(void) { return 11; }
+int ns2vc_profile_num_kinds(void) { return 12; }
 const char* ns2vc_profile_kind_name(int k) {
   static const char* names[] = {"gemm_tc", "attention", "ln_split", "ln_apply", "small_linear", "nct_to_split",
-                               "pool_class_token", "pool_attend", "mask_bias", "prep_split", "memset"};
-  return (k >= 0 && k < 11) ? names[k] : "";
+                               "pool_class_token", "pool_attend", "mask_bias", "prep_split", "memset", "gemm_ffn"};
+  return (k >= 0 && k < 12) ? names[k] : "";
 }
 int ns2vc_unet_profile_read(ns2vc_unet* h, int kind, double* ms_total, long long* launches) {
   NS_REQUIRE(h && ms_total && launches, "null argument");
diff --git a/ns2vc_b200/csrc/ffn_tc.cu b/ns2vc_b200/csrc/ffn_tc.cu
--- /dev/null
+++ b/ns2vc_b200/csrc/ffn_tc.cu
@@ -0,0 +1,326 @@
+#include "gemm_common.cuh"
+#include "tc_common.cuh"
+#include "launch.cuh"
+
+namespace ns2vc {
+namespace {
+
+constexpr int kEpiWarps = 8;
+constexpr int kThreads = (2 + kEpiWarps) * 32;
+constexpr int kTileBytes = 128 * 64 * 2;
+constexpr int kPairBytes = 2 * kTileBytes;
+constexpr int kChunks = 4;
+constexpr int kStagePerWarp = 8192;
+constexpr uint32_t kIdesc = umma_idesc_bf16(128, 128);
+
+constexpr unsigned long long kSched = 0x0ull | 1ull << 4 | 4ull << 8 | 2ull << 12 | 5ull << 16 | 3ull << 20 | 6ull << 24 | 8ull << 28 | 7ull << 32;
+constexpr int kSteps = 9;
+__device__ __forceinline__ int sched(int i) { return (int)((kSched >> (4 * i)) & 15); }
+
+template <int CC> struct FfnCfg {
+  static constexpr int KS = CC / 64;
+  static constexpr int NH = CC / 128;
+  static constexpr int kStages = CC == 128 ? 4 : 2;
+  static constexpr int kOffRing = KS * kPairBytes;
+  static constexpr int kOffG = kOffRing + kStages * kPairBytes;
+  static constexpr int kOffTab = kOffG + kPairBytes;
+  static constexpr int kOffBar = kOffTab + 1024;
+  static constexpr int kSmemBytes = kOffBar + 256 + 1024 ;
+  static constexpr int kAcc2 = 256;
+  static constexpr int kTotalStages = kChunks * (KS + NH) + NH;
+  static_assert(kSmemBytes <= 227 * 1024, "shared memory budget");
+  static_assert(2 * 128 <= kAcc2 && kAcc2 + CC <= 512, "TMEM budget: two FF1 chunk buffers and the FF2 accumulator");
+  static_assert(kEpiWarps * kStagePerWarp <= kStages * kPairBytes, "output staging overlays the weight ring");
+  static_assert((KS - 1) * 128 * 64 * 4 <= kOffRing, "partners' partial slices overlay the A region");
+  static_assert(4 * 64 * 2 * 4 <= kPairBytes, "column sums overlay the G tile");
+  static_assert(kTotalStages > kStages, "the producer waits for the dependency inside its stage loop");
+};
+
+template <int CC> __device__ __forceinline__ size_t w_off(int code, int sub, int r) {
+  if (code < 4) return ((size_t)sub * (8 * CC) + (size_t)(r * kChunks + code) * 128) * 64;
+  const int kb = code < 8 ? r * kChunks + (code - 4) : CC / 16 + r;
+  return ((size_t)kb * CC + sub * 128) * 64;
+}
+
+template <int CC>
+__global__ void __launch_bounds__(kThreads, 1) ffn_tc_kernel(const __grid_constant__ FfnOp op) {
+  using Cfg = FfnCfg<CC>;
+  constexpr int KS = Cfg::KS, NH = Cfg::NH, kStages = Cfg::kStages;
+  extern __shared__ uint8_t smem_raw[];
+  const uint32_t raw = smem_u32(smem_raw);
+  const uint32_t base = (raw + 1023u) & ~1023u;
+  uint8_t* smem = smem_raw + (base - raw);
+  const uint32_t bar = base + Cfg::kOffBar;
+  auto w_full = [&](int s) { return bar + 8u * s; };
+  auto w_empty = [&](int s) { return bar + 8u * (4 + s); };
+  auto acc1_full = [&](int a) { return bar + 8u * (8 + a); };
+  auto acc1_empty = [&](int a) { return bar + 8u * (10 + a); };
+  const uint32_t a_full = bar + 8u * 12, g_full = bar + 8u * 13, g_empty = bar + 8u * 14, acc2_full = bar + 8u * 15;
+  const uint32_t peer_ready = bar + 8u * 16;
+  const uint32_t land_full = bar + 8u * 17;
+  volatile uint32_t* tmem_slot = reinterpret_cast<volatile uint32_t*>(smem + Cfg::kOffBar + 8 * 18);
+
+  const int tid = threadIdx.x, warp = tid >> 5, lane = tid & 31;
+  const int r = (int)blockIdx.x % KS, rb = (int)blockIdx.x / KS;
+  const int tpb = (op.T + 127) / 128, b = rb / tpb, t0 = (rb % tpb) * 128;
+  span_begin(op.span);
+
+  if (warp == 1 && lane == 0) {
+    for (int s = 0; s < kStages; ++s) { mbar_init(w_full(s), 1); mbar_init(w_empty(s), 1); }
+    for (int a = 0; a < 2; ++a) { mbar_init(acc1_full(a), 1); mbar_init(acc1_empty(a), kEpiWarps); }
+    mbar_init(a_full, 1); mbar_init(g_full, kEpiWarps); mbar_init(g_empty, 1); mbar_init(acc2_full, 1);
+    mbar_init(peer_ready, KS - 1); mbar_init(land_full, (KS - 1) * kEpiWarps);
+    mbar_fence_init();
+  }
+  if (warp == 0 && lane == 0) {
+    prefetch_tmap(&op.tmap_a[0]); prefetch_tmap(&op.tmap_a[1]);
+    if (op.tma_out & 1) prefetch_tmap(&op.tmap_out[0]);
+    if (op.tma_out & 2) { prefetch_tmap(&op.tmap_out[1]); prefetch_tmap(&op.tmap_out[2]); }
+  }
+  pdl_trigger();
+  if (warp == 2) tmem_alloc(smem_u32((const void*)tmem_slot), 512);
+  tc_fence_before();
+  __syncthreads();
+  tc_fence_after();
+  const uint32_t tmem_base = *tmem_slot;
+  cluster_sync_all();
+
+  if (warp == 0) {
+    if (elect_one()) {
+      int step = 0, sub = 0;
+      for (int g = 0; g < Cfg::kTotalStages; ++g) {
+        if (g == kStages) {
+          pdl_wait();
+          mbar_arrive_expect_tx(a_full, (uint32_t)(KS * kPairBytes));
+          for (int kb = 0; kb < KS; ++kb) {
+            tma_load_3d(base + kb * kPairBytes, &op.tmap_a[0], kb * 64, t0, b, a_full);
+            tma_load_3d(base + kb * kPairBytes + kTileBytes, &op.tmap_a[1], kb * 64, t0, b, a_full);
+          }
+        }
+        const int code = sched(step), s = g % kStages;
+        if (g >= kStages) mbar_wait(w_empty(s), (uint32_t)(((g / kStages) & 1) ^ 1));
+        const size_t e = w_off<CC>(code, sub, r);
+        const uint32_t dst = base + Cfg::kOffRing + s * kPairBytes;
+        mbar_arrive_expect_tx(w_full(s), (uint32_t)kPairBytes);
+        bulk_g2s(dst, (code < 4 ? op.w1_hi : op.w2_hi) + e, kTileBytes, w_full(s));
+        bulk_g2s(dst + kTileBytes, (code < 4 ? op.w1_lo : op.w2_lo) + e, kTileBytes, w_full(s));
+        if (++sub == (code < 4 ? KS : NH)) { sub = 0; ++step; }
+      }
+    }
+  } else if (warp == 1) {
+    if (elect_one()) {
+      mbar_wait(a_full, 0);
+      tc_fence_after();
+      int g = 0;
+      auto mma4 = [&](uint32_t acc, uint32_t a_hi, uint32_t b_hi, bool first) {
+#pragma unroll
+        for (int k = 0; k < 4; ++k) {
+          const uint64_t dah = umma_desc(a_hi + k * 32), dal = umma_desc(a_hi + kTileBytes + k * 32);
+          const uint64_t dbh = umma_desc(b_hi + k * 32), dbl = umma_desc(b_hi + kTileBytes + k * 32);
+          umma_bf16(acc, dah, dbh, kIdesc, (first && k == 0) ? 0u : 1u);
+          umma_bf16(acc, dah, dbl, kIdesc, 1u);
+          umma_bf16(acc, dal, dbh, kIdesc, 1u);
+          umma_bf16(acc, dal, dbl, kIdesc, 1u);
+        }
+      };
+      for (int i = 0; i < kSteps; ++i) {
+        const int code = sched(i);
+        if (code < 4) {
+          const int buf = code & 1;
+          const uint32_t acc = tmem_base + (uint32_t)(buf * 128);
+          if (code >= 2) { mbar_wait(acc1_empty(buf), 0); tc_fence_after(); }
+          for (int kb = 0; kb < KS; ++kb, ++g) {
+            const int s = g % kStages;
+            mbar_wait(w_full(s), (uint32_t)((g / kStages) & 1));
+            tc_fence_after();
+            mma4(acc, base + kb * kPairBytes, base + Cfg::kOffRing + s * kPairBytes, kb == 0);
+            umma_commit(w_empty(s));
+          }
+          umma_commit(acc1_full(buf));
+        } else {
+          uint32_t a_hi = base + r * kPairBytes;
+          if (code < 8) { mbar_wait(g_full, (uint32_t)(code & 1)); tc_fence_after(); a_hi = base + Cfg::kOffG; }
+          for (int h = 0; h < NH; ++h, ++g) {
+            const int s = g % kStages;
+            mbar_wait(w_full(s), (uint32_t)((g / kStages) & 1));
+            tc_fence_after();
+            mma4(tmem_base + (uint32_t)(Cfg::kAcc2 + h * 128), a_hi, base + Cfg::kOffRing + s * kPairBytes, code == 4);
+            umma_commit(w_empty(s));
+          }
+          if (code < 8) umma_commit(g_empty);
+        }
+      }
+      umma_commit(acc2_full);
+    }
+  } else {
+    const int te = tid - 64, q = warp & 3, hh = (warp - 2) >> 2;
+    const int row = q * 32 + lane, t = t0 + row;
+    const bool mv = t < op.T;
+    const long long m = (long long)b * op.T + t;
+    const uint32_t lane_off = (uint32_t)(q * 32) << 16;
+    float* tab = reinterpret_cast<float*>(smem + Cfg::kOffTab);
+    auto sync_epi = [] { asm volatile("bar.sync 1, 256;" ::: "memory"); };
+    auto tab_entry = [&](int ch) {
+      const int part = te >> 6, n = (r * kChunks + ch) * 64 + (te & 63);
+      return __ldg(((part & 2) ? op.ln_bf : op.ln_g) + ((part & 1) ? 4 * CC : 0) + n);
+    };
+    float tnext = tab_entry(0);
+    pdl_wait();
+    float mu = 0.f, rstd = 1.f;
+    if (mv) ln_row_stats(op, m, mu, rstd);
+    __syncwarp();
+    const bool leader = elect_one();
+    uint8_t* gt = smem + Cfg::kOffG;
+    for (int ch = 0; ch < kChunks; ++ch) {
+      const int buf = ch & 1;
+      sync_epi();
+      tab[te] = tnext;
+      if (ch + 1 < kChunks) tnext = tab_entry(ch + 1);
+      sync_epi();
+      mbar_wait(acc1_full(buf), (uint32_t)((ch >> 1) & 1));
+      tc_fence_after();
+      float val[32], gate[32];
+      tmem_ld32(tmem_base + (uint32_t)(buf * 128 + hh * 32) + lane_off, val);
+      tmem_ld32(tmem_base + (uint32_t)(buf * 128 + 64 + hh * 32) + lane_off, gate);
+      tc_fence_before();
+      __syncwarp();
+      if (lane == 0) mbar_arrive(acc1_empty(buf));
+      const float* sg = tab + hh * 32;
+      if (mv) {
+#pragma unroll
+        for (int j = 0; j < 32; j += 2) {
+          const float v0 = fmaf(rstd, val[j] - mu * sg[j], sg[128 + j]), v1 = fmaf(rstd, val[j + 1] - mu * sg[j + 1], sg[129 + j]);
+          const float g0 = fmaf(rstd, gate[j] - mu * sg[64 + j], sg[192 + j]), g1 = fmaf(rstd, gate[j + 1] - mu * sg[65 + j], sg[193 + j]);
+          upk2(fmul2(pk2(v0, v1), gelu_erf2(pk2(g0, g1))), val[j], val[j + 1]);
+        }
+      } else {
+#pragma unroll
+        for (int j = 0; j < 32; ++j) val[j] = 0.f;
+      }
+      uint4 h4[4], l4[4];
+#pragma unroll
+      for (int j = 0; j < 4; ++j) split8(val + 8 * j, h4[j], l4[j]);
+      if (ch > 0) mbar_wait(g_empty, (uint32_t)((ch - 1) & 1));
+#pragma unroll
+      for (int j = 0; j < 4; ++j) {
+        const int off = row * 128 + (((hh * 4 + j) ^ (row & 7)) << 4);
+        *reinterpret_cast<uint4*>(gt + off) = h4[j];
+        *reinterpret_cast<uint4*>(gt + kTileBytes + off) = l4[j];
+      }
+      fence_proxy_async();
+      __syncwarp();
+      if (lane == 0) mbar_arrive(g_full);
+    }
+
+    const int n0 = r * 64, nbase = n0 + hh * 32;
+    float pre[32];
+    if (mv) {
+      const float4* pb = reinterpret_cast<const float4*>(op.bias + nbase);
+      const float4* pr = reinterpret_cast<const float4*>(op.res + m * CC + nbase);
+#pragma unroll
+      for (int j = 0; j < 8; ++j) {
+        const float4 u = __ldg(pb + j), v = __ldg(pr + j);
+        pre[4 * j] = u.x + v.x; pre[4 * j + 1] = u.y + v.y; pre[4 * j + 2] = u.z + v.z; pre[4 * j + 3] = u.w + v.w;
+      }
+    }
+    mbar_wait(acc2_full, 0);
+    tc_fence_after();
+    if (warp == 2 && lane == 0)
+      for (int p = 0; p < KS; ++p) if (p != r) mbar_arrive_remote(mapa_u32(peer_ready, (uint32_t)p));
+    if (KS > 1) mbar_wait_cluster(peer_ready, 0);
+#pragma unroll 1
+    for (int p = 0; p < KS; ++p) {
+      if (p == r) continue;
+      float v[32];
+      tmem_ld32(tmem_base + (uint32_t)(Cfg::kAcc2 + p * 64 + hh * 32) + lane_off, v);
+      const uint32_t dst = mapa_u32(base + (uint32_t)((r < p ? r : r - 1) * 256 * 128), (uint32_t)p);
+#pragma unroll
+      for (int j = 0; j < 8; ++j) st_remote_f32x4(dst + (uint32_t)((j * 256 + te) * 16), v[4 * j], v[4 * j + 1], v[4 * j + 2], v[4 * j + 3]);
+    }
+    if (KS > 1) {
+      asm volatile("fence.acq_rel.cluster;" ::: "memory");
+      __syncwarp();
+      if (lane == 0)
+        for (int p = 0; p < KS; ++p) if (p != r) mbar_arrive_remote(mapa_u32(land_full, (uint32_t)p));
+    }
+    float acc[32];
+    tmem_ld32(tmem_base + (uint32_t)(Cfg::kAcc2 + r * 64 + hh * 32) + lane_off, acc);
+    if (KS > 1) {
+      mbar_wait_cluster(land_full, 0);
+#pragma unroll 1
+      for (int s = 0; s < KS - 1; ++s) {
+        const float4* xr = reinterpret_cast<const float4*>(smem + s * 256 * 128);
+#pragma unroll
+        for (int j = 0; j < 8; ++j) {
+          const float4 v = xr[j * 256 + te];
+          acc[4 * j] += v.x; acc[4 * j + 1] += v.y; acc[4 * j + 2] += v.z; acc[4 * j + 3] += v.w;
+        }
+      }
+    }
+#pragma unroll
+    for (int j = 0; j < 32; ++j) acc[j] = mv ? acc[j] + pre[j] : 0.f;
+    uint8_t* st = smem + Cfg::kOffRing + (warp - 2) * kStagePerWarp;
+    const bool stats = (op.flags & EPI_STATS) != 0;
+    emit_chunk(op, op.tmap_out, st, lane, leader, (op.tma_out & 1) || stats, b, t, t0 + q * 32, m, mv, nbase, acc);
+    if (stats) {
+      __syncwarp();
+      float cs = 0.f, cq = 0.f;
+#pragma unroll
+      for (int rr = 0; rr < 32; ++rr) { const float v = stage_f32_ptr(st, rr, lane >> 2)[lane & 3]; cs += v; cq += v * v; }
+      float* sm_part = reinterpret_cast<float*>(gt);
+      sm_part[(q * 64 + hh * 32 + lane) * 2] = cs;
+      sm_part[(q * 64 + hh * 32 + lane) * 2 + 1] = cq;
+      sync_epi();
+      if (te < 64) {
+        double ds = 0, dq = 0;
+#pragma unroll
+        for (int w = 0; w < 4; ++w) { ds += (double)sm_part[(w * 64 + te) * 2]; dq += (double)sm_part[(w * 64 + te) * 2 + 1]; }
+        atomicAdd(op.stat_sum + (long long)b * CC + n0 + te, ds);
+        atomicAdd(op.stat_sq + (long long)b * CC + n0 + te, dq);
+      }
+    }
+    if (op.tma_out && leader) asm volatile("cp.async.bulk.wait_group.read 0;" ::: "memory");
+  }
+
+  tc_fence_before();
+  __syncthreads();
+  span_end(op.span);
+  if (warp == 2) tmem_dealloc(tmem_base, 512);
+}
+
+template <int CC>
+int launch_cc(const FfnOp& op, cudaStream_t st) {
+  constexpr int smem = FfnCfg<CC>::kSmemBytes;
+  static bool attr_set = false;
+  if (!attr_set) {
+    cudaError_t e = cudaFuncSetAttribute(ffn_tc_kernel<CC>, cudaFuncAttributeMaxDynamicSharedMemorySize, smem);
+    if (e != cudaSuccess) { set_error("ffn_tc: cannot set %d B dynamic smem: %s", smem, cudaGetErrorString(e)); return -2; }
+    attr_set = true;
+  }
+  const int grid = op.B * ceil_div(op.T, 128) * (CC / 64);
+  cudaError_t e = launch_kc(ffn_tc_kernel<CC>, dim3(grid), dim3(kThreads), (size_t)smem, st, dim3(CC / 64, 1, 1), op);
+  if (e != cudaSuccess) { set_error("ffn_tc launch failed: %s", cudaGetErrorString(e)); return -2; }
+  return 0;
+}
+
+}
+
+bool ffn_tc_supported(int C) { return C == 128 || C == 256; }
+
+int encode_ffn_tmaps(FfnOp& op) {
+  int rc = encode_tmap_any(&op.tmap_a[0], op.a.hi, 2, op.a.C, op.a.T, op.B, op.a.ld, 64, 128, 128, op.a.bpitch);
+  if (!rc) rc = encode_tmap_any(&op.tmap_a[1], op.a.lo, 2, op.a.C, op.a.T, op.B, op.a.ld, 64, 128, 128, op.a.bpitch);
+  if (!rc) rc = encode_store_tmaps(op.tmap_out, op.tma_out, op.flags, op.out, op.out_ld, op.out_hi, op.out_lo, op.out_split_ld, op.n_valid, op.T_out, op.B);
+  return rc;
+}
+
+int launch_ffn_tc(const FfnOp& op, cudaStream_t st) {
+  if (op.n_valid != op.C || op.T_out != op.T || op.ln_C != op.C || op.a.C != op.C) { set_error("ffn_tc: inconsistent operator (C=%d)", op.C); return -1; }
+  if ((op.flags & EPI_STATS) && !(op.stat_sum && op.stat_sq)) { set_error("ffn_tc: EPI_STATS without sums"); return -1; }
+  if (op.C == 128) return launch_cc<128>(op, st);
+  if (op.C == 256) return launch_cc<256>(op, st);
+  set_error("ffn_tc: width %d not supported (128 or 256)", op.C);
+  return -1;
+}
+
+}
diff --git a/ns2vc_b200/csrc/gemm_common.cuh b/ns2vc_b200/csrc/gemm_common.cuh
--- a/ns2vc_b200/csrc/gemm_common.cuh
+++ b/ns2vc_b200/csrc/gemm_common.cuh
@@ -1,5 +1,7 @@
 #pragma once
 #include "common.cuh"
+#include "tc_common.cuh"
+#include <cuda_fp16.h>
 
 namespace ns2vc {
 
@@ -107,7 +109,8 @@
   return __bfloat162float(src.hi[off]) + __bfloat162float(src.lo[off]);
 }
 
-__device__ __forceinline__ void ln_row_stats(const GemmOp& op, long long m, float& mu, float& rstd) {
+template <class Op>
+__device__ __forceinline__ void ln_row_stats(const Op& op, long long m, float& mu, float& rstd) {
   const double s = op.ln_stats[m * 2], q = op.ln_stats[m * 2 + 1];
   const double mean = s / (double)op.ln_C;
   double var = q / (double)op.ln_C - mean * mean;
@@ -138,4 +141,81 @@
   return v;
 }
 
-}
+__device__ __forceinline__ float* stage_f32_ptr(uint8_t* st, int row, int c4) {
+  return reinterpret_cast<float*>(st + row * 128 + ((c4 ^ (row & 7)) << 4));
+}
+
+template <class Op>
+__device__ __noinline__ void store_cold(const Op& op, int flags, int b, int t, long long m, int nbase, uint8_t* st, int lane) {
+  const bool f16 = nbase >= op.f16_col0;
+#pragma unroll 1
+  for (int j = 0; j < 32; ++j) {
+    const int n = nbase + j;
+    if (n >= op.n_valid) break;
+    const float v = stage_f32_ptr(st, lane, j >> 2)[j & 3];
+    if (flags & EPI_OUT_NCT) { op.out[((long long)b * op.n_valid + n) * op.T_out + t] = v; continue; }
+    if (flags & EPI_OUT_F32) op.out[m * op.out_ld + n] = v;
+    if (flags & EPI_OUT_SPLIT) {
+      const long long o = m * op.out_split_ld + n;
+      if (f16) {
+        const __half h = __float2half_rn(v);
+        reinterpret_cast<__half*>(op.out_hi)[o] = h;
+        reinterpret_cast<__half*>(op.out_lo)[o] = __float2half_rn(v - __half2float(h));
+      } else {
+        const __nv_bfloat16 h = __float2bfloat16_rn(v);
+        op.out_hi[o] = h;
+        op.out_lo[o] = __float2bfloat16_rn(v - __bfloat162float(h));
+      }
+    }
+  }
+}
+__device__ __forceinline__ void park_row(uint8_t* st, int lane, const float* val) {
+#pragma unroll
+  for (int j = 0; j < 8; ++j) *reinterpret_cast<float4*>(stage_f32_ptr(st, lane, j)) = make_float4(val[4 * j], val[4 * j + 1], val[4 * j + 2], val[4 * j + 3]);
+}
+__device__ __forceinline__ void fetch_row(uint8_t* st, int lane, float* val) {
+#pragma unroll
+  for (int j = 0; j < 8; ++j) { const float4 v = *reinterpret_cast<const float4*>(stage_f32_ptr(st, lane, j)); val[4 * j] = v.x; val[4 * j + 1] = v.y; val[4 * j + 2] = v.z; val[4 * j + 3] = v.w; }
+}
+
+template <class Op>
+__device__ __forceinline__ void emit_chunk(const Op& op, const TMap* tmo, uint8_t* st, int lane, bool leader, bool stage_f32, int b, int t,
+                                           int t_warp0, long long m, bool mv, int nbase, const float* val, bool with_split = true,
+                                           unsigned long long* stamp = nullptr) {
+  if (stage_f32) {
+#pragma unroll
+    for (int j = 0; j < 8; ++j) *reinterpret_cast<float4*>(stage_f32_ptr(st, lane, j)) = make_float4(val[4 * j], val[4 * j + 1], val[4 * j + 2], val[4 * j + 3]);
+  }
+  const int tma = with_split ? op.tma_out : (op.tma_out & ~2);
+  if (tma & 2) {
+    const bool f16 = nbase >= op.f16_col0;
+#pragma unroll
+    for (int j = 0; j < 4; ++j) {
+      uint4 hi, lo;
+      if (f16) split8_f16(val + 8 * j, hi, lo); else split8(val + 8 * j, hi, lo);
+      const int off = lane * 64 + ((j ^ ((lane >> 1) & 3)) << 4);
+      *reinterpret_cast<uint4*>(st + 4096 + off) = hi;
+      *reinterpret_cast<uint4*>(st + 6144 + off) = lo;
+    }
+  }
+  if (stamp) { long long t; asm volatile("mov.u64 %0, %%clock64;" : "=l"(t)); stamp[12] = t; }
+  if (tma & 3) {
+    fence_proxy_async();
+    __syncwarp();
+    if (stamp) { long long t; asm volatile("mov.u64 %0, %%clock64;" : "=l"(t)); stamp[13] = t; }
+    if (leader) {
+      const uint32_t sa = smem_u32(st);
+      if (tma & 1) tma_store_3d(&tmo[0], sa, nbase, t_warp0, b);
+      if (tma & 2) { tma_store_3d(&tmo[1], sa + 4096u, nbase, t_warp0, b); tma_store_3d(&tmo[2], sa + 6144u, nbase, t_warp0, b); }
+      bulk_commit();
+    }
+  }
+  const int direct = ((op.flags & EPI_OUT_NCT) ? EPI_OUT_NCT : 0) | (((op.flags & EPI_OUT_F32) && !(op.tma_out & 1)) ? EPI_OUT_F32 : 0) |
+                     (((op.flags & EPI_OUT_SPLIT) && with_split && !(op.tma_out & 2)) ? EPI_OUT_SPLIT : 0);
+  if (direct) {
+    if (!stage_f32) park_row(st, lane, val);
+    if (mv) store_cold(op, direct, b, t, m, nbase, st, lane);
+  }
+}
+
+}
diff --git a/ns2vc_b200/csrc/gemm_tc.cu b/ns2vc_b200/csrc/gemm_tc.cu
--- a/ns2vc_b200/csrc/gemm_tc.cu
+++ b/ns2vc_b200/csrc/gemm_tc.cu
@@ -48,10 +48,6 @@
 static_assert(kXOffAff + kXAffBytes <= TileCfg<64>::kPipeBytes && kPrepSlots * kEpiWarps * 32 >= kXfMaxC, "panel mode: stages + affine table inside the pipeline area");
 
 
-__device__ __forceinline__ float* stage_f32_ptr(uint8_t* st, int row, int c4) {
-  return reinterpret_cast<float*>(st + row * 128 + ((c4 ^ (row & 7)) << 4));
-}
-
 
 template <bool LNF>
 __device__ __noinline__ void epi_cold(const GemmOp& op, int b, long long m, int nbase, uint8_t* st, int lane, bool with_gate) {
@@ -62,77 +58,6 @@
     *pv = (nbase + j < op.n_valid) ? epi_value<LNF>(op, b, m, nbase + j, *pv, g) : 0.f;
   }
 }
-__device__ __noinline__ void store_cold(const GemmOp& op, int flags, int b, int t, long long m, int nbase, uint8_t* st, int lane) {
-  const bool f16 = nbase >= op.f16_col0;
-#pragma unroll 1
-  for (int j = 0; j < 32; ++j) {
-    const int n = nbase + j;
-    if (n >= op.n_valid) break;
-    const float v = stage_f32_ptr(st, lane, j >> 2)[j & 3];
-    if (flags & EPI_OUT_NCT) { op.out[((long long)b * op.n_valid + n) * op.T_out + t] = v; continue; }
-    if (flags & EPI_OUT_F32) op.out[m * op.out_ld + n] = v;
-    if (flags & EPI_OUT_SPLIT) {
-      const long long o = m * op.out_split_ld + n;
-      if (f16) {
-        const __half h = __float2half_rn(v);
-        reinterpret_cast<__half*>(op.out_hi)[o] = h;
-        reinterpret_cast<__half*>(op.out_lo)[o] = __float2half_rn(v - __half2float(h));
-      } else {
-        const __nv_bfloat16 h = __float2bfloat16_rn(v);
-        op.out_hi[o] = h;
-        op.out_lo[o] = __float2bfloat16_rn(v - __bfloat162float(h));
-      }
-    }
-  }
-}
-__device__ __forceinline__ void park_row(uint8_t* st, int lane, const float* val) {
-#pragma unroll
-  for (int j = 0; j < 8; ++j) *reinterpret_cast<float4*>(stage_f32_ptr(st, lane, j)) = make_float4(val[4 * j], val[4 * j + 1], val[4 * j + 2], val[4 * j + 3]);
-}
-__device__ __forceinline__ void fetch_row(uint8_t* st, int lane, float* val) {
-#pragma unroll
-  for (int j = 0; j < 8; ++j) { const float4 v = *reinterpret_cast<const float4*>(stage_f32_ptr(st, lane, j)); val[4 * j] = v.x; val[4 * j + 1] = v.y; val[4 * j + 2] = v.z; val[4 * j + 3] = v.w; }
-}
-
-__device__ __forceinline__ void emit_chunk(const GemmOp& op, const TMap* tmo, uint8_t* st, int lane, bool leader, bool stage_f32, int b, int t,
-                                           int t_warp0, long long m, bool mv, int nbase, const float* val, bool with_split = true,
-                                           unsigned long long* stamp = nullptr) {
-  if (stage_f32) {
-#pragma unroll
-    for (int j = 0; j < 8; ++j) *reinterpret_cast<float4*>(stage_f32_ptr(st, lane, j)) = make_float4(val[4 * j], val[4 * j + 1], val[4 * j + 2], val[4 * j + 3]);
-  }
-  const int tma = with_split ? op.tma_out : (op.tma_out & ~2);
-  if (tma & 2) {
-    const bool f16 = nbase >= op.f16_col0;
-#pragma unroll
-    for (int j = 0; j < 4; ++j) {
-      uint4 hi, lo;
-      if (f16) split8_f16(val + 8 * j, hi, lo); else split8(val + 8 * j, hi, lo);
-      const int off = lane * 64 + ((j ^ ((lane >> 1) & 3)) << 4);
-      *reinterpret_cast<uint4*>(st + 4096 + off) = hi;
-      *reinterpret_cast<uint4*>(st + 6144 + off) = lo;
-    }
-  }
-  if (stamp) { long long t; asm volatile("mov.u64 %0, %%clock64;" : "=l"(t)); stamp[12] = t; }
-  if (tma & 3) {
-    fence_proxy_async();
-    __syncwarp();
-    if (stamp) { long long t; asm volatile("mov.u64 %0, %%clock64;" : "=l"(t)); stamp[13] = t; }
-    if (leader) {
-      const uint32_t sa = smem_u32(st);
-      if (tma & 1) tma_store_3d(&tmo[0], sa, nbase, t_warp0, b);
-      if (tma & 2) { tma_store_3d(&tmo[1], sa + 4096u, nbase, t_warp0, b); tma_store_3d(&tmo[2], sa + 6144u, nbase, t_warp0, b); }
-      bulk_commit();
-    }
-  }
-  const int direct = ((op.flags & EPI_OUT_NCT) ? EPI_OUT_NCT : 0) | (((op.flags & EPI_OUT_F32) && !(op.tma_out & 1)) ? EPI_OUT_F32 : 0) |
-                     (((op.flags & EPI_OUT_SPLIT) && with_split && !(op.tma_out & 2)) ? EPI_OUT_SPLIT : 0);
-  if (direct) {
-    if (!stage_f32) park_row(st, lane, val);
-    if (mv) store_cold(op, direct, b, t, m, nbase, st, lane);
-  }
-}
-
 __device__ __forceinline__ unsigned long long gtime() { unsigned long long t; asm volatile("mov.u64 %0, %%globaltimer;" : "=l"(t)); return t; }
 #define XTRACE(i) do { if (op_param.trace && blockIdx.x == 0 && tid == 64) op_param.trace[16 + (i)] = gtime(); } while (0)
 #define TRACE(i) do { if (op.trace && blockIdx.x == 0 && blockIdx.y == 0) op.trace[i] = gtime(); } while (0)
@@ -763,28 +688,34 @@
   return encode_tmap_any(out, base, 2, s.C, s.T, B, s.ld, 64, box_rows, 128, s.bpitch);
 }
 
+int encode_store_tmaps(TMap* maps, int& tma_out, int flags, const float* out, int out_ld, const __nv_bfloat16* out_hi,
+                       const __nv_bfloat16* out_lo, int out_split_ld, int n_valid, int T_out, int B) {
+  tma_out = 0;
+  if (flags & EPI_OUT_NCT) return 0;
+  if ((flags & EPI_OUT_F32) && out && (out_ld & 3) == 0 && (reinterpret_cast<uintptr_t>(out) & 15) == 0) {
+    int rc = encode_tmap_any(&maps[0], out, 4, n_valid, T_out, B, out_ld, 32, 32, 128);
+    if (rc) return rc;
+    tma_out |= 1;
+  }
+  if ((flags & EPI_OUT_SPLIT) && (out_split_ld & 7) == 0 && (reinterpret_cast<uintptr_t>(out_hi) & 15) == 0 &&
+      (reinterpret_cast<uintptr_t>(out_lo) & 15) == 0) {
+    int rc = encode_tmap_any(&maps[1], out_hi, 2, n_valid, T_out, B, out_split_ld, 32, 32, 64);
+    if (rc) return rc;
+    rc = encode_tmap_any(&maps[2], out_lo, 2, n_valid, T_out, B, out_split_ld, 32, 32, 64);
+    if (rc) return rc;
+    tma_out |= 2;
+  }
+  return 0;
+}
+
 int encode_tmaps(GemmOp& op) {
-  op.tma_out = 0;
-  if (!(op.flags & EPI_OUT_NCT)) {
-    if ((op.flags & EPI_OUT_F32) && op.out && (op.out_ld & 3) == 0 && (reinterpret_cast<uintptr_t>(op.out) & 15) == 0) {
-      int rc = encode_tmap_any(&op.tmap_out[0], op.out, 4, op.n_valid, op.T_out, op.B, op.out_ld, 32, 32, 128);
-      if (rc) return rc;
-      op.tma_out |= 1;
-    }
-    if ((op.flags & EPI_OUT_SPLIT) && (op.out_split_ld & 7) == 0 && (reinterpret_cast<uintptr_t>(op.out_hi) & 15) == 0 &&
-        (reinterpret_cast<uintptr_t>(op.out_lo) & 15) == 0) {
-      int rc = encode_tmap_any(&op.tmap_out[1], op.out_hi, 2, op.n_valid, op.T_out, op.B, op.out_split_ld, 32, 32, 64);
-      if (rc) return rc;
-      rc = encode_tmap_any(&op.tmap_out[2], op.out_lo, 2, op.n_valid, op.T_out, op.B, op.out_split_ld, 32, 32, 64);
-      if (rc) return rc;
-      op.tma_out |= 2;
-    }
-  }
+  int rc = encode_store_tmaps(op.tmap_out, op.tma_out, op.flags, op.out, op.out_ld, op.out_hi, op.out_lo, op.out_split_ld, op.n_valid, op.T_out, op.B);
+  if (rc) return rc;
   for (int i = 0; i < op.nsrc; ++i) {
     int box_rows = BM;
     if (op.xmode)
       for (int k = 0; k < op.nxs; ++k) if (op.xs[k].src == i && op.xs[k].ntap == 3) box_rows = kPanelRows;
-    int rc = encode_one(&op.tmap[2 * i], op.src[i].hi, op.src[i], op.B, box_rows);
+    rc = encode_one(&op.tmap[2 * i], op.src[i].hi, op.src[i], op.B, box_rows);
     if (rc) return rc;
     rc = encode_one(&op.tmap[2 * i + 1], op.src[i].lo, op.src[i], op.B, box_rows);
     if (rc) return rc;
```

Measured after the change: 2988 (median of 6 runs). +1.6%, better.
